# arendu-zz/MacaronicUserModeling

Measured on AMD Instinct MI355X. Metric: LBP sweep iters/sec (whole node), batch=8192 graphs |X|=64, higher is better.
Workload: dtype f64

## Files before the change

include/mlbp.h:

```cpp
#ifndef MLBP_H
#define MLBP_H

#include <stdint.h>

#ifdef __cplusplus
extern "C" {
#endif

#define MLBP_VERSION_MAJOR 0
#define MLBP_VERSION_MINOR 1

enum {
  MLBP_OK = 0,
  MLBP_EINVAL = -1,
  MLBP_EHIP = -2,
  MLBP_ENODEVICE = -3,
  MLBP_ENOMEM = -4,
  MLBP_EUNSUPPORTED = -5
};

int mlbp_version(void);
const char* mlbp_arch(void);
const char* mlbp_last_error(void);
int mlbp_device_count(void);
// ... 16 lines not shown
                       int32_t* unary_slot);

enum { MLBP_OP_UNARY = 0, MLBP_OP_PAIR_TM = 1, MLBP_OP_PAIR_MT = 2, MLBP_OP_VAR = 3 };
int mlbp_compile_sweep(const mlbp_topology* t, int32_t root_var, int32_t* ops, int32_t cap_ops,
                       int32_t* srcs, int32_t cap_srcs, int32_t* n_srcs);

typedef struct mlbp_program mlbp_program;

int mlbp_program_create(const int32_t* ops, int32_t n_ops, const int32_t* srcs, int32_t n_srcs,
                        const int32_t* sweeps, int32_t n_sweeps, int32_t n_msgs, int32_t P, int32_t U,
                        mlbp_program** out);
int mlbp_program_destroy(mlbp_program* p);

int mlbp_program_reserve(mlbp_program* p, int32_t max_graphs);

int mlbp_program_plan(const int32_t* ops, int32_t n_ops, const int32_t* srcs, int32_t n_srcs,
                      const int32_t* sweeps, int32_t n_sweeps, int32_t n_msgs, int32_t P, int32_t U,
                      int32_t* out8);

enum { MLBP_IMAGE_FUSED = 0, MLBP_IMAGE_LEAN = 1, MLBP_IMAGE_SHARED = 2, MLBP_IMAGE_LEAN_READOUT = 3,
       MLBP_IMAGE_SHARED_READOUT = 4, MLBP_IMAGE_PRUNED = 5 };
int mlbp_program_image(const int32_t* ops, int32_t n_ops, const int32_t* srcs, int32_t n_srcs,
                       const int32_t* sweeps, int32_t n_sweeps, int32_t n_msgs, int32_t P, int32_t U,
                       int32_t n_vars, const int32_t* in_off, const int32_t* in_slots,
                       int32_t which, int32_t* out, int32_t cap);

int mlbp_program_set_readout(mlbp_program* p, int32_t n_vars, const int32_t* in_off, const int32_t* in_slots);

int mlbp_program_exact_count(const mlbp_program* p, int32_t B);
int mlbp_program_skippable_updates(const mlbp_program* p);

int mlbp_program_status(const mlbp_program* p);

struct mlbp_gradient_args;

typedef struct mlbp_posterior_args {
  const int32_t* labels;
  double* out;
  double* sum_out;
} mlbp_posterior_args;

typedef struct mlbp_sweep_args {
  int32_t B;
  int32_t X;
  int32_t n_pair_tables;
  int32_t n_unary_tables;
  const double* pair_tables;
  const int32_t* pair_tab;
  const double* unary_tables;
  const int32_t* unary_tab;
  double* msgs;
  int32_t normalize_messages;
  int32_t init_messages;
  double* marginals;
  const struct mlbp_gradient_args* gradient;
  int32_t flags;
  const int32_t* pair_tab_host;
  const float* pair_tables_f32;
  const mlbp_posterior_args* posterior;
} mlbp_sweep_args;

#define MLBP_SWEEP_SHARED_PAIR_TABLES 1
#define MLBP_SWEEP_NO_MESSAGE_WRITEBACK 2
#define MLBP_SWEEP_PAIR_TABLES_F32 4
#define MLBP_SWEEP_DENSE_TABLES 8
#define MLBP_SWEEP_APPROX_INFERENCE 16
#define MLBP_APPROX_K 100
#define MLBP_SWEEP_SKIP_UNCHANGED 32

int mlbp_sweep_f64(const mlbp_program* prog, const mlbp_sweep_args* a, void* stream);

int mlbp_sweep_groups_f64(const mlbp_program* const* progs, const mlbp_sweep_args* args, int32_t n_groups, void* stream);

int mlbp_set_sweep_variant(int32_t variant);

#define MLBP_KERNEL_EXACT 2
#define MLBP_KERNEL_SHARED_MFMA 3
#define MLBP_KERNEL_WIDE 4
#define MLBP_KERNEL_GENERIC 5
#define MLBP_KERNEL_SHARED_GEMM 6
#define MLBP_KERNEL_LEAN 7
int mlbp_last_sweep_kernel(void);
int mlbp_last_sweep_fused_gradient(void);

void mlbp_launch_log_reset(void);
int mlbp_launch_log(const void** handles, int max);

int mlbp_init_messages_f64(double* msgs, int64_t n_rows, int32_t X, void* stream);

int mlbp_marginals_f64(const double* msgs, int32_t B, int32_t n_msgs, int32_t X, int32_t n_vars,
                       const int32_t* in_off, const int32_t* in_slots, int32_t normalize_messages,
                       double* out, void* stream);

int mlbp_log_posterior_f64(const double* marginals, const int32_t* labels, int32_t B, int32_t n_vars,
                           int32_t X, double* out, void* stream);
int mlbp_log_posterior_sum_f64(const double* marginals, const int32_t* labels, int32_t B, int32_t n_vars,
                               int32_t X, double* out, double* sum_out, void* stream);

typedef struct mlbp_posterior_group {
  const double* marginals;
  const int32_t* labels;
  int32_t n_vars, B;
  int64_t start;
} mlbp_posterior_group;
int mlbp_log_posterior_groups_f64(const mlbp_posterior_group* groups, int32_t n_groups, int64_t n_total, int32_t X, double* out,
                                  void* stream);

int mlbp_pair_beliefs_f64(const double* msgs, int32_t B, int32_t n_msgs, int32_t X, int32_t P,
                          const double* pair_tables, const int32_t* pair_tab, int32_t n_pair_tables,
                          const int32_t* c_slot, const int32_t* r_slot, double* out, void* stream);

typedef struct mlbp_gradient_args {
  int32_t B, X, n_msgs, P, U;
  int32_t F_ee, F_ed;
  int32_t Vde;
  int32_t n_pair_tables, n_unary_tables;
  const double* msgs;
  const double* pair_tables;
  const int32_t* pair_tab;
  const int32_t* pair_c_slot;
  const int32_t* pair_r_slot;
  const int32_t* pair_phi;
  const int32_t* pair_label;
  const double* unary_tables;
  const int32_t* unary_tab;
  const int32_t* unary_kind;
  const int32_t* unary_obs;
  const int32_t* unary_label;
  const double* phi_en_en;
  const double* phi_en_en_w1;
  const double* phi_en_de;
  const double* phi_en_en_t;
  const double* phi_en_en_w1_t;
  const double* phi_en_de_t;
  const double* phi_en_en_p;
  const double* phi_en_en_w1_p;
  double* grad_en_en;
  double* grad_en_de;
  int32_t flags;
  const int32_t* pair_tab_host;
  const double* unary_expect;
  const int32_t* pair_slots_host;
  void* workspace;
  int64_t workspace_bytes;
} mlbp_gradient_args;
int64_t mlbp_gradient_workspace_bytes(const mlbp_gradient_args* a);
#define MLBP_GRADIENT_SHARED_PAIR_TABLES 1
#define MLBP_GRADIENT_APPROX_BELIEFS 2
int mlbp_gradient_f64(const mlbp_gradient_args* a, void* stream);

int mlbp_unary_expectations_f64(const double* unary_tables, int32_t n_rows, int32_t X, const int32_t* row_kind,
                                const int32_t* row_obs, const double* phi_en_en_t, const double* phi_en_en_w1_t,
                                const double* phi_en_de_t, int32_t F_ee, int32_t F_ed, int32_t Vde, double* out,
                                void* stream);
int mlbp_gradient_status(void);

int mlbp_patch_unary_tables_f64(const double* base_tables, const int32_t* base_row, const int32_t* item_off,
                                const int32_t* item_x, const int32_t* item_k, const double* item_val,
                                const double* theta, int32_t n_rows, int32_t X, double* out, void* stream);

int mlbp_patch_gradient_f64(const double* priv_tables, const int32_t* item_off, const int32_t* item_x,
                            const int32_t* item_k, const double* item_val, const int32_t* row_graph,
                            const int32_t* row_label, int32_t n_rows, int32_t X, int32_t F, double* grad, void* stream);

int mlbp_sum_rows_f64(const double* in, int64_t rows, int32_t cols, double* out, void* stream);
int mlbp_sum_rows_cat_f64(const double* in0, int32_t cols0, const double* in1, int32_t cols1, const double* in2,
// ... 67 lines not shown
```

macaronicusermodeling_amd/_ffi.py:

```python
import ctypes as C
import os

_PKG = os.path.dirname(os.path.abspath(__file__))
LIB_PATH = os.path.join(_PKG, 'libmlbp.so')

MLBP_OK, MLBP_EINVAL, MLBP_EHIP, MLBP_ENODEVICE, MLBP_ENOMEM, MLBP_EUNSUPPORTED = 0, -1, -2, -3, -4, -5
OP_UNARY, OP_PAIR_TM, OP_PAIR_MT, OP_VAR = 0, 1, 2, 3
IMAGES = ('fused', 'lean', 'shared', 'lean_readout', 'shared_readout', 'pruned')
NORM_ZERO, NORM_UNIFORM = 0, 1


class MlbpError(RuntimeError):
    def __init__(self, code, msg):
        RuntimeError.__init__(self, 'libmlbp error %d: %s' % (code, msg))
        self.code = code


class Topology(C.Structure):
    _fields_ = [('n_vars', C.c_int32), ('n_factors', C.c_int32),
                ('fac_nvars', C.POINTER(C.c_int32)), ('fac_var', C.POINTER(C.c_int32)),
                ('fac_dim', C.POINTER(C.c_int32)), ('var_fac_off', C.POINTER(C.c_int32)),
                ('var_fac', C.POINTER(C.c_int32))]


class GradientArgs(C.Structure):
    _fields_ = [('B', C.c_int32), ('X', C.c_int32), ('n_msgs', C.c_int32), ('P', C.c_int32), ('U', C.c_int32),
                ('F_ee', C.c_int32), ('F_ed', C.c_int32), ('Vde', C.c_int32), ('n_pair_tables', C.c_int32),
                ('n_unary_tables', C.c_int32), ('msgs', C.c_void_p), ('pair_tables', C.c_void_p),
                ('pair_tab', C.c_void_p), ('pair_c_slot', C.c_void_p), ('pair_r_slot', C.c_void_p),
                ('pair_phi', C.c_void_p), ('pair_label', C.c_void_p), ('unary_tables', C.c_void_p),
                ('unary_tab', C.c_void_p), ('unary_kind', C.c_void_p), ('unary_obs', C.c_void_p),
                ('unary_label', C.c_void_p), ('phi_en_en', C.c_void_p), ('phi_en_en_w1', C.c_void_p),
                ('phi_en_de', C.c_void_p), ('phi_en_en_t', C.c_void_p), ('phi_en_en_w1_t', C.c_void_p),
                ('phi_en_de_t', C.c_void_p), ('phi_en_en_p', C.c_void_p), ('phi_en_en_w1_p', C.c_void_p),
                ('grad_en_en', C.c_void_p), ('grad_en_de', C.c_void_p), ('flags', C.c_int32), ('pair_tab_host', C.c_void_p), ('unary_expect', C.c_void_p),
                ('pair_slots_host', C.c_void_p), ('workspace', C.c_void_p), ('workspace_bytes', C.c_int64)]


class PotentialsJob(C.Structure):
    _fields_ = [('phi', C.c_void_p), ('theta', C.c_void_p), ('pot', C.c_void_p), ('pot_t', C.c_void_p),
                ('theta_stride', C.c_int64), ('pot_stride', C.c_int64), ('pot_t_stride', C.c_int64),
                ('rows', C.c_int32), ('cols', C.c_int32), ('F', C.c_int32), ('reserved', C.c_int32),
                ('expect', C.c_void_p), ('expect_stride', C.c_int64)]


class PosteriorArgs(C.Structure):
    _fields_ = [('labels', C.c_void_p), ('out', C.c_void_p), ('sum_out', C.c_void_p)]


class SweepArgs(C.Structure):
    _fields_ = [('B', C.c_int32), ('X', C.c_int32), ('n_pair_tables', C.c_int32),
                ('n_unary_tables', C.c_int32), ('pair_tables', C.c_void_p), ('pair_tab', C.c_void_p),
                ('unary_tables', C.c_void_p), ('unary_tab', C.c_void_p), ('msgs', C.c_void_p),
                ('normalize_messages', C.c_int32), ('init_messages', C.c_int32), ('marginals', C.c_void_p), ('gradient', C.c_void_p),
                ('flags', C.c_int32), ('pair_tab_host', C.c_void_p), ('pair_tables_f32', C.c_void_p), ('posterior', C.c_void_p)]


SWEEP_SHARED_PAIR_TABLES = 1
SWEEP_NO_MESSAGE_WRITEBACK = 2
SWEEP_PAIR_TABLES_F32 = 4
SWEEP_DENSE_TABLES = 8
SWEEP_APPROX_INFERENCE = 16
SWEEP_SKIP_UNCHANGED = 32
APPROX_K = 100
GRADIENT_SHARED_PAIR_TABLES = 1
GRADIENT_APPROX_BELIEFS = 2


_i32p = C.POINTER(C.c_int32)
_vp = C.c_void_p
_i32, _i64 = C.c_int32, C.c_int64

SIGNATURES = {
    'mlbp_version': (C.c_int, []),
    'mlbp_arch': (C.c_char_p, []),
    'mlbp_last_error': (C.c_char_p, []),
    'mlbp_device_count': (C.c_int, []),
    'mlbp_last_sweep_kernel': (C.c_int, []),
    'mlbp_last_sweep_fused_gradient': (C.c_int, []),
    'mlbp_launch_log_reset': (None, []),
    'mlbp_launch_log': (C.c_int, [C.POINTER(_vp), C.c_int]),
    'mlbp_has_loops': (C.c_int, [C.POINTER(Topology), _i32]),
    'mlbp_message_schedule': (C.c_int, [C.POINTER(Topology), _i32, _i32p, _i32]),
    'mlbp_message_slots': (C.c_int, [C.POINTER(Topology), _i32p, _i32p, _i32p, _i32p]),
    'mlbp_compile_sweep': (C.c_int, [C.POINTER(Topology), _i32, _i32p, _i32, _i32p, _i32, _i32p]),
    'mlbp_program_create': (C.c_int, [_i32p, _i32, _i32p, _i32, _i32p, _i32, _i32, _i32, _i32,
                                      C.POINTER(_vp)]),
    'mlbp_program_destroy': (C.c_int, [_vp]),
    'mlbp_program_plan': (C.c_int, [_i32p, _i32, _i32p, _i32, _i32p, _i32, _i32, _i32, _i32, _i32p]),
    'mlbp_program_image': (C.c_int, [_i32p, _i32, _i32p, _i32, _i32p, _i32, _i32, _i32, _i32, _i32, _i32p, _i32p, _i32, _i32p, _i32]),
    'mlbp_program_reserve': (C.c_int, [_vp, _i32]),
    'mlbp_program_set_readout': (C.c_int, [_vp, _i32, _i32p, _i32p]),
    'mlbp_program_exact_count': (C.c_int, [_vp, _i32]),
    'mlbp_program_skippable_updates': (C.c_int, [_vp]),
    'mlbp_program_status': (C.c_int, [_vp]),
    'mlbp_set_sweep_variant': (C.c_int, [_i32]),
    'mlbp_sweep_f64': (C.c_int, [_vp, C.POINTER(SweepArgs), _vp]),
    'mlbp_sweep_groups_f64': (C.c_int, [C.POINTER(_vp), C.POINTER(SweepArgs), _i32, _vp]),
    'mlbp_init_messages_f64': (C.c_int, [_vp, _i64, _i32, _vp]),
    'mlbp_marginals_f64': (C.c_int, [_vp, _i32, _i32, _i32, _i32, _vp, _vp, _i32, _vp, _vp]),
    'mlbp_log_posterior_f64': (C.c_int, [_vp, _vp, _i32, _i32, _i32, _vp, _vp]),
    'mlbp_log_posterior_sum_f64': (C.c_int, [_vp, _vp, _i32, _i32, _i32, _vp, _vp, _vp]),
    'mlbp_log_posterior_groups_f64': (C.c_int, [_vp, _i32, _i64, _i32, _vp, _vp]),
    'mlbp_pair_beliefs_f64': (C.c_int, [_vp, _i32, _i32, _i32, _i32, _vp, _vp, _i32, _vp, _vp, _vp, _vp]),
    'mlbp_gradient_f64': (C.c_int, [C.POINTER(GradientArgs), _vp]),
    'mlbp_gradient_status': (C.c_int, []),
    'mlbp_gradient_workspace_bytes': (C.c_int64, [C.POINTER(GradientArgs)]),
    'mlbp_unary_expectations_f64': (C.c_int, [_vp, _i32, _i32, _vp, _vp, _vp, _vp, _vp, _i32, _i32, _i32, _vp, _vp]),
    'mlbp_patch_unary_tables_f64': (C.c_int, [_vp, _vp, _vp, _vp, _vp, _vp, _vp, _i32, _i32, _vp, _vp]),
    'mlbp_patch_gradient_f64': (C.c_int, [_vp, _vp, _vp, _vp, _vp, _vp, _vp, _i32, _i32, _i32, _vp, _vp]),
    'mlbp_sum_rows_f64': (C.c_int, [_vp, _i64, _i32, _vp, _vp]),
    'mlbp_sum_rows_cat_f64': (C.c_int, [_vp, _i32, _vp, _i32, _vp, _i32, _i64, _i32, _vp, _vp]),
    'mlbp_select_sum_rows_cat_f64': (C.c_int, [_vp, _i32, _vp, _i32, _vp, _i32, _i64, _vp, _vp, _i32, _vp, _vp]),
    'mlbp_segment_sum_rows_f64': (C.c_int, [_vp, _i64, _i32, _vp, _i32, _vp, _vp]),
    'mlbp_step_statistics_f64': (C.c_int, [_vp, _i32, _vp, _i32, _vp, _vp, _i32, _i32, _i64, _vp, _vp, _vp]),
    'mlbp_dense_dot_f64': (C.c_int, [_i32, _i32, _i32, _i32, _vp, _i64, _i64, _i64, _vp, _i64, _i64,
                                     _i64, _vp, _i64, _i64, _vp]),
    'mlbp_pointwise_multiply_f64': (C.c_int, [_vp, _vp, _vp, _i64, _i32, _vp]),
    'mlbp_normalize_f64': (C.c_int, [_vp, _vp, _i32, _i64, _i32, _vp, _vp]),
    'mlbp_topk_f64': (C.c_int, [_vp, _i64, _i32, _i32, _vp, _vp]),
    'mlbp_topk_rows_f64': (C.c_int, [_vp, _i64, _i32, _i32, _vp, _vp]),
    'mlbp_sparse_vec_mat_dot_f64': (C.c_int, [_vp, _i64, _vp, _i64, _i64, _i32, _vp, _i32, _i32, _vp, _vp]),
    'mlbp_sparse_dot_f64': (C.c_int, [_vp, _vp, _i32, _vp, _vp, _i32, _vp, _vp]),
    'mlbp_sparse_pointwise_multiply_f64': (C.c_int, [_vp, _vp, _i32, _i32, _vp, _i32, _vp, _i32, _vp, _vp]),
    'mlbp_sparse_normalize_f64': (C.c_int, [_vp, _i32, _vp, _i32, _vp, _i32, _vp, _vp]),
    'mlbp_potentials_f64': (C.c_int, [_vp, _vp, _i32, _i32, _i32, _vp, _vp, _vp]),
    'mlbp_potentials_multi_f64': (C.c_int, [_vp, _i32, _i32, _vp]),
    'mlbp_log_f64': (C.c_int, [_vp, _vp, _i64, _vp]),
    'mlbp_observed_minus_f64': (C.c_int, [_vp, _i64, _i64, _vp, _vp]),
}


def _load():
    if not os.path.exists(LIB_PATH):
        raise ImportError(
            'libmlbp.so not found at %s.  Build it with `python -m macaronicusermodeling_amd.build` '
            '(hipcc, gfx950).  There is no CPU fallback.' % LIB_PATH)
    import torch
    lib = C.CDLL(LIB_PATH)
    for name, (res, args) in SIGNATURES.items():
        fn = getattr(lib, name)
        fn.restype = res
        fn.argtypes = args
    return lib


lib = _load()


def last_error():
    return lib.mlbp_last_error().decode('utf-8', 'replace')


def check(rc):
    if rc < 0:
        raise MlbpError(rc, last_error())
    return rc


def i32ptr(arr):
    return arr.ctypes.data_as(_i32p)
```

macaronicusermodeling_amd/build.py:

```python
import os
import subprocess
import sys

PKG = os.path.dirname(os.path.abspath(__file__))
CSRC = os.path.join(PKG, 'csrc')
LIB = os.path.join(PKG, 'libmlbp.so')
SOURCES = ['mlbp_host.cpp', 'mlbp_compile.cpp', 'mlbp_compile_shared.cpp', 'mlbp_sweep.hip', 'mlbp_lean.hip', 'mlbp_shared.hip', 'mlbp_gemm.hip', 'mlbp_prims.hip', 'mlbp_grad.hip']
CSRC_MAP = os.path.join(PKG, 'csrc_map')
LIB_MAP = os.path.join(PKG, 'libmlbp_map.so')
SOURCES_MAP = ['mlbp_map.hip']
CSRC_LOGZ = os.path.join(PKG, 'csrc_logz')
LIB_LOGZ = os.path.join(PKG, 'libmlbp_logz.so')
SOURCES_LOGZ = ['mlbp_logz.hip']
FLAGS = ['-O3', '-std=c++17', '-fPIC', '--offload-arch=gfx950', '-fno-fast-math', '-Wall',
         '-Wno-unused-function']


def _stale(obj, deps):
    if not os.path.exists(obj):
        return True
    t = os.path.getmtime(obj)
    return any(os.path.getmtime(d) > t for d in deps)


def _build_one(hipcc, csrc, sources, headers, lib, force, verbose):
    objs = []
    for src in sources:
        path = os.path.join(csrc, src)
        obj = os.path.join(csrc, os.path.splitext(src)[0] + '.o')
        if force or _stale(obj, [path] + headers):
            cmd = [hipcc] + FLAGS + ['-x', 'hip', '-c', path, '-o', obj]
            if verbose:
                cmd.insert(1, '-Rpass-analysis=kernel-resource-usage')
                print(' '.join(cmd))
            subprocess.check_call(cmd)
        objs.append(obj)
    if force or _stale(lib, objs):
        subprocess.check_call([hipcc, '-shared', '-fPIC', '--offload-arch=gfx950', '-o', lib] + objs)
    return lib


def build(force=False, verbose=False):
    hipcc = os.environ.get('HIPCC', '/opt/rocm/bin/hipcc')
    headers = [os.path.join(CSRC, 'mlbp_internal.h'), os.path.join(CSRC, 'mlbp_device.h'), os.path.join(PKG, '..', 'include', 'mlbp.h')]
    lib = _build_one(hipcc, CSRC, SOURCES, headers, LIB, force, verbose)
    headers_map = [os.path.join(CSRC, 'mlbp_device.h'), os.path.join(PKG, '..', 'include', 'mlbp_map.h')]
    _build_one(hipcc, CSRC_MAP, SOURCES_MAP, headers_map, LIB_MAP, force, verbose)
    headers_logz = [os.path.join(CSRC, 'mlbp_device.h'), os.path.join(PKG, '..', 'include', 'mlbp_logz.h')]
    _build_one(hipcc, CSRC_LOGZ, SOURCES_LOGZ, headers_logz, LIB_LOGZ, force, verbose)
    return lib


if __name__ == '__main__':
    print(build(force='--force' in sys.argv, verbose='-v' in sys.argv))
```

macaronicusermodeling_amd/csrc/mlbp_internal.h:

```cpp
#ifndef MLBP_INTERNAL_H
#define MLBP_INTERNAL_H

#include <vector>

#include "../../include/mlbp.h"

namespace mlbp_dev { struct GradFusedDev; }

struct mlbp_program;

namespace mlbp {
int fail(int code, const char* fmt, ...) __attribute__((format(printf, 2, 3)));

#define HIP_TRY(expr)                                                                      \
  do {                                                                                     \
    hipError_t _e = (expr);                                                                \
    if (_e != hipSuccess) return mlbp::fail(MLBP_EHIP, "%s failed: %s", #expr, hipGetErrorString(_e)); \
  } while (0)

int grant_lds(const void* kernel, size_t bytes, bool* fresh = nullptr);
void launch_begin();
int launch_verdict(const char* what);

void launch_log_record(const void* kernel);
#define MLBP_LAUNCH(kernel, ...)                                                           \
  do {                                                                                     \
    mlbp::launch_log_record((const void*)(kernel));                                        \
    hipLaunchKernelGGL(kernel, __VA_ARGS__);                                               \
  } while (0)

int validate_program(const int32_t* ops, int32_t n_ops, const int32_t* srcs, int32_t n_srcs, const int32_t* sweeps,
                     int32_t n_sweeps, int32_t n_msgs, int32_t P, int32_t U, int* max_srcs_out);
int drop_unchanged_updates(const int32_t* ops, const int32_t* srcs, const int32_t* sweeps, int n_sweeps, int n_msgs,
                           std::vector<int32_t>& ops_out, std::vector<int32_t>& sweeps_out);
int find_cprod(const std::vector<std::vector<int32_t>>& cprods, const std::vector<int32_t>& consts);

enum { FOP_UNARY = 0, FOP_PAIR_TM = 1, FOP_PAIR_MT = 2, FOP_VAR = 3, FOP_VAR_PAIR_TM = 4, FOP_VAR_PAIR_MT = 5,
       FOP_BUNDLED = 0x100  };
struct FusedProgram {
  std::vector<int32_t> fops, psrcs, fsweeps, hoist, cpw, pairseq, written;
  int n_cprod = 0;
  bool has_unary_fops = false;
};
void build_fused_program(const int32_t* ops, const int32_t* srcs, const int32_t* sweeps, int n_sweeps, int n_msgs, FusedProgram& out);

constexpr int UOP_VAR = 1;
constexpr int UOP_MT = 2;
constexpr int UOP_PSLOT_SHIFT = 2;
constexpr int UOP_NOP = 32;
constexpr int UOP_STORE_VF = 64;
constexpr int UOP_NSRC_SHIFT = 8;
constexpr int UOP_CARRY_IN = 0x1000;
constexpr int UOP_CARRY_OUT = 0x2000;
struct LeanProgram {
  bool ok = false;
  const char* why = "";
  int n_bundles = 0, HL = 0, n_cprod = 0, WL = 0;
  std::vector<int32_t> image;
  std::vector<char> hoisted;
  std::vector<std::vector<int32_t>> cprods;
};
void build_lean_program(const FusedProgram& fp, int n_msgs, LeanProgram& out);
bool build_lean_readout(const LeanProgram& lp, int n_msgs, int n_vars, const int32_t* in_off, const int32_t* in_slots,
                        std::vector<int32_t>& image);
int launch_lean_sweep(const mlbp_program* prog, const mlbp_sweep_args* a, const mlbp_dev::GradFusedDev* gf, void* stream, bool* launched);
int launch_lean_groups(const mlbp_program* const* progs, const mlbp_sweep_args* args, int n_groups, void* stream, std::vector<char>& member);

struct SharedProgram {
  bool ok = false;
  const char* why = "";
  int n_ops = 0, n_live = 0, n_cpw = 0, n_back = 0, n_fill = 0, n_init = 0, n_bundles = 0;
  int off_ent = 0, off_back = 0, off_fill = 0, off_init = 0, off_ptile = 0, off_written = 0;
  int max_sources = 1;
  bool pf_ok = false;
  int off_pfb = 0, off_stash = 0, off_pinit = 0, n_stash = 0, n_pinit = 0, off_vftile = 0;
  bool vf_direct = false;
  bool p3_ok = false;
  int n_lds = 0, sqrt_mask = 0, off_map3 = 0, off_kind3 = 0, off_back3 = 0;
  std::vector<int32_t> sweeps;
  std::vector<int32_t> image;
  std::vector<int32_t> live_of_slot;
  std::vector<int32_t> hoisted;
  std::vector<char> written;
  std::vector<std::vector<int32_t>> cprods;
};
void build_shared_program(const FusedProgram& fp, int n_msgs, int P, int U, SharedProgram& out);
bool build_shared_readout(const SharedProgram& sp, int n_msgs, int n_vars, const int32_t* in_off, const int32_t* in_slots,
                          std::vector<int32_t>& image);
int launch_shared_sweep(const mlbp_program* prog, const mlbp_sweep_args* a, void* stream, bool* launched);
bool shared_gradient_fused(const mlbp_program* prog, const mlbp_sweep_args* a);
bool exact_kernel_fuses_gradient(const mlbp_program* prog, const mlbp_sweep_args* a);
int gradient_flagged_only(const mlbp_gradient_args* a, const uint8_t* flags, void* stream);
int gradient_flagged_groups(const mlbp_gradient_args* args, const uint8_t* const* flags, int n_groups, mlbp_program* owner, void* stream);
int launch_shared_groups(const mlbp_program* const* progs, const mlbp_sweep_args* args, int n_groups, void* stream, std::vector<char>& member);
int launch_shared_pair_gradient(const mlbp_gradient_args* a, int32_t* status, void* stream);
int launch_gemm_sweep(const mlbp_program* prog, const mlbp_sweep_args* a, void* stream);
int gemm_path_ready();
bool gemm_path_supports(int X);
int launch_gemm_pair_gradient(const mlbp_gradient_args* a, int32_t* status, void* stream);
size_t gemm_gradient_workspace_bytes(const mlbp_gradient_args* a);
size_t shared_gradient_workspace_bytes(const mlbp_gradient_args* a);

int program_grow(mlbp_program* prog, void** p, size_t* cap, size_t bytes, bool zero = false);
int fallback_scratch(int purpose, size_t bytes, void** out);
enum { SCRATCH_GEMM_GRADIENT = 0, SCRATCH_SHARED_GRADIENT = 1, SCRATCH_PURPOSES = 2 };
}

namespace mlbp {
struct GroupTables {
  enum { MAX = 64 };
  struct Entry { std::vector<int32_t> words; int32_t* dev = nullptr; size_t cap_words = 0; };
  std::vector<Entry> entries;
  size_t next_evict = 0;
};
int group_table_device(GroupTables& gt, const std::vector<int32_t>& table, void* stream, int32_t** out);
void group_tables_free(GroupTables& gt);
}

struct mlbp_program {
  int32_t n_ops, n_srcs, n_sweeps, n_msgs, P, U;
  int32_t n_pairseq;
  int32_t max_srcs;
  int32_t* d_ops;
  int32_t* d_srcs;
  int32_t* d_sweeps;
  int32_t* d_pairseq;
  int32_t* d_status;
  int32_t n_fops, n_hoist, n_psrcs, n_cprod, n_cpw, n_written;
  bool sf_ok;
  unsigned char* d_bail;
  int32_t bail_cap;
  int32_t* d_readout;
  int32_t n_vars, n_readout;
  int32_t* d_fops;
  int32_t* d_fsweeps;
  int32_t* d_fpairseq;
  int device;
  mlbp::FusedProgram fused;
  mlbp::LeanProgram lean;
  mlbp_program* pruned = nullptr;
  int32_t n_dropped = 0;
  bool is_twin = false;
  bool last_was_pruned = false;
  int32_t* d_limage = nullptr;
  int32_t* d_lreadout = nullptr;
  mlbp::GroupTables gtables;
  mlbp::GroupTables stables;
  mlbp::SharedProgram shared;
// ... 24 lines not shown
```

macaronicusermodeling_amd/csrc/mlbp_lean.hip:

```cpp
#include <hip/hip_runtime.h>

#include <vector>

#include "mlbp_device.h"
#include "mlbp_internal.h"

using mlbp::fail;
using namespace mlbp_dev;

namespace {

constexpr int WG = 256;

typedef double nt_d2 __attribute__((ext_vector_type(2)));
#define NT_LOAD2(p) ([&] { const nt_d2 v_ = __builtin_nontemporal_load(reinterpret_cast<const nt_d2*>(p)); return make_double2(v_.x, v_.y); }())

constexpr int GROUP_WORDS = 48;
using mlbp::UOP_VAR; using mlbp::UOP_MT; using mlbp::UOP_PSLOT_SHIFT; using mlbp::UOP_NOP; using mlbp::UOP_STORE_VF;
using mlbp::UOP_NSRC_SHIFT; using mlbp::UOP_CARRY_IN; using mlbp::UOP_CARRY_OUT;

struct LeanDev {
  const int32_t* image;
  const int32_t* readout;
  uint8_t* bail;
  int32_t n_bundles, HL, n_cprod, WL, n_ext, init, dense, keep;
};

__device__ __forceinline__ double swapadd16(double a, double b) {
  auto lo = __builtin_amdgcn_permlane16_swap((unsigned)__double2loint(a), (unsigned)__double2loint(b), false, false);
  auto hi = __builtin_amdgcn_permlane16_swap((unsigned)__double2hiint(a), (unsigned)__double2hiint(b), false, false);
  return __hiloint2double((int)hi[0], (int)lo[0]) + __hiloint2double((int)hi[1], (int)lo[1]);
}
__device__ __forceinline__ double swapadd32(double a, double b) {
  auto lo = __builtin_amdgcn_permlane32_swap((unsigned)__double2loint(a), (unsigned)__double2loint(b), false, false);
  auto hi = __builtin_amdgcn_permlane32_swap((unsigned)__double2hiint(a), (unsigned)__double2hiint(b), false, false);
  return __hiloint2double((int)hi[0], (int)lo[0]) + __hiloint2double((int)hi[1], (int)lo[1]);
}

__device__ __forceinline__ bool vote_any(bool p, int32_t* votes, int wave, int lane) {
  const int mine = __ballot(p) != 0 ? 1 : 0;
  if (lane == 0) votes[wave] = mine;
  lds_barrier();
  const int4 v = *reinterpret_cast<const int4*>(votes);
  return (v.x | v.y | v.z | v.w) != 0;
}

struct LaneGeo {
  int tm0, tm1;
  int mt;
  int red_tm;
  int red_mt;
  bool up, st_tm, st_mt, wr_tm;
};

__device__ __forceinline__ double2 lds2(const char* p) { return *reinterpret_cast<const double2*>(p); }
__device__ __forceinline__ void mul2(double2& a, const double2 b) { a.x *= b.x; a.y *= b.y; }

struct RegTable {
  const double2 (&T)[4][2];
  __device__ __forceinline__ double2 operator()(int r, int k) const { return T[r][k]; }
};
struct LdsTable {
  const double2* base;
  __device__ __forceinline__ double2 operator()(int r, int k) const { return base[(r * 2 + k) * WG]; }
};

template <bool MT, bool WIDE, typename TB>
__device__ __forceinline__ void contract(const TB T, char* wb, int u0, int s1, int s2, int s3, int s4, int vf,
                                         const LaneGeo& G, char* redA) {
  const int nsrc = (u0 >> UOP_NSRC_SHIFT) & 15;
  const bool has_vf = (u0 & UOP_STORE_VF) != 0;
  if (MT) {
    double2 ma = lds2(wb + s1 + G.mt), mb = lds2(wb + s1 + G.mt + 16);
    {
      const double2 a = lds2(wb + s2 + G.mt), b = lds2(wb + s2 + G.mt + 16);
      mul2(ma, a); mul2(mb, b);
    }
    if (nsrc > 2) {
      if (WIDE) {
        const double2 a2 = lds2(wb + s3 + G.mt), b2 = lds2(wb + s3 + G.mt + 16);
        const double2 a3 = lds2(wb + s4 + G.mt), b3 = lds2(wb + s4 + G.mt + 16);
        mul2(ma, a2); mul2(mb, b2);
        mul2(ma, a3); mul2(mb, b3);
      } else {
        mul2(ma, lds2(wb + s3 + G.mt)); mul2(mb, lds2(wb + s3 + G.mt + 16));
        if (nsrc > 3) { mul2(ma, lds2(wb + s4 + G.mt)); mul2(mb, lds2(wb + s4 + G.mt + 16)); }
      }
    }
    if (has_vf && G.st_mt) {
      *reinterpret_cast<double2*>(wb + vf + G.mt) = ma;
      *reinterpret_cast<double2*>(wb + vf + G.mt + 16) = mb;
    }
    double a00, a01, a10, a11;
    { const double2 t0 = T(0, 0), t1 = T(0, 1); a00 = ma.x * t0.x; a01 = ma.x * t0.y; a10 = ma.x * t1.x; a11 = ma.x * t1.y; }
    { const double2 t0 = T(1, 0), t1 = T(1, 1); a00 += ma.y * t0.x; a01 += ma.y * t0.y; a10 += ma.y * t1.x; a11 += ma.y * t1.y; }
    { const double2 t0 = T(2, 0), t1 = T(2, 1); a00 += mb.x * t0.x; a01 += mb.x * t0.y; a10 += mb.x * t1.x; a11 += mb.x * t1.y; }
    { const double2 t0 = T(3, 0), t1 = T(3, 1); a00 += mb.y * t0.x; a01 += mb.y * t0.y; a10 += mb.y * t1.x; a11 += mb.y * t1.y; }
    a00 += dpp_mov<0x128>(a10);
    a01 += dpp_mov<0x128>(a11);
    *reinterpret_cast<double*>(redA + G.red_mt) = swapadd32(a00, a01);
  } else {
    double2 m0 = lds2(wb + s1 + G.tm0), m1 = lds2(wb + s1 + G.tm1);
    {
      const double2 a = lds2(wb + s2 + G.tm0), b = lds2(wb + s2 + G.tm1);
      mul2(m0, a); mul2(m1, b);
    }
    if (nsrc > 2) {
      if (WIDE) {
        const double2 a2 = lds2(wb + s3 + G.tm0), b2 = lds2(wb + s3 + G.tm1);
// ... 162 lines not shown
        const int kind = __builtin_amdgcn_readfirstlane(gst[2 * U + u]), obs = __builtin_amdgcn_readfirstlane(gst[3 * U + u]);
        const int lab = __builtin_amdgcn_readfirstlane(gst[4 * U + u]);
        const int cols = kind == 2 ? gf.Vde : 64;
        if ((unsigned)obs >= (unsigned)cols || (unsigned)lab >= 64u || (unsigned)kind > 2u) { bad = true; continue; }
        kd[j] = kind;
        const int slot = __builtin_amdgcn_readfirstlane(gst[u]);
        b[j] = __builtin_amdgcn_readfirstlane(gst[U + u]) ? *reinterpret_cast<const double*>(wb + slot * 512 + lane * 8) : 0.0;
        if (kind == 2) {
          const double2* ph = reinterpret_cast<const double2*>(gf.phi_en_de_t + ((size_t)obs * 64 + lane) * FED);
          at[j] = (obs * 64 + lab) * FED;
          const double2 a0 = ph[0], a1 = ph[1], a2 = ph[2];
          pv[j][0] = a0.x; pv[j][1] = a0.y; pv[j][2] = a1.x; pv[j][3] = a1.y; pv[j][4] = a2.x; pv[j][5] = a2.y;
        } else {
          typedef const double __attribute__((address_space(1))) * gptr1;
          const gptr1 ph = (gptr1)(uintptr_t)((kind ? gf.phi_en_en_w1_t : gf.phi_en_en_t) + ((size_t)obs * 64 + lane) * FEE);
          at[j] = (obs * 64 + lab) * FEE;
#pragma unroll
          for (int q = 0; q < FEE; ++q) pv[j][q] = ph[q];
        }
      }
    }
#pragma unroll
    for (int j = 0; j < UB; ++j) {
      if (kd[j] == 2) {
#pragma unroll
        for (int q = 0; q < FED; ++q) { lab_ed[q] += as_const_f64(gf.phi_en_de_t)[at[j] + q]; exp_ed[q] += b[j] * pv[j][q]; }
      } else if (kd[j] >= 0) {
        const double* base = kd[j] ? gf.phi_en_en_w1_t : gf.phi_en_en_t;
#pragma unroll
        for (int q = 0; q < FEE; ++q) { lab_ee[q] += as_const_f64(base)[at[j] + q]; exp_ee[q] += b[j] * pv[j][q]; }
      }
    }
  }
  if (bad && lane == 0) atomicExch(d.status, 1);
  constexpr int PER = FEE + FEE + FED;
  {
    double ue[FEE], ud[FED];
#pragma unroll
    for (int q = 0; q < FEE; ++q) ue[q] = lab_ee[q] - wave_sum(exp_ee[q]);
#pragma unroll
    for (int q = 0; q < FED; ++q) ud[q] = lab_ed[q] - wave_sum(exp_ed[q]);
    if (lane == 0) {
      double* o = scratch + wave * PER;
#pragma unroll
      for (int q = 0; q < FEE; ++q) o[q] = gsum[q];
#pragma unroll
      for (int q = 0; q < FEE; ++q) o[FEE + q] = ue[q];
#pragma unroll
      for (int q = 0; q < FED; ++q) o[FEE + FEE + q] = ud[q];
    }
  }
  lds_barrier();
  if (t == 0) {
    double tot[PER];
#pragma unroll
    for (int q = 0; q < PER; ++q) tot[q] = (scratch[q] + scratch[PER + q]) + (scratch[2 * PER + q] + scratch[3 * PER + q]);
    double gee[FEE];
#pragma unroll
    for (int q = 0; q < FEE; ++q) gee[q] = tot[FEE + q] - tot[q];
#pragma unroll
    for (int p = 0; p < NT; ++p) {
      if (p < d.P) {
#pragma unroll
        for (int q = 0; q < FEE; ++q) gee[q] += lfs[p * FEE + q];
      }
    }
#pragma unroll
    for (int q = 0; q < FEE; ++q) gf.grad_en_en[(size_t)g * FEE + q] = gee[q];
#pragma unroll
    for (int q = 0; q < FED; ++q) gf.grad_en_de[(size_t)g * FED + q] = tot[FEE + FEE + q];
  }
}

__device__ __forceinline__ double rescale(double r, int& bad) {
  const unsigned key = mag_key(r);
  const unsigned long long normal = __ballot(key - KEY_MIN < KEY_BAD - KEY_MIN);
  const unsigned long long wrong = __ballot(key >= KEY_BAD);
  bad |= (wrong != 0) | (normal == 0);
  const int ref = __builtin_amdgcn_readlane((int)key, normal ? __builtin_ctzll(normal) : 0);
  return __builtin_ldexp(r, 1023 - ((ref >> 20) & 0x7FF));
}

template <int NT, bool PADX, bool MULTI, int NL, bool GRAD>
__global__ __launch_bounds__(WG, (NT >= 7 ? 1 : (NT >= 4 ? 2 : 3))) void sweep_x64_lean_kernel(SweepDev d, LeanDev f, const int32_t* groups,
                                                                                             int n_groups, GradFusedDev gf) {
  int g = blockIdx.x;
  if (MULTI) {
    int lo = 0, hi = n_groups - 1;
    while (lo < hi) {
      const int mid = (lo + hi + 1) >> 1;
      if (as_const(groups)[(size_t)mid * GROUP_WORDS] <= g) lo = mid; else hi = mid - 1;
    }
    const int32_t* G = groups + (size_t)lo * GROUP_WORDS;
    const Words16 w0 = sload16(G), w1 = sload16(G + 16), w2 = sload16(G + 32);
    auto ptr = [](int32_t a, int32_t b) { return (uintptr_t)(uint32_t)a | ((uintptr_t)(uint32_t)b << 32); };
    g -= w0.w[0];
    f.image = (const int32_t*)ptr(w0.w[2], w0.w[3]); f.readout = (const int32_t*)ptr(w0.w[4], w0.w[5]);
    f.bail = (uint8_t*)ptr(w0.w[6], w0.w[7]); d.msgs = (double*)ptr(w0.w[8], w0.w[9]);
    d.marginals = (double*)ptr(w0.w[10], w0.w[11]); d.pair_tables = (const double*)ptr(w0.w[12], w0.w[13]);
    d.pair_tab = (const int32_t*)ptr(w0.w[14], w0.w[15]); d.unary_tables = (const double*)ptr(w1.w[0], w1.w[1]);
    d.unary_tab = (const int32_t*)ptr(w1.w[2], w1.w[3]); d.status = (int32_t*)ptr(w1.w[4], w1.w[5]);
    f.n_bundles = w1.w[6]; f.HL = w1.w[7]; f.n_cprod = w1.w[8]; f.WL = w1.w[9]; f.n_ext = w1.w[10];
    d.n_msgs = w1.w[11]; d.P = w1.w[12]; d.U = w1.w[13]; d.n_vars = w1.w[14]; d.n_pair_tables = w1.w[15];
    d.n_unary_tables = w2.w[0]; f.dense = w2.w[1];
  }
  extern __shared__ double lds[];
  double* work = lds;
  double* red = lds + (size_t)(d.n_msgs + f.n_ext) * 64;
  int32_t* limg = reinterpret_cast<int32_t*>(red + 4 * 256);
  double2* tl = reinterpret_cast<double2*>(limg + 16 * (f.n_bundles + 1));
  int32_t* gst = reinterpret_cast<int32_t*>(tl + (size_t)NL * 8 * WG);

  const int t = threadIdx.x, lane = t & 63, wave = __builtin_amdgcn_readfirstlane(t >> 6);
  const int X = PADX ? d.X : 64;
  const double uniform = 1.0 / (double)X;
  const double uni_l = (!PADX || lane < X) ? uniform : 0.0;
  double* gm = d.msgs + (size_t)g * d.n_msgs * X;
  const int32_t* img_hoist = f.image + 16 * (size_t)f.n_bundles;
  const int32_t* img_cprod = img_hoist + 8 * (size_t)f.HL;
  const int32_t* img_written = img_cprod + 16 * (size_t)f.n_cprod;
  int32_t* votes = reinterpret_cast<int32_t*>(red);
  constexpr bool LEAN_SYNC = !GRAD;
  constexpr bool EARLY = !GRAD;
  static_assert(!(GRAD && PADX), "the GRAD form of phase A loads whole rows: X = 64 only");

  LaneGeo G;
  const int c_ = (lane & 7) | ((lane >> 1) & 8), b3_ = (lane >> 3) & 1, R_ = 4 * wave + (b3_ | ((lane >> 5) << 1));
  {
    const int b5 = lane >> 5, b4 = (lane >> 4) & 1, b2 = (lane >> 2) & 1;
    G.tm0 = (32 * b3_ + 2 * c_) * 8;
    G.tm1 = (32 * (1 - b3_) + 2 * c_) * 8;
    G.mt = 4 * R_ * 8;
    G.red_tm = (4 * R_ + 2 * b4 + b2) * 8;
    G.red_mt = (wave * 64 + 32 * b3_ + 2 * c_ + b5) * 8;
    G.up = b2 != 0;
    G.st_tm = wave == 0 && (lane & 0x28) == 0;
    G.st_mt = (lane & 0x17) == 0;
    G.wr_tm = (lane & 3) == 0;
  }

  if (t == 0) f.bail[g] = 0;
  int g_kind = 0, g_obs = 0, g_lab = 0;
  if (GRAD && t < d.U) {
    g_kind = gf.unary_kind[t]; g_obs = gf.unary_obs[(size_t)g * d.U + t]; g_lab = gf.unary_label[(size_t)g * d.U + t];
  }
  bool ok = true;
  const double* nowhere = reinterpret_cast<const double*>(f.image);
  constexpr int HB = 8;
  double ur[HB];
  int uslot[HB], ufac[HB];
  {
    const Words16 hl = sload16(img_hoist + wave * 2 * f.HL);
#pragma unroll
    for (int j = 0; j < HB; ++j) {
      const int u = hl.w[2 * j];
      uslot[j] = hl.w[2 * j + 1];
      ufac[j] = u;
      if (EARLY) {
        int row = -1;
        if (u >= 0) row = f.dense ? g * d.U + u : as_const(d.unary_tab)[(size_t)g * d.U + u];
        const bool in = (unsigned)row < (unsigned)d.n_unary_tables;
        if (u >= 0 && !in) ok = false;
        const double* at = in ? d.unary_tables + (size_t)row * X + (PADX ? min(lane, X - 1) : lane) : nowhere;
        ur[j] = *at;
      } else {
        ur[j] = 0.0;
        if (u >= 0) {
          const int row = f.dense ? g * d.U + u : as_const(d.unary_tab)[(size_t)g * d.U + u];
          if ((unsigned)row >= (unsigned)d.n_unary_tables) ok = false;
          else ur[j] = d.unary_tables[(size_t)row * X + lane];
        }
      }
    }
  }
  double2 tab[NT][4][2];
#pragma unroll
  for (int p = 0; p < NT; ++p) {
    if (!PADX && EARLY) {
      const int pc = p < d.P ? p : 0;
      const int ti = f.dense ? g * d.P + pc : as_const(d.pair_tab)[(size_t)g * d.P + pc];
      const bool in = (unsigned)ti < (unsigned)d.n_pair_tables;
      if (p < d.P && !in) ok = false;
      const double* T = (p < d.P && in) ? d.pair_tables + (size_t)ti * 4096 + (size_t)(4 * R_) * 64 + 2 * c_ : nowhere;
#pragma unroll
      for (int r = 0; r < 4; ++r) {
        tab[p][r][0] = NT_LOAD2(T + r * 64 + 32 * b3_);
        tab[p][r][1] = NT_LOAD2(T + r * 64 + 32 * (1 - b3_));
      }
    } else if (p < d.P) {
      const int ti = f.dense ? g * d.P + p : as_const(d.pair_tab)[(size_t)g * d.P + p];
      if ((unsigned)ti >= (unsigned)d.n_pair_tables) { ok = false; continue; }
      if (!PADX) {
        const double* T = d.pair_tables + (size_t)ti * 4096 + (size_t)(4 * R_) * 64 + 2 * c_;
#pragma unroll
        for (int r = 0; r < 4; ++r) {
          tab[p][r][0] = NT_LOAD2(T + r * 64 + 32 * b3_);
          tab[p][r][1] = NT_LOAD2(T + r * 64 + 32 * (1 - b3_));
        }
      } else {
        const double* T = d.pair_tables + (size_t)ti * X * X;
#pragma unroll
        for (int r = 0; r < 4; ++r)
#pragma unroll
          for (int k = 0; k < 2; ++k) {
            const int row = 4 * R_ + r, col = 32 * (k ? 1 - b3_ : b3_) + 2 * c_;
            tab[p][r][k].x = (row < X && col < X) ? T[(size_t)row * X + col] : 0.0;
            tab[p][r][k].y = (row < X && col + 1 < X) ? T[(size_t)row * X + col + 1] : 0.0;
          }
      }
    }
  }
#pragma unroll
  for (int p = NT; p < NT + NL; ++p) {
    if (p < d.P && !PADX) {
      const int ti = f.dense ? g * d.P + p : as_const(d.pair_tab)[(size_t)g * d.P + p];
      if ((unsigned)ti >= (unsigned)d.n_pair_tables) { ok = false; continue; }
      const double* T = d.pair_tables + (size_t)ti * 4096 + (size_t)(4 * R_) * 64 + 2 * c_;
#pragma unroll
      for (int r = 0; r < 4; ++r)
#pragma unroll
        for (int k = 0; k < 2; ++k) {
          typedef __attribute__((address_space(3))) void* lds_ptr;
          typedef const __attribute__((address_space(1))) void* glb_ptr;
          double2* dst = tl + ((p - NT) * 8 + r * 2 + k) * WG + wave * 64;
          __builtin_amdgcn_global_load_lds((glb_ptr)(T + r * 64 + 32 * (k ? 1 - b3_ : b3_)), (lds_ptr)dst, 16, 0, 0);
        }
    }
  }
  int dense_word = 0;
  bool dense_ok = true;
  if (EARLY) {
    const int i = min(t, d.P + d.U - 1);
    const int32_t* at = i < d.P ? d.pair_tab + (size_t)g * d.P + i : d.unary_tab + (size_t)g * d.U + (i - d.P);
    dense_word = *(f.dense ? at : f.image);
  } else if (f.dense) {
    for (int i = t; i < d.P + d.U; i += WG)
      dense_ok &= i < d.P ? d.pair_tab[(size_t)g * d.P + i] == g * d.P + i : d.unary_tab[(size_t)g * d.U + (i - d.P)] == g * d.U + (i - d.P);
  }
  constexpr int PW = 2;
  int32_t pre[PW];
#pragma unroll
  for (int q = 0; q < PW; ++q)
    pre[q] = EARLY ? f.image[min(t + q * WG, 16 * (f.n_bundles + 1) - 1)] : ((t + q * WG < 16 * (f.n_bundles + 1)) ? f.image[t + q * WG] : 0);
  unsigned bad_key = 0;
  {
    double2* dst = reinterpret_cast<double2*>(work);
    const int x0 = (2 * t) & 63;
    const double2 uni2 = PADX ? make_double2(x0 < X ? uniform : 0.0, x0 + 1 < X ? uniform : 0.0) : make_double2(uniform, uniform);
    if (f.init) {
      for (int i = t; i < d.n_msgs * 32; i += WG) dst[i] = uni2;
    } else if (!PADX) {
      const double2* src = reinterpret_cast<const double2*>(gm);
      for (int i = t; i < d.n_msgs * 32; i += WG) {
        const double2 v = src[i];
        bad_key = max(bad_key, max(mag_key(v.x), mag_key(v.y)));
        dst[i] = v;
      }
    } else {
      for (int i = t; i < d.n_msgs * 64; i += WG) {
        const int slot = i >> 6, x = i & 63;
        const double v = x < X ? gm[(size_t)slot * X + x] : 0.0;
        bad_key = max(bad_key, mag_key(v));
        work[i] = v;
      }
    }
    if (t < 32) dst[d.n_msgs * 32 + t] = uni2;
    if (t >= 32 && t < 64) dst[(d.n_msgs + f.n_ext - 1) * 32 + (t - 32)] = make_double2(1.0, 1.0);
  }
  lds_barrier();
#pragma unroll
  for (int j = 0; j < HB; ++j) {
    if (uslot[j] >= 0) {
      const double r = (!PADX || lane < X) ? ur[j] : 0.0;
      const double s = wave_sum(r);
      const double m = renorm(r, s, uni_l, true);
      bad_key = max(bad_key, s > 0.0 ? mag_key(m) : KEY_BAD);
      work[uslot[j] * 64 + lane] = m;
      if (GRAD && lane == 0) { gst[ufac[j]] = uslot[j]; gst[d.U + ufac[j]] = s > 0.0 ? 1 : 0; }
    }
  }
  if (GRAD && t < d.U) { gst[2 * d.U + t] = g_kind; gst[3 * d.U + t] = g_obs; gst[4 * d.U + t] = g_lab; }
  for (int j = HB; j < f.HL; ++j) {
    const const_i32p hp = as_const(img_hoist + (wave * f.HL + j) * 2);
    const int u = hp[0], slot = hp[1];
    if (u < 0) break;
    const int row = f.dense ? g * d.U + u : as_const(d.unary_tab)[(size_t)g * d.U + u];
    double r = 0.0;
    if ((unsigned)row >= (unsigned)d.n_unary_tables) ok = false;
    else if (!PADX || lane < X) r = d.unary_tables[(size_t)row * X + lane];
    const double s = wave_sum(r);
    const double m = renorm(r, s, uni_l, true);
    bad_key = max(bad_key, s > 0.0 ? mag_key(m) : KEY_BAD);
    work[slot * 64 + lane] = m;
    if (GRAD && lane == 0) { gst[u] = slot; gst[d.U + u] = s > 0.0 ? 1 : 0; }
  }
  if (LEAN_SYNC ? vote_any(!ok, votes, wave, lane) : !__syncthreads_and(ok ? 1 : 0)) {
    if (t == 0) atomicExch(d.status, 1);
    if (f.init)
      for (int i = t; i < d.n_msgs * X; i += WG) gm[i] = uniform;
    return;
  }
  for (int k = wave; k < f.n_cprod; k += 4) {
    const Words16 cl = sload16(img_cprod + 16 * k);
    double acc = uni_l;
#pragma unroll
    for (int q0 = 1; q0 < 16; q0 += 5) {
      if (cl.w[0] >= q0) {
        double m[5];
#pragma unroll
        for (int q = 0; q < 5; ++q) m[q] = work[cl.w[q0 + q] * 64 + lane];
#pragma unroll
        for (int q = 0; q < 5; ++q) acc *= m[q];
      }
    }
    bad_key = max(bad_key, mag_key(acc));
    work[(d.n_msgs + 1 + k) * 64 + lane] = acc;
  }
  auto fill_limg = [&]() {
    if (NL > 0) asm volatile("s_waitcnt vmcnt(0)" ::: "memory");
#pragma unroll
    for (int q = 0; q < PW; ++q)
      if (t + q * WG < 16 * (f.n_bundles + 1)) limg[t + q * WG] = pre[q];
    for (int i = t + PW * WG; i < 16 * (f.n_bundles + 1); i += WG) limg[i] = f.image[i];
  };
  if (LEAN_SYNC) fill_limg();
  if (LEAN_SYNC ? vote_any(bad_key >= KEY_BAD, votes + 1024, wave, lane) : __syncthreads_or(bad_key >= KEY_BAD ? 1 : 0) != 0) {
    if (t == 0) f.bail[g] = 1;
    return;
  }
  if (!LEAN_SYNC) { fill_limg(); lds_barrier(); }

  char* wb = reinterpret_cast<char*>(work);
  int parity = 0, bad = 0;
  double carry = 1.0;
  const int4* li = reinterpret_cast<const int4*>(limg);
  int4 A0 = li[0], A1 = li[1], B0 = li[2], B1 = li[3];
  for (int k = 0; k < f.n_bundles; ++k) {
    const int4 nA0 = li[4 * k + 4], nA1 = li[4 * k + 5], nB0 = li[4 * k + 6], nB1 = li[4 * k + 7];
    const int fA = __builtin_amdgcn_readfirstlane(A0.x), fB = __builtin_amdgcn_readfirstlane(B0.x);
    if (fA & UOP_VAR) {
      const int nsrc = (fA >> UOP_NSRC_SHIFT) & 15;
      double m = work[(A0.y >> 3) + lane];
      const double m2 = work[(A0.z >> 3) + lane];
      if (fA & UOP_CARRY_IN) m *= carry;
      m *= m2;
      if (nsrc > 2) {
        const double m3 = work[(A0.w >> 3) + lane], m4 = work[(A1.x >> 3) + lane];
        m *= m3;
        m *= m4;
      }
      if (fA & UOP_CARRY_OUT) carry = m;
      else work[(A1.y >> 3) + lane] = m;
    } else {
      char* redP = reinterpret_cast<char*>(red) + parity * 4096;
      front<NT, NL>(tab, tl + t, wb, fA, A0, A1, G, redP);
      const bool two = !(fB & UOP_NOP);
      if (two) front<NT, NL>(tab, tl + t, wb, fB, B0, B1, G, redP + 2048);
      lds_barrier();
      const double* rd = reinterpret_cast<const double*>(redP);
      double rA = rd[lane];
      if (fA & UOP_MT) rA = (rA + rd[64 + lane]) + (rd[128 + lane] + rd[192 + lane]);
      work[(A1.z >> 3) + lane] = rescale(rA, bad);
      if (two) {
        double rB = rd[256 + lane];
        if (fB & UOP_MT) rB = (rB + rd[320 + lane]) + (rd[384 + lane] + rd[448 + lane]);
        work[(B1.z >> 3) + lane] = rescale(rB, bad);
      }
      parity ^= 1;
    }
    A0 = nA0; A1 = nA1; B0 = nB0; B1 = nB1;
  }
  if (bad) {
    if (t == 0) f.bail[g] = 2;
    return;
  }
  lds_barrier();
  double marg[2] = {0.0, 0.0};
  if (EARLY) dense_ok = !f.dense || t >= d.P + d.U || dense_word == (t < d.P ? g * d.P + t : g * d.U + (t - d.P));
  bool bad_out = !dense_ok;
  if (f.readout) {
#pragma unroll
    for (int j = 0; j < 2; ++j) {
      const int v = wave + 4 * j;
      if (v < d.n_vars) {
        const Words16 rl = sload16(f.readout + 16 * v);
        double acc = work[rl.w[1] * 64 + lane];
#pragma unroll
        for (int q0 = 2; q0 < 16; q0 += 7) {
          if (rl.w[0] >= q0) {
            double m[7];
#pragma unroll
            for (int q = 0; q < 7; ++q) m[q] = work[rl.w[q0 + q] * 64 + lane];
#pragma unroll
            for (int q = 0; q < 7; ++q) acc *= m[q];
          }
        }
        const unsigned key = wave_max_u32(mag_key(acc));
        bad_out |= key >= KEY_BAD || key < KEY_MIN;
        marg[j] = acc / wave_sum(acc);
      }
    }
    for (int v = wave + 8; v < d.n_vars; v += 4) {
      const Words16 rl = sload16(f.readout + 16 * v);
      double acc = work[rl.w[1] * 64 + lane];
      for (int q = 2; q <= rl.w[0]; ++q) acc *= work[as_const(f.readout + 16 * v)[q] * 64 + lane];
      const unsigned key = wave_max_u32(mag_key(acc));
      bad_out |= key >= KEY_BAD || key < KEY_MIN;
      if (!bad_out) d.marginals[((size_t)g * d.n_vars + v) * 64 + lane] = acc / wave_sum(acc);
    }
  }
  lds_barrier();
  if (f.keep || GRAD) {
    for (int j0 = 0; j0 < f.WL; j0 += 4) {
      const const_i32p wl = as_const(img_written + wave * f.WL + j0);
      int slot[4];
      double v[4], s[4];
#pragma unroll
      for (int j = 0; j < 4; ++j) { slot[j] = wl[j]; v[j] = slot[j] >= 0 ? work[slot[j] * 64 + lane] : 1.0; }
#pragma unroll
      for (int j = 0; j < 4; ++j) {
        const unsigned key = wave_max_u32(mag_key(v[j]));
        bad_out |= key >= KEY_BAD || key < KEY_MIN;
        s[j] = wave_sum(v[j]);
      }
#pragma unroll
      for (int j = 0; j < 4; ++j)
        if (slot[j] >= 0) work[slot[j] * 64 + lane] = v[j] / s[j];
    }
  }
  if (LEAN_SYNC ? vote_any(bad_out, votes, wave, lane) : __syncthreads_or(bad_out ? 1 : 0) != 0) {
    if (t == 0) f.bail[g] = 3;
    return;
  }
  if (f.keep && !PADX) {
    const double2* src = reinterpret_cast<const double2*>(work);
    double2* dst = reinterpret_cast<double2*>(gm);
    for (int i = t; i < d.n_msgs * 32; i += WG) dst[i] = src[i];
  } else if (f.keep) {
    for (int i = t; i < d.n_msgs * 64; i += WG)
      if ((i & 63) < X) gm[(size_t)(i >> 6) * X + (i & 63)] = work[i];
  }
  if (f.readout) {
#pragma unroll
    for (int j = 0; j < 2; ++j) {
      const int v = wave + 4 * j;
      if (v < d.n_vars) d.marginals[((size_t)g * d.n_vars + v) * 64 + lane] = marg[j];
    }
  }
  if (GRAD) {
    gradient_epilogue<NT>(d, gf, tab, reinterpret_cast<const char*>(work), gst, reinterpret_cast<double*>(red), G, g, R_, c_, b3_);
  }
}

}

namespace mlbp {

static int lean_plan(const mlbp_program* prog, const mlbp_sweep_args* a, bool grad, bool* ok, SweepDev* d, LeanDev* f, size_t* lds) {
  *ok = false;
  const LeanProgram& lp = prog->lean;
  if (!lp.ok || !prog->d_limage || a->X > 64 || a->X < 2 || !a->normalize_messages || prog->P < 1 || prog->P > 8) return MLBP_OK;
  const bool padx = a->X < 64;
  if (padx && prog->P > 4) return MLBP_OK;
  if (a->gradient && padx) return MLBP_OK;
  if (grad && (prog->P > 3 || prog->U > WG)) return fail(MLBP_EINVAL, "lean kernel: fused gradient needs P <= 3 and U <= %d", WG);
  if (a->flags & MLBP_SWEEP_APPROX_INFERENCE) return MLBP_OK;
  if (a->marginals && !prog->d_lreadout && !padx) return MLBP_OK;
  const int n_ext = 2 + lp.n_cprod;
  *lds = ((size_t)(prog->n_msgs + n_ext) * 64 + 4 * 256) * sizeof(double) + 16 * (size_t)(lp.n_bundles + 1) * sizeof(int32_t);
  if (prog->P == 7 && !padx) *lds += 32 * 1024;
  if (grad) *lds += 5 * (size_t)prog->U * sizeof(int32_t);
  if (*lds > 80 * 1024) return MLBP_OK;
  if (prog->P + prog->U > WG) return MLBP_OK;
  const bool dense = (a->flags & MLBP_SWEEP_DENSE_TABLES) != 0;
  if (dense && ((int64_t)a->B * prog->P > a->n_pair_tables || (int64_t)a->B * prog->U > a->n_unary_tables))
    return fail(MLBP_EINVAL, "mlbp_sweep_f64: MLBP_SWEEP_DENSE_TABLES needs B*P pair tables and B*U unary columns");
  mlbp_program* mp = const_cast<mlbp_program*>(prog);
  if (mp->bail_cap < a->B)
    if (int e = mlbp_program_reserve(mp, a->B)) return e;
  d->pair_tables = a->pair_tables; d->pair_tab = a->pair_tab;
  d->unary_tables = a->unary_tables; d->unary_tab = a->unary_tab;
  d->msgs = a->msgs;
  d->ops = nullptr; d->srcs = nullptr; d->sweeps = nullptr; d->pairseq = nullptr;
  d->status = prog->d_status;
  d->n_sweeps = prog->n_sweeps; d->n_msgs = prog->n_msgs; d->P = prog->P; d->U = prog->U; d->X = a->X;
  d->n_pair_tables = a->n_pair_tables; d->n_unary_tables = a->n_unary_tables;
  d->marginals = padx ? nullptr : a->marginals; d->readout = nullptr; d->n_vars = prog->n_vars;
  d->only = nullptr; d->fill_uniform = 0; d->approx_k = 0;
  f->image = prog->d_limage; f->readout = (a->marginals && !padx) ? prog->d_lreadout : nullptr; f->bail = mp->d_bail;
  f->n_bundles = lp.n_bundles; f->HL = lp.HL; f->n_cprod = lp.n_cprod; f->WL = lp.WL;
  f->n_ext = n_ext; f->init = a->init_messages; f->dense = dense ? 1 : 0;
  const bool waived = (a->flags & MLBP_SWEEP_NO_MESSAGE_WRITEBACK) && !padx && (a->marginals || grad) && (!a->gradient || grad);
  f->keep = waived ? 0 : 1;
  *ok = true;
  return MLBP_OK;
}

typedef void (*lean_fn)(SweepDev, LeanDev, const int32_t*, int, GradFusedDev);

template <bool MULTI>
static lean_fn pick_lean(int P, bool padx) {
  if constexpr (!MULTI) {
    if (padx) {
      switch (P) {
        case 1: return sweep_x64_lean_kernel<1, true, false, 0, false>;
        case 2: return sweep_x64_lean_kernel<2, true, false, 0, false>;
        case 3: return sweep_x64_lean_kernel<3, true, false, 0, false>;
        default: return sweep_x64_lean_kernel<4, true, false, 0, false>;
      }
    }
  }
  switch (P) {
    case 1: return sweep_x64_lean_kernel<1, false, MULTI, 0, false>;
    case 2: return sweep_x64_lean_kernel<2, false, MULTI, 0, false>;
    case 3: return sweep_x64_lean_kernel<3, false, MULTI, 0, false>;
    case 4: return sweep_x64_lean_kernel<4, false, MULTI, 0, false>;
    case 5: case 6: return sweep_x64_lean_kernel<6, false, MULTI, 0, false>;
    case 7: return sweep_x64_lean_kernel<6, false, MULTI, 1, false>;
    default: return sweep_x64_lean_kernel<8, false, MULTI, 0, false>;
  }
}
static lean_fn pick_lean_grad(int P) {
  switch (P) {
    case 1: return sweep_x64_lean_kernel<1, false, false, 0, true>;
    case 2: return sweep_x64_lean_kernel<2, false, false, 0, true>;
    default: return sweep_x64_lean_kernel<3, false, false, 0, true>;
  }
}

int launch_lean_sweep(const mlbp_program* prog, const mlbp_sweep_args* a, const GradFusedDev* gf, void* stream, bool* launched) {
  *launched = false;
  SweepDev d;
  LeanDev f;
  size_t lds = 0;
  bool ok = false;
  if (int e = lean_plan(prog, a, gf != nullptr, &ok, &d, &f, &lds)) return e;
  if (!ok) return MLBP_OK;
  lean_fn k = gf ? pick_lean_grad(prog->P) : pick_lean<false>(prog->P, a->X < 64);
  if (int e = grant_lds((const void*)k, lds)) return e;
  launch_begin();
  MLBP_LAUNCH(k, dim3(a->B), dim3(WG), lds, (hipStream_t)stream, d, f, nullptr, 0, gf ? *gf : GradFusedDev{});
  if (int e = launch_verdict("lean sweep")) return e;
  *launched = true;
  return MLBP_OK;
}

int launch_lean_groups(const mlbp_program* const* progs, const mlbp_sweep_args* args, int n_groups, void* stream, std::vector<char>& member) {
  std::vector<int32_t> table;
  size_t lds_max = 0;
  int p_max = 0, total = 0, n_in = 0;
  SweepDev d0;
  LeanDev f0;
  for (int k = 0; k < n_groups; ++k) {
    if (!member[k]) continue;
    member[k] = 0;
    if (args[k].X != 64) continue;
    SweepDev d;
    LeanDev f;
    size_t lds = 0;
    bool ok = false;
    if (int e = lean_plan(progs[k], &args[k], false, &ok, &d, &f, &lds)) return e;
    if (!ok) continue;
    if (n_in == 0) { d0 = d; f0 = f; }
    else if (f.init != f0.init || f.keep != f0.keep || (f.readout != nullptr) != (f0.readout != nullptr)) continue;
    member[k] = 1;
    ++n_in;
    lds_max = std::max(lds_max, lds + (progs[k]->P < 7 ? 32 * 1024 : 0));
    p_max = std::max(p_max, (int)progs[k]->P);
    table.resize(table.size() + GROUP_WORDS, 0);
    int32_t* w = &table[table.size() - GROUP_WORDS];
    auto put = [&](int at, const void* p) { const uintptr_t v = (uintptr_t)p; w[at] = (int32_t)(uint32_t)v; w[at + 1] = (int32_t)(uint32_t)(v >> 32); };
    w[0] = total; w[1] = args[k].B;
    put(2, f.image); put(4, f.readout); put(6, f.bail); put(8, d.msgs); put(10, d.marginals); put(12, d.pair_tables);
    put(14, d.pair_tab); put(16, d.unary_tables); put(18, d.unary_tab); put(20, d.status);
    w[22] = f.n_bundles; w[23] = f.HL; w[24] = f.n_cprod; w[25] = f.WL; w[26] = f.n_ext; w[27] = d.n_msgs; w[28] = d.P; w[29] = d.U;
    w[30] = d.n_vars; w[31] = d.n_pair_tables; w[32] = d.n_unary_tables; w[33] = f.dense;
    total += args[k].B;
  }
  if (n_in == 0) return MLBP_OK;
  mlbp_program* owner = const_cast<mlbp_program*>(progs[0]);
  int32_t* d_gtable = nullptr;
  if (int e = group_table_device(owner->gtables, table, stream, &d_gtable)) return e;
  lean_fn k = pick_lean<true>(p_max, false);
  if (int e = grant_lds((const void*)k, lds_max)) return e;
  launch_begin();
  MLBP_LAUNCH(k, dim3(total), dim3(WG), lds_max, (hipStream_t)stream, d0, f0, d_gtable, n_in, GradFusedDev{});
  return launch_verdict("grouped lean sweep");
}

}
```

macaronicusermodeling_amd/csrc/mlbp_sweep.hip:

```cpp
#include <hip/hip_runtime.h>

#include <atomic>

#include <algorithm>
#include <cfloat>
#include <cstdlib>
#include <cstring>
#include <mutex>
#include <utility>
#include <map>
#include <vector>

#include "mlbp_internal.h"
#include "mlbp_device.h"

using mlbp::fail;
using namespace mlbp_dev;

namespace {

constexpr int WG = 256;

__device__ __forceinline__ bool tables_in_range(const SweepDev& d, int g) {
  bool ok = true;
  for (int i = threadIdx.x; i < d.P; i += WG)
    ok &= (unsigned)d.pair_tab[(size_t)g * d.P + i] < (unsigned)d.n_pair_tables;
  for (int i = threadIdx.x; i < d.U; i += WG)
    ok &= (unsigned)d.unary_tab[(size_t)g * d.U + i] < (unsigned)d.n_unary_tables;
  int all_ok = __syncthreads_and(ok ? 1 : 0);
  if (!all_ok && threadIdx.x == 0) atomicExch(d.status, 1);
  return all_ok != 0;
}

__device__ __forceinline__ void marginals_from_lds_x64(const SweepDev& d, const double* msg, int g, int wave, int lane) {
  if (!d.marginals) return;
  const const_i32p off = as_const(d.readout), slots = as_const(d.readout + d.n_vars + 1);
  for (int v = wave; v < d.n_vars; v += 4) {
    double acc = 1.0 / 64.0;
    for (int q = off[v]; q < off[v + 1]; ++q) acc = mul_nan_to_num(msg[slots[q] * 64 + lane], acc);
    d.marginals[((size_t)g * d.n_vars + v) * 64 + lane] = renorm(acc, wave_sum(acc), 1.0 / 64.0, true);
  }
}

using mlbp::FOP_UNARY; using mlbp::FOP_PAIR_TM; using mlbp::FOP_PAIR_MT; using mlbp::FOP_VAR;
using mlbp::FOP_VAR_PAIR_TM; using mlbp::FOP_VAR_PAIR_MT; using mlbp::FOP_BUNDLED;

constexpr int LP_MAX_BLOCKS = 4096;
constexpr int LP_WG = 256;
__device__ double g_lp_partials[LP_MAX_BLOCKS];
__device__ unsigned g_lp_done[2] = {0, 0};

struct PosteriorDev {
  const int32_t* labels;
  double* out;
  double* sum_out;
  unsigned generation;
  int32_t pad_;
};

struct FusedDev {
  PosteriorDev post;
  const uint8_t* only;
  const int32_t* image;
  const int32_t* fsweeps;
  int32_t n_fops, n_psrcs, n_hoist, n_cprod, n_cpw, n_ext, init;
  int32_t n_graphs;
};
constexpr int FIXUP_GRAPHS_PER_WG = 64;

template <bool MT>
__device__ __forceinline__ void pair_partials(const double2 (&T)[8], const double* m, double* red, int rg, int cp,
                                              int lane) {
  if (MT) {
    double a0 = 0.0, a1 = 0.0;
#pragma unroll
    for (int k = 0; k < 8; ++k) {
      const double mi = m[8 * k + rg];
      a0 += mi * T[k].x;
      a1 += mi * T[k].y;
    }
    reinterpret_cast<double2*>(red + rg * 64)[cp] = make_double2(a0, a1);
  } else {
    const double2 mj = reinterpret_cast<const double2*>(m)[cp];
    double v[8];
#pragma unroll
    for (int k = 0; k < 8; ++k) v[k] = T[k].x * mj.x + T[k].y * mj.y;
    {
      const bool up = lane & 8;
#pragma unroll
      for (int i = 0; i < 4; ++i) {
        const double send = up ? v[i] : v[i + 4], keep = up ? v[i + 4] : v[i];
        v[i] = keep + dpp_mov<0x140>(send);
      }
    }
    {
      const bool up = lane & 4;
#pragma unroll
      for (int i = 0; i < 2; ++i) {
        const double send = up ? v[i] : v[i + 2], keep = up ? v[i + 2] : v[i];
        v[i] = keep + dpp_mov<0x141>(send);
      }
    }
    {
      const bool up = lane & 2;
      const double send = up ? v[0] : v[1], keep = up ? v[1] : v[0];
      v[0] = keep + dpp_mov<0x1B>(send);
    }
    v[0] += dpp_mov<0xB1>(v[0]);
    if ((lane & 1) == 0) {
      const int k = ((lane >> 3) & 1) * 4 + ((lane >> 2) & 1) * 2 + ((lane >> 1) & 1);
      red[((lane >> 4) & 1) * 64 + 8 * k + rg] = v[0];
    }
  }
}

template <int NT>
__device__ __forceinline__ void gradient_epilogue_x64(const SweepDev& d, const GradFusedDev& gf, const double2 (&tab)[NT][8],
                                                      const double* msg, const int32_t* umsg, const int32_t* upos,
                                                      double* scratch, int g) {
  const int32_t* ukind = upos + d.U;
  const int32_t* uobs = ukind + d.U;
  const int32_t* ulab = uobs + d.U;
  constexpr int FEE = 3, FED = 6;
  const int t = threadIdx.x, lane = t & 63, wave = t >> 6, rg = t >> 5, cp = t & 31;
  double pacc[NT][FEE + 1];
#pragma unroll
  for (int p = 0; p < NT; ++p) {
#pragma unroll
    for (int f = 0; f <= FEE; ++f) pacc[p][f] = 0.0;
    if (p < d.P) {
      const double* c = msg + gf.pair_c_slot[p] * 64;
      const double* r = msg + gf.pair_r_slot[p] * 64;
      const double* phi = gf.pair_phi[p] ? gf.phi_en_en_w1 : gf.phi_en_en;
      const double2 rj = reinterpret_cast<const double2*>(r)[cp];
#pragma unroll
      for (int k = 0; k < 8; ++k) {
        const double ci = c[8 * k + rg];
        const double w0 = (ci * rj.x) * tab[p][k].x, w1 = (ci * rj.y) * tab[p][k].y;
        pacc[p][0] += w0 + w1;
        const double* ph = phi + ((size_t)(8 * k + rg) * 64 + 2 * cp) * FEE;
#pragma unroll
        for (int f = 0; f < FEE; ++f) pacc[p][1 + f] += w0 * ph[f] + w1 * ph[FEE + f];
      }
#pragma unroll
      for (int f = 0; f <= FEE; ++f) pacc[p][f] = wave_sum(pacc[p][f]);
    }
  }
  double uee[FEE] = {0.0, 0.0, 0.0}, ued[FED] = {0.0, 0.0, 0.0, 0.0, 0.0, 0.0};
  bool bad = false;
  constexpr int UB = 3;
  for (int u0 = wave; u0 < d.U; u0 += 4 * UB) {
    double b[UB], pv[UB][FED];
    int kd[UB], at[UB];
#pragma unroll
    for (int j = 0; j < UB; ++j) {
      const int u = u0 + 4 * j;
      kd[j] = -1;
      if (u < d.U) {
        const int kind = __builtin_amdgcn_readfirstlane(ukind[u]), obs = __builtin_amdgcn_readfirstlane(uobs[u]);
        const int lab = __builtin_amdgcn_readfirstlane(ulab[u]);
        const int cols = kind == 2 ? gf.Vde : 64;
        if ((unsigned)obs >= (unsigned)cols || (unsigned)lab >= 64u) { bad = true; continue; }
        kd[j] = kind;
        b[j] = upos[u] ? msg[umsg[u] * 64 + lane] : 0.0;
        if (kind == 2) {
          const double* ph = gf.phi_en_de_t + ((size_t)obs * 64 + lane) * FED;
          at[j] = (obs * 64 + lab) * FED;
#pragma unroll
          for (int f = 0; f < FED; ++f) pv[j][f] = ph[f];
        } else {
          const double* ph = (kind ? gf.phi_en_en_w1_t : gf.phi_en_en_t) + ((size_t)obs * 64 + lane) * FEE;
          at[j] = (obs * 64 + lab) * FEE;
#pragma unroll
          for (int f = 0; f < FEE; ++f) pv[j][f] = ph[f];
        }
      }
    }
#pragma unroll
    for (int j = 0; j < UB; ++j) {
      if (kd[j] == 2) {
#pragma unroll
        for (int f = 0; f < FED; ++f) ued[f] += gf.phi_en_de_t[at[j] + f] - wave_sum(b[j] * pv[j][f]);
      } else if (kd[j] >= 0) {
        const double* base = kd[j] ? gf.phi_en_en_w1_t : gf.phi_en_en_t;
#pragma unroll
        for (int f = 0; f < FEE; ++f) uee[f] += base[at[j] + f] - wave_sum(b[j] * pv[j][f]);
      }
    }
  }
  if (bad && lane == 0) atomicExch(d.status, 1);
  constexpr int PER = NT * (FEE + 1) + FEE + FED;
  if (lane == 0) {
    double* o = scratch + wave * PER;
#pragma unroll
    for (int p = 0; p < NT; ++p)
#pragma unroll
      for (int f = 0; f <= FEE; ++f) o[p * (FEE + 1) + f] = pacc[p][f];
#pragma unroll
    for (int f = 0; f < FEE; ++f) o[NT * (FEE + 1) + f] = uee[f];
#pragma unroll
    for (int f = 0; f < FED; ++f) o[NT * (FEE + 1) + FEE + f] = ued[f];
  }
  lds_barrier();
  if (t == 0) {
    double tot[PER];
#pragma unroll
    for (int q = 0; q < PER; ++q) tot[q] = (scratch[q] + scratch[PER + q]) + (scratch[2 * PER + q] + scratch[3 * PER + q]);
    double gee[FEE];
#pragma unroll
    for (int f = 0; f < FEE; ++f) gee[f] = tot[NT * (FEE + 1) + f];
    bool lbad = false;
#pragma unroll
    for (int p = 0; p < NT; ++p) {
      if (p < d.P) {
        const int l0 = gf.pair_label[((size_t)g * d.P + p) * 2], l1 = gf.pair_label[((size_t)g * d.P + p) * 2 + 1];
        if ((unsigned)l0 >= 64u || (unsigned)l1 >= 64u) { lbad = true; continue; }
        const double* phi = gf.pair_phi[p] ? gf.phi_en_en_w1 : gf.phi_en_en;
        const double Z = tot[p * (FEE + 1)];
#pragma unroll
        for (int f = 0; f < FEE; ++f)
          gee[f] += phi[((size_t)l0 * 64 + l1) * FEE + f] - (Z > 0.0 ? tot[p * (FEE + 1) + 1 + f] / Z : 0.0);
      }
    }
    if (lbad) atomicExch(d.status, 1);
#pragma unroll
    for (int f = 0; f < FEE; ++f) gf.grad_en_en[(size_t)g * FEE + f] = gee[f];
#pragma unroll
    for (int f = 0; f < FED; ++f) gf.grad_en_de[(size_t)g * FED + f] = tot[NT * (FEE + 1) + FEE + f];
  }
}

template <bool NORM, int NT, bool GRAD>
__device__ __forceinline__ void sweep_x64_fused_body(const SweepDev& d, const FusedDev& f, const GradFusedDev& gf, const int g) {
  extern __shared__ double lds[];
  double* msg = lds;
  double* gin = lds + (size_t)(d.n_msgs + f.n_ext) * 64;
  double* red = gin + 64;
  int32_t* prog = reinterpret_cast<int32_t*>(red + 512);
  const int32_t* psrcs = prog + f.n_fops * 8;
  const int32_t* phoist = psrcs + f.n_psrcs;
  const int32_t* pcp = phoist + 2 * f.n_hoist;
  int32_t* tabidx = const_cast<int32_t*>(pcp) + f.n_cpw;
  int32_t* flags = tabidx + d.P + d.U;
  int32_t* umsg = flags + 4;
  int32_t* upos = umsg + d.U;

  const int t = threadIdx.x;
  const int lane = t & 63, wave = t >> 6;
  const int rg = t >> 5, cp = t & 31;
  double* gm = d.msgs + (size_t)g * d.n_msgs * 64;
  const double uniform = 1.0 / 64.0;
  const const_i32p c_fsweeps = as_const(f.fsweeps), c_pairseq = as_const(d.pairseq);

  bool ok = true;
  for (int i = t; i < d.P + d.U; i += WG) {
    const int v = i < d.P ? d.pair_tab[(size_t)g * d.P + i] : d.unary_tab[(size_t)g * d.U + (i - d.P)];
    ok &= (unsigned)v < (unsigned)(i < d.P ? d.n_pair_tables : d.n_unary_tables);
    tabidx[i] = v;
  }
  {
    const int n_img = f.n_fops * 8 + f.n_psrcs + 2 * f.n_hoist + f.n_cpw;
    for (int i = t; i < n_img; i += WG) prog[i] = f.image[i];
    double2* dst = reinterpret_cast<double2*>(msg);
    if (f.init) {
      for (int i = t; i < d.n_msgs * 32; i += WG) dst[i] = make_double2(uniform, uniform);
    } else {
      const double2* src = reinterpret_cast<const double2*>(gm);
      for (int i = t; i < d.n_msgs * 32; i += WG) dst[i] = src[i];
    }
    if (t < 32) dst[d.n_msgs * 32 + t] = make_double2(uniform, uniform);
    if (t == 0) flags[0] = 0;
    if (GRAD)
      for (int i = t; i < d.U; i += WG) {
        umsg[i] = -1; upos[i] = 0;
        upos[d.U + i] = gf.unary_kind[i];
        upos[2 * d.U + i] = gf.unary_obs[(size_t)g * d.U + i];
        upos[3 * d.U + i] = gf.unary_label[(size_t)g * d.U + i];
      }
  }
  if (!__syncthreads_and(ok ? 1 : 0)) {
    if (t == 0) atomicExch(d.status, 1);
    return;
  }

  constexpr int NR = NT > 0 ? NT : 1;
  double2 tab[NR][8];
  int pair_k = 0;
  if (NT > 0) {
#pragma unroll
    for (int p = 0; p < NT; ++p) {
      if (p < d.P) {
        const int ti = __builtin_amdgcn_readfirstlane(tabidx[p]);
        const double2* T = reinterpret_cast<const double2*>(d.pair_tables + (size_t)ti * 4096);
#pragma unroll
        for (int k = 0; k < 8; ++k) tab[p][k] = T[k * WG + t];
      }
    }
  } else {
    const int s0 = c_pairseq[0];
    if (s0 >= 0) {
      const int ti = __builtin_amdgcn_readfirstlane(tabidx[s0]);
      const double2* T = reinterpret_cast<const double2*>(d.pair_tables + (size_t)ti * 4096);
#pragma unroll
      for (int k = 0; k < 8; ++k) tab[0][k] = T[k * WG + t];
    }
  }
  constexpr int HB = 8;
  for (int h0 = wave; h0 < f.n_hoist; h0 += 4 * HB) {
    double r[HB];
#pragma unroll
    for (int j = 0; j < HB; ++j) {
      const int h = h0 + 4 * j;
      r[j] = (h < f.n_hoist) ? d.unary_tables[(size_t)tabidx[d.P + phoist[2 * h]] * 64 + lane] : 0.0;
    }
#pragma unroll
    for (int j = 0; j < HB; ++j) {
      const int h = h0 + 4 * j;
      if (h < f.n_hoist) {
        const double tot = wave_sum(r[j]);
        msg[phoist[2 * h + 1] * 64 + lane] = renorm(r[j], tot, uniform, NORM);
        if (GRAD && lane == 0) { umsg[phoist[2 * h]] = phoist[2 * h + 1]; upos[phoist[2 * h]] = tot > 0.0 ? 1 : 0; }
      }
    }
  }
  lds_barrier();
  {
    int at = 0;
    for (int k = 0; k < f.n_cprod; ++k) {
      const int cnt = pcp[at];
      if ((k & 3) == wave) {
        double acc = uniform;
        bool clean = true;
        for (int q = 0; q < cnt; ++q) {
          acc *= msg[pcp[at + 1 + q] * 64 + lane];
          clean = clean && __all(__builtin_isfinite(acc));
        }
        msg[(d.n_msgs + 1 + k) * 64 + lane] = clean ? acc : __builtin_nan("");
      }
      at += 1 + cnt;
    }
  }
  lds_barrier();

  for (int s = 0; s < d.n_sweeps; ++s) {
    const int op0 = c_fsweeps[2 * s], nop = c_fsweeps[2 * s + 1];
    for (int o = op0; o < op0 + nop; ++o) {
      const int4 h0 = reinterpret_cast<const int4*>(prog)[2 * o];
      const int4 h1 = reinterpret_cast<const int4*>(prog)[2 * o + 1];
      const int kind = __builtin_amdgcn_readfirstlane(h0.x) & 0xFF;
      if (kind == FOP_UNARY) {
        if (wave == 0) {
          const int us = __builtin_amdgcn_readfirstlane(h0.y), c = __builtin_amdgcn_readfirstlane(h0.w);
          const double r = d.unary_tables[(size_t)tabidx[d.P + us] * 64 + lane];
          msg[c * 64 + lane] = renorm(r, wave_sum(r), uniform, NORM);
        }
        continue;
      }
      int pslot, dst;
      const double* m;
      const bool from_var = (kind == FOP_VAR || kind == FOP_VAR_PAIR_TM || kind == FOP_VAR_PAIR_MT);
      const int c = __builtin_amdgcn_readfirstlane(h0.w);
      if (from_var) {
        if (wave == 0) {
          const int a = __builtin_amdgcn_readfirstlane(h0.y), n = __builtin_amdgcn_readfirstlane(h0.z);
          const int4 s4 = *reinterpret_cast<const int4*>(psrcs + a);
          double acc = msg[s4.x * 64 + lane];
          if (n > 1) acc *= msg[s4.y * 64 + lane];
          if (n > 2) acc *= msg[s4.z * 64 + lane];
          if (n > 3) acc *= msg[s4.w * 64 + lane];
          for (int q = 4; q < n; ++q) acc *= msg[psrcs[a + q] * 64 + lane];
          const bool fast = __all(acc >= 0.0 && acc < __builtin_huge_val()) && __any(acc > 0.0);
          if (fast && kind != FOP_VAR) {
            gin[lane] = acc;
            if (lane == 0) flags[0] = 0;
          } else {
            const int ae = __builtin_amdgcn_readfirstlane(h1.z), ne = __builtin_amdgcn_readfirstlane(h1.w);
            double ex = uniform;
            for (int q = 0; q < ne; ++q) ex = mul_nan_to_num(msg[psrcs[ae + q] * 64 + lane], ex);
            const double mn = renorm(ex, wave_sum(ex), uniform, NORM);
            msg[c * 64 + lane] = mn;
            gin[lane] = mn;
            if (lane == 0) flags[0] = 1;
          }
        }
        if (kind == FOP_VAR) continue;
        m = gin;
        pslot = __builtin_amdgcn_readfirstlane(h1.x);
        dst = __builtin_amdgcn_readfirstlane(h1.y);
      } else {
        pslot = __builtin_amdgcn_readfirstlane(h0.y);
        m = msg + __builtin_amdgcn_readfirstlane(h0.z) * 64;
        dst = c;
      }
      const bool mt = (kind == FOP_PAIR_MT || kind == FOP_VAR_PAIR_MT);
      lds_barrier();
      if (NT > 0) {
#pragma unroll
        for (int p = 0; p < NT; ++p) {
          if (p == pslot) {
            if (mt) pair_partials<true>(tab[p], m, red, rg, cp, lane);
            else pair_partials<false>(tab[p], m, red, rg, cp, lane);
          }
        }
      } else {
        double2 cur[8];
#pragma unroll
        for (int k = 0; k < 8; ++k) cur[k] = tab[0][k];
        ++pair_k;
        const int sn = c_pairseq[pair_k];
        if (sn >= 0) {
          const int ti = __builtin_amdgcn_readfirstlane(tabidx[sn]);
          const double2* T = reinterpret_cast<const double2*>(d.pair_tables + (size_t)ti * 4096);
#pragma unroll
          for (int k = 0; k < 8; ++k) tab[0][k] = T[k * WG + t];
        }
        if (mt) pair_partials<true>(cur, m, red, rg, cp, lane);
        else pair_partials<false>(cur, m, red, rg, cp, lane);
      }
      if (from_var && wave == 1 && flags[0] == 0) {
        const double v = gin[lane];
        msg[c * 64 + lane] = renorm(v, wave_sum(v), uniform, NORM);
      }
      lds_barrier();
      if (wave == 0) {
        double r;
        if (mt) {
          r = 0.0;
#pragma unroll
          for (int q = 0; q < 8; ++q) r += red[q * 64 + lane];
        } else {
          r = red[lane] + red[64 + lane];
        }
        msg[dst * 64 + lane] = renorm(r, wave_sum(r), uniform, NORM);
      }
    }
  }
  lds_barrier();
  {
    const double2* src = reinterpret_cast<const double2*>(msg);
    double2* dst = reinterpret_cast<double2*>(gm);
    for (int i = t; i < d.n_msgs * 32; i += WG) dst[i] = src[i];
  }
  if (NORM) marginals_from_lds_x64(d, msg, g, wave, lane);
  if (GRAD) gradient_epilogue_x64<(NT > 0 ? NT : 1)>(d, gf, tab, msg, umsg, upos, red, g);
}

__device__ __forceinline__ int posterior_prefetch_label(const SweepDev& d, const PosteriorDev& p, int base, int n_graphs) {
  const int t = threadIdx.x, v = t >> 6, g = base + (t & 63);
  if (!p.labels || d.n_vars > WG / 64 || v >= d.n_vars || g >= n_graphs) return -1;
  return p.labels[(size_t)g * d.n_vars + v];
}
__device__ __forceinline__ void posterior_of_block(const SweepDev& d, const PosteriorDev& p, int base, int n_graphs, int my_label) {
  __shared__ double part[WG / 64];
  __shared__ double lpv[WG];
  __shared__ bool last;
  __syncthreads();
  const int t = threadIdx.x, lane = t & 63, wave = t >> 6;
  double total = 0.0;
  const int g = base + t;
  if (d.n_vars <= WG / 64) {
    double lp = 0.0;
    if (wave < d.n_vars && base + lane < n_graphs) {
      if ((unsigned)my_label >= 64u) atomicExch(d.status, 1);
      else {
        lp = log(d.marginals[((size_t)(base + lane) * d.n_vars + wave) * 64 + my_label]);
        if (lp == -__builtin_huge_val()) lp = -99.99;
      }
    }
    lpv[t] = lp;
    __syncthreads();
    if (t < FIXUP_GRAPHS_PER_WG && g < n_graphs) {
      for (int v = 0; v < d.n_vars; ++v) total += lpv[v * 64 + t];
      p.out[g] = total;
    }
  } else if (t < FIXUP_GRAPHS_PER_WG && g < n_graphs) {
    for (int v = 0; v < d.n_vars; ++v) {
      const int lab = p.labels[(size_t)g * d.n_vars + v];
      if ((unsigned)lab >= 64u) { atomicExch(d.status, 1); continue; }
      const double lp = log(d.marginals[((size_t)g * d.n_vars + v) * 64 + lab]);
      total += (lp == -__builtin_huge_val()) ? -99.99 : lp;
    }
    p.out[g] = total;
  }
  if (!p.sum_out) return;
  if (wave == 0) {
    const double ws = wave_sum(total);
    if (lane == 0) {
      g_lp_partials[blockIdx.x] = ws;
      __threadfence();
      if (blockIdx.x == 0) g_lp_done[(p.generation + 1) & 1] = 0;
      last = atomicAdd(&g_lp_done[p.generation & 1], 1u) == gridDim.x - 1;
    }
  }
  __syncthreads();
  if (!last) return;
  __threadfence();
  double acc = 0.0;
  for (unsigned q = t; q < gridDim.x; q += WG) acc += __builtin_nontemporal_load(&g_lp_partials[q]);
  const double fs = wave_sum(acc);
  if (lane == 0) part[wave] = fs;
  __syncthreads();
  if (t == 0) {
    double v = part[0];
    for (int w = 1; w < WG / 64; ++w) v += part[w];
    *p.sum_out = v;
    g_lp_done[p.generation & 1] = 0;
  }
}

template <bool NORM, int NT, bool GRAD>
__global__ __launch_bounds__(WG, (NT >= 4 ? 2 : (NT == 3 ? 3 : 4))) void sweep_x64_fused_kernel(SweepDev d, FusedDev f, GradFusedDev gf) {
  int base = blockIdx.x;
  unsigned long long todo = 1;
  int my_label = -1;
  if (f.only) {
    base = blockIdx.x * FIXUP_GRAPHS_PER_WG;
    const int mine = base + (threadIdx.x & 63);
    my_label = posterior_prefetch_label(d, f.post, base, f.n_graphs);
    todo = __ballot(mine < f.n_graphs && f.only[mine] != 0);
  }
  while (todo) {
    const int i = __builtin_ctzll(todo);
    todo &= todo - 1;
    sweep_x64_fused_body<NORM, NT, GRAD>(d, f, gf, base + i);
    if (todo) __syncthreads();
  }
  if (f.only && f.post.labels) posterior_of_block(d, f.post, base, f.n_graphs, my_label);
}

struct FixupGroup { SweepDev d; FusedDev f; int32_t first_block, per_wg; };
__global__ __launch_bounds__(WG, 4) void sweep_x64_fixup_groups_kernel(const FixupGroup* groups, int n_groups) {
  int lo = 0, hi = n_groups - 1;
  while (lo < hi) {
    const int mid = (lo + hi + 1) >> 1;
    if (groups[mid].first_block <= (int)blockIdx.x) lo = mid; else hi = mid - 1;
  }
  const FixupGroup& G = groups[lo];
  const int base = ((int)blockIdx.x - G.first_block) * G.per_wg;
  const int mine = base + (threadIdx.x & 63);
  unsigned long long todo = __ballot((int)(threadIdx.x & 63) < G.per_wg && mine < G.f.n_graphs && G.f.only[mine] != 0);
  if (!todo) return;
  const SweepDev d = G.d;
  const FusedDev f = G.f;
  const GradFusedDev gf = {};
  while (todo) {
    const int i = __builtin_ctzll(todo);
    todo &= todo - 1;
    sweep_x64_fused_body<true, 0, false>(d, f, gf, base + i);
    if (todo) __syncthreads();
  }
}

__device__ __forceinline__ double block_sum(double v, double* scratch ) {
  v = wave_sum(v);
  __syncthreads();
  if ((threadIdx.x & 63) == 0) scratch[threadIdx.x >> 6] = v;
  __syncthreads();
  return scratch[0] + scratch[1] + scratch[2] + scratch[3];
}

template <bool NORM, bool LDSMSG>
__global__ __launch_bounds__(WG) void sweep_generic_kernel(SweepDev d) {
  extern __shared__ double lds[];
  const int X = d.X;
// ... 249 lines not shown
    double* o = out + ((size_t)g * n_vars + v) * X;
    for (int j = t; j < X; j += WG) {
      double acc = uniform;
      for (int q = s0; q < s1; ++q) acc = nan_to_num(gm[(size_t)in_slots[q] * X + j] * acc);
      o[j] = acc;
      part += acc;
    }
    if (normalize) {
      const double total = block_sum(part, scratch);
      for (int j = t; j < X; j += WG) o[j] = renorm(o[j], total, uniform, true);
    }
    __syncthreads();
  }
}


__global__ __launch_bounds__(LP_WG) void log_posterior_kernel(const double* marg, const int32_t* labels, int B, int n_vars, int X,
                                                              double* out, double* sum_out, int32_t* status, unsigned generation) {
  __shared__ double part[LP_WG / 64];
  __shared__ bool last;
  const int g = blockIdx.x * LP_WG + threadIdx.x, lane = threadIdx.x & 63, wave = threadIdx.x >> 6;
  double total = 0.0;
  if (g < B) {
    for (int v = 0; v < n_vars; ++v) {
      int lab = labels[(size_t)g * n_vars + v];
      if ((unsigned)lab >= (unsigned)X) { atomicExch(status, 1); continue; }
      double lp = log(marg[((size_t)g * n_vars + v) * X + lab]);
      total += (lp == -__builtin_huge_val()) ? -99.99 : lp;
    }
    out[g] = total;
  }
  if (!sum_out) return;
  const double ws = wave_sum(total);
  if (lane == 0) part[wave] = ws;
  __syncthreads();
  if (threadIdx.x == 0) {
    double v = part[0];
    for (int w = 1; w < LP_WG / 64; ++w) v += part[w];
    g_lp_partials[blockIdx.x] = v;
    __threadfence();
    if (blockIdx.x == 0) g_lp_done[(generation + 1) & 1] = 0;
    last = atomicAdd(&g_lp_done[generation & 1], 1u) == gridDim.x - 1;
  }
  __syncthreads();
  if (!last) return;
  __threadfence();
  double acc = 0.0;
  for (unsigned q = threadIdx.x; q < gridDim.x; q += LP_WG) acc += __builtin_nontemporal_load(&g_lp_partials[q]);
  const double fs = wave_sum(acc);
  if (lane == 0) part[wave] = fs;
  __syncthreads();
  if (threadIdx.x == 0) {
    double v = part[0];
    for (int w = 1; w < LP_WG / 64; ++w) v += part[w];
    *sum_out = v;
    g_lp_done[generation & 1] = 0;
  }
}

__global__ __launch_bounds__(LP_WG) void log_posterior_groups_kernel(const mlbp_posterior_group* groups, int n_groups, long long n_total, int X,
                                                                     double* out, int32_t* status) {
  const long long i = (long long)blockIdx.x * LP_WG + threadIdx.x;
  if (i >= n_total) return;
  int lo = 0, hi = n_groups - 1;
  while (lo < hi) {
    const int mid = (lo + hi + 1) >> 1;
    if (groups[mid].start <= i) lo = mid; else hi = mid - 1;
  }
  const mlbp_posterior_group g = groups[lo];
  const long long b = i - g.start;
  if (b >= g.B) return;
  double total = 0.0;
  for (int v = 0; v < g.n_vars; ++v) {
    const int lab = g.labels[(size_t)b * g.n_vars + v];
    if ((unsigned)lab >= (unsigned)X) { atomicExch(status, 1); continue; }
    const double lp = log(g.marginals[((size_t)b * g.n_vars + v) * X + lab]);
    total += (lp == -__builtin_huge_val()) ? -99.99 : lp;
  }
  out[i] = total;
}

int g_sweep_variant = 1;
thread_local int g_last_kernel = -1;
thread_local int g_last_fused_gradient = 0;
}

namespace mlbp {
bool exact_kernel_fuses_gradient(const mlbp_program* prog, const mlbp_sweep_args* a) {
  const mlbp_gradient_args* ga = a->gradient;
  if (!ga || a->X != 64 || !a->normalize_messages) return false;
  if (ga->B != a->B || ga->X != a->X || ga->P != prog->P || ga->U != prog->U || ga->n_msgs != prog->n_msgs || ga->msgs != a->msgs) return false;
  if (prog->P == 0 && a->B > 1024) return false;
  return ga->F_ee == 3 && ga->F_ed == 6 && prog->P >= 0 && prog->P <= 3 && prog->n_hoist == prog->U && prog->U <= WG &&
         ga->phi_en_en_t && ga->phi_en_en_w1_t && ga->phi_en_de_t && !(ga->flags & MLBP_GRADIENT_APPROX_BELIEFS);
}
}

namespace {
int check_device() {
  int n = 0;
  if (hipGetDeviceCount(&n) != hipSuccess || n <= 0) {
    (void)hipGetLastError();
    return fail(MLBP_ENODEVICE, "no HIP device visible: libmlbp.so has no CPU fallback");
  }
  return MLBP_OK;
}

int32_t* g_status = nullptr;
int global_status(int32_t** out) {
  if (!g_status) {
    HIP_TRY(hipMalloc(&g_status, sizeof(int32_t)));
    HIP_TRY(hipMemset(g_status, 0, sizeof(int32_t)));
  }
  *out = g_status;
  return MLBP_OK;
}

}

extern "C" {

int mlbp_device_count(void) {
  int n = 0;
  if (hipGetDeviceCount(&n) != hipSuccess) {
    (void)hipGetLastError();
    return 0;
  }
  return n;
}

static int create_program(const int32_t* ops, int32_t n_ops, const int32_t* srcs, int32_t n_srcs,
                          const int32_t* sweeps, int32_t n_sweeps, int32_t n_msgs, int32_t P, int32_t U,
                          mlbp_program** out, bool with_pruned);

int mlbp_program_create(const int32_t* ops, int32_t n_ops, const int32_t* srcs, int32_t n_srcs,
                        const int32_t* sweeps, int32_t n_sweeps, int32_t n_msgs, int32_t P, int32_t U,
                        mlbp_program** out) {
  return create_program(ops, n_ops, srcs, n_srcs, sweeps, n_sweeps, n_msgs, P, U, out, true);
}

static int create_program(const int32_t* ops, int32_t n_ops, const int32_t* srcs, int32_t n_srcs,
                          const int32_t* sweeps, int32_t n_sweeps, int32_t n_msgs, int32_t P, int32_t U,
                          mlbp_program** out, bool with_pruned) {
  if (!out) return fail(MLBP_EINVAL, "out is NULL");
  *out = nullptr;
  int max_srcs = 0;
  if (int e = mlbp::validate_program(ops, n_ops, srcs, n_srcs, sweeps, n_sweeps, n_msgs, P, U, &max_srcs)) return e;
  std::vector<int32_t> pairseq;
  for (int s = 0; s < n_sweeps; ++s) {
    const int first = sweeps[2 * s], cnt = sweeps[2 * s + 1];
    for (int o = first; o < first + cnt; ++o)
      if (ops[4 * o] == MLBP_OP_PAIR_TM || ops[4 * o] == MLBP_OP_PAIR_MT) pairseq.push_back(ops[4 * o + 1]);
  }
  if (int e = check_device()) return e;
  mlbp_program* p = new mlbp_program();
  p->n_ops = n_ops; p->n_srcs = n_srcs; p->n_sweeps = n_sweeps; p->n_msgs = n_msgs; p->P = P; p->U = U;
  p->n_pairseq = (int)pairseq.size();
  p->max_srcs = max_srcs;
  pairseq.push_back(-1);
  p->d_ops = p->d_srcs = p->d_sweeps = p->d_pairseq = p->d_status = nullptr;
  p->d_fops = p->d_fsweeps = p->d_fpairseq = nullptr;
  (void)hipGetDevice(&p->device);
  auto up = [&](int32_t** dst, const int32_t* src, size_t n) -> hipError_t {
    hipError_t e = hipMalloc(dst, (n ? n : 1) * sizeof(int32_t));
    if (e != hipSuccess) return e;
    return n ? hipMemcpy(*dst, src, n * sizeof(int32_t), hipMemcpyHostToDevice) : hipSuccess;
  };
  hipError_t e = up(&p->d_ops, ops, (size_t)n_ops * 4);
  std::vector<int32_t> srcs_padded(srcs ? srcs : nullptr, srcs ? srcs + n_srcs : nullptr);
  srcs_padded.resize(((size_t)n_srcs + 16 + 3) / 4 * 4, 0);
  if (e == hipSuccess) e = up(&p->d_srcs, srcs_padded.data(), srcs_padded.size());
  if (e == hipSuccess) e = up(&p->d_sweeps, sweeps, (size_t)n_sweeps * 2);
  if (e == hipSuccess) e = up(&p->d_pairseq, pairseq.data(), pairseq.size());
  int32_t zero = 0;
  if (e == hipSuccess) e = up(&p->d_status, &zero, 1);
  mlbp::FusedProgram fp;
  mlbp::build_fused_program(ops, srcs, sweeps, n_sweeps, n_msgs, fp);
  p->n_fops = (int)fp.fops.size() / 8;
  p->n_hoist = (int)fp.hoist.size() / 2;
  p->n_psrcs = (int)fp.psrcs.size();
  p->n_cprod = fp.n_cprod;
  p->n_cpw = (int)fp.cpw.size();
  std::vector<int32_t> image(fp.fops);
  image.insert(image.end(), fp.psrcs.begin(), fp.psrcs.end());
  image.insert(image.end(), fp.hoist.begin(), fp.hoist.end());
  image.insert(image.end(), fp.cpw.begin(), fp.cpw.end());
  image.insert(image.end(), fp.written.begin(), fp.written.end());
  p->n_written = (int)fp.written.size();
  p->sf_ok = !fp.has_unary_fops;
  p->d_bail = nullptr;
  p->bail_cap = 0;
  p->d_readout = nullptr;
  p->n_vars = 0;
  p->n_readout = 0;
  p->d_simage = p->d_sreadout = nullptr;
  p->d_tfrag = nullptr;
  p->h_ops.assign(ops, ops + 4 * (size_t)n_ops);
  p->h_sweeps.assign(sweeps, sweeps + 2 * (size_t)n_sweeps);
  p->n_sreadout = 0;
  mlbp::build_shared_program(fp, n_msgs, P, U, p->shared);
  if (p->shared.ok && e == hipSuccess) e = up(&p->d_simage, p->shared.image.data(), p->shared.image.size());
  p->fused = fp;
  mlbp::build_lean_program(fp, n_msgs, p->lean);
  if (p->lean.ok && e == hipSuccess) e = up(&p->d_limage, p->lean.image.data(), p->lean.image.size());
  if (e == hipSuccess) e = up(&p->d_fops, image.data(), image.size());
  if (e == hipSuccess) e = up(&p->d_fsweeps, fp.fsweeps.data(), fp.fsweeps.size());
  if (e == hipSuccess) e = up(&p->d_fpairseq, fp.pairseq.data(), fp.pairseq.size());
  if (e != hipSuccess) {
    mlbp_program_destroy(p);
    return fail(MLBP_EHIP, "mlbp_program_create: device upload failed: %s", hipGetErrorString(e));
  }
  if (with_pruned) {
    std::vector<int32_t> ops2, sweeps2;
    p->n_dropped = mlbp::drop_unchanged_updates(ops, srcs, sweeps, n_sweeps, n_msgs, ops2, sweeps2);
    if (p->n_dropped > 0) {
      if (int rc = create_program(ops2.data(), (int)ops2.size() / 4, srcs, n_srcs, sweeps2.data(), n_sweeps, n_msgs, P, U, &p->pruned, false)) {
        mlbp_program_destroy(p);
        return rc;
      }
      p->pruned->is_twin = true;
    }
  }
  *out = p;
  return MLBP_OK;
}

static const mlbp_program* effective_program(const mlbp_program* p, const mlbp_sweep_args* a) {
  const bool pruned = p && a && (a->flags & MLBP_SWEEP_SKIP_UNCHANGED) && p->pruned;
  if (p && a && !p->is_twin) const_cast<mlbp_program*>(p)->last_was_pruned = pruned;
  return pruned ? p->pruned : p;
}

int mlbp_program_destroy(mlbp_program* p) {
  if (!p) return MLBP_OK;
  if (p->pruned) (void)mlbp_program_destroy(p->pruned);
  (void)hipFree(p->d_ops); (void)hipFree(p->d_srcs); (void)hipFree(p->d_sweeps);
  (void)hipFree(p->d_pairseq); (void)hipFree(p->d_status);
  (void)hipFree(p->d_fops); (void)hipFree(p->d_fsweeps); (void)hipFree(p->d_fpairseq); (void)hipFree(p->d_bail); (void)hipFree(p->d_readout);
  (void)hipFree(p->d_limage); (void)hipFree(p->d_lreadout); (void)hipFree(p->d_simage); (void)hipFree(p->d_sreadout); (void)hipFree(p->d_tfrag); (void)hipFree(p->d_spill); (void)hipFree(p->d_ptiles); (void)hipFree(p->d_wfrag); (void)hipFree(p->d_header);
  if (p->side_stream) (void)hipStreamDestroy((hipStream_t)p->side_stream);
  if (p->ev_fork) (void)hipEventDestroy((hipEvent_t)p->ev_fork);
  if (p->ev_join) (void)hipEventDestroy((hipEvent_t)p->ev_join);
  (void)hipFree(p->d_gfrag); (void)hipFree(p->d_gxbuf); (void)hipFree(p->d_gwork);
  for (void* q : p->retired) (void)hipFree(q);
  mlbp::group_tables_free(p->gtables); mlbp::group_tables_free(p->stables);
  delete p;
  return MLBP_OK;
}

static int gradient_behind_sweeps(const mlbp_program* prog, const mlbp_gradient_args* ga, void* stream) {
  mlbp_gradient_args g = *ga;
  if (!g.workspace) {
    const int64_t need = mlbp_gradient_workspace_bytes(&g);
    if (need > 0) {
      mlbp_program* mp = const_cast<mlbp_program*>(prog);
      if (int e = mlbp::program_grow(mp, &mp->d_gwork, &mp->gwork_cap, (size_t)need)) return e;
      g.workspace = mp->d_gwork;
      g.workspace_bytes = (int64_t)mp->gwork_cap;
// ... 10 lines not shown
static int posterior_behind_sweeps(const mlbp_program* prog, const mlbp_sweep_args* a, void* stream) {
  const mlbp_posterior_args* pa = a->posterior;
  if (!pa) return MLBP_OK;
  return mlbp_log_posterior_sum_f64(a->marginals, pa->labels, a->B, prog->n_vars, a->X, pa->out, pa->sum_out, stream);
}

static int check_sweep_args(const mlbp_program* prog, const mlbp_sweep_args* a) {
  if (a->B <= 0 || a->X <= 0) return fail(MLBP_EINVAL, "mlbp_sweep_f64: B=%d X=%d", a->B, a->X);
  if (!a->msgs) return fail(MLBP_EINVAL, "mlbp_sweep_f64: msgs is NULL");
  const bool f32_tables = (a->flags & MLBP_SWEEP_PAIR_TABLES_F32) != 0;
  if (prog->P > 0 && (!(f32_tables ? (const void*)a->pair_tables_f32 : (const void*)a->pair_tables) || !a->pair_tab || a->n_pair_tables <= 0))
    return fail(MLBP_EINVAL, "mlbp_sweep_f64: program has %d pairwise factors but no pair tables", prog->P);
  if (prog->U > 0 && (!a->unary_tables || !a->unary_tab || a->n_unary_tables <= 0))
    return fail(MLBP_EINVAL, "mlbp_sweep_f64: program has %d unary factors but no unary tables", prog->U);
  if (a->X > 4096) return fail(MLBP_EUNSUPPORTED, "mlbp_sweep_f64: X=%d > 4096", a->X);
  const bool approx = (a->flags & MLBP_SWEEP_APPROX_INFERENCE) != 0;
  if (approx && a->X < MLBP_APPROX_K)
    return fail(MLBP_EINVAL, "mlbp_sweep_f64: approximate inference keeps the %d largest entries; kth(=%d) out of bounds (%d)",
                MLBP_APPROX_K, MLBP_APPROX_K - 1, a->X);
  if (approx && !(a->X > 64 && a->X <= 1024 && a->normalize_messages && !f32_tables))
    return fail(MLBP_EUNSUPPORTED, "mlbp_sweep_f64: batched approximate inference needs 100 <= X <= 1024, normalised messages, float64 tables");
  if (f32_tables && !(a->X == 256 || a->X == 512))
    return fail(MLBP_EUNSUPPORTED, "mlbp_sweep_f64: float32 pairwise tables need X = 256 or 512 (got %d)", a->X);
  if (f32_tables && a->gradient) return fail(MLBP_EUNSUPPORTED, "mlbp_sweep_f64: no gradient with float32 pairwise tables");
  if (int e = check_device()) return e;
  int dev = -1;
  if (hipGetDevice(&dev) != hipSuccess || dev != prog->device)
    return fail(MLBP_EINVAL, "mlbp_sweep_f64: the program was created on device %d, the calling thread's current device is %d",
                prog->device, dev);
  if (a->marginals && !prog->d_readout)
    return fail(MLBP_EINVAL, "mlbp_sweep_f64: marginals requested but mlbp_program_set_readout was not called");
  if (a->posterior && (!a->marginals || !a->posterior->labels || !a->posterior->out))
    return fail(MLBP_EINVAL, "mlbp_sweep_f64: posterior needs marginals, labels and an output array");
  const mlbp_gradient_args* ga = a->gradient;
  if (ga && (ga->B != a->B || ga->X != a->X || ga->P != prog->P || ga->U != prog->U || ga->n_msgs != prog->n_msgs || ga->msgs != a->msgs))
    return fail(MLBP_EINVAL, "mlbp_sweep_f64: gradient arguments do not describe the same batch");
  return MLBP_OK;
}

static void fill_sweep_dev(const mlbp_program* prog, const mlbp_sweep_args* a, SweepDev* d) {
  memset(d, 0, sizeof(*d));
  d->pair_tables = a->pair_tables; d->pair_tab = a->pair_tab; d->unary_tables = a->unary_tables; d->unary_tab = a->unary_tab;
  d->msgs = a->msgs; d->ops = prog->d_ops; d->srcs = prog->d_srcs; d->sweeps = prog->d_sweeps; d->pairseq = prog->d_pairseq;
  d->status = prog->d_status;
  d->n_sweeps = prog->n_sweeps; d->n_msgs = prog->n_msgs; d->P = prog->P; d->U = prog->U; d->X = a->X;
  d->n_pair_tables = a->n_pair_tables; d->n_unary_tables = a->n_unary_tables;
  d->readout = prog->d_readout; d->n_vars = prog->n_vars;
}

constexpr size_t X64_LDS_MAX = 160 * 1024;
static size_t fill_fixup_group(const mlbp_program* prog, const mlbp_sweep_args* a, FixupGroup* G) {
  memset(G, 0, sizeof(*G));
  fill_sweep_dev(prog, a, &G->d);
  G->d.pairseq = prog->d_fpairseq;
  G->d.marginals = a->normalize_messages ? a->marginals : nullptr;
  FusedDev& f = G->f;
  f.image = prog->d_fops; f.fsweeps = prog->d_fsweeps;
  f.n_fops = prog->n_fops; f.n_psrcs = prog->n_psrcs; f.n_hoist = prog->n_hoist; f.n_cprod = prog->n_cprod; f.n_cpw = prog->n_cpw;
  f.n_ext = 1 + prog->n_cprod; f.init = a->init_messages; f.n_graphs = a->B;
  const size_t img_words = (size_t)prog->n_fops * 8 + prog->n_psrcs + 2 * prog->n_hoist + prog->n_cpw + prog->n_written;
  return ((size_t)(prog->n_msgs + f.n_ext) * 64 + 64 + 512) * sizeof(double) + (img_words + prog->P + 6 * prog->U + 8) * sizeof(int32_t);
}

struct SweepTail {
  bool marginals = true;
  bool grad_done = false;
  bool grad_flagged = false;
  bool post_done = false;
};
static int sweep_tail(const mlbp_program* prog, const mlbp_sweep_args* a, const SweepTail& t, void* stream) {
  if (a->marginals && t.marginals)
    if (int e = mlbp_marginals_f64(a->msgs, a->B, prog->n_msgs, a->X, prog->n_vars, prog->d_readout, prog->d_readout + prog->n_vars + 1,
                                   a->normalize_messages ? 1 : 0, a->marginals, stream)) return e;
  if (a->gradient && !t.grad_done)
    if (int e = t.grad_flagged ? mlbp::gradient_flagged_only(a->gradient, prog->d_bail, stream) : gradient_behind_sweeps(prog, a->gradient, stream))
      return e;
  return t.post_done ? MLBP_OK : posterior_behind_sweeps(prog, a, stream);
}

enum FastPass { FAST_NONE, FAST_LEAN, FAST_SHARED };

static int run_sweep(const mlbp_program* prog, const mlbp_sweep_args* a, FastPass pass, int variant, void* stream) {
  g_last_fused_gradient = 0;
  hipStream_t st = (hipStream_t)stream;
  const bool norm = a->normalize_messages != 0;
  FixupGroup G;
  const size_t lds = fill_fixup_group(prog, a, &G);
  if (a->X == 64 && lds <= X64_LDS_MAX) {
    mlbp_program* mp = const_cast<mlbp_program*>(prog);
    const bool fast = variant == 1;
    if (pass == FAST_NONE && fast) {
      bool launched = false;
      if (int e = mlbp::launch_shared_sweep(prog, a, stream, &launched)) return e;
      if (launched) pass = FAST_SHARED;
    }
    const bool exact_grad = mlbp::exact_kernel_fuses_gradient(prog, a) && pass != FAST_LEAN;
    const bool shared_grad = pass == FAST_SHARED && mlbp::shared_gradient_fused(prog, a);
    SweepTail tail;
    tail.marginals = !norm;
    tail.grad_done = exact_grad && (pass != FAST_SHARED || shared_grad);
    tail.grad_flagged = shared_grad && !exact_grad;
    GradFusedDev gf = {};
    if (tail.grad_done) {
      const mlbp_gradient_args* ga = a->gradient;
      gf.pair_c_slot = ga->pair_c_slot; gf.pair_r_slot = ga->pair_r_slot; gf.pair_phi = ga->pair_phi; gf.pair_label = ga->pair_label;
      gf.unary_kind = ga->unary_kind; gf.unary_obs = ga->unary_obs; gf.unary_label = ga->unary_label;
      gf.phi_en_en = ga->phi_en_en; gf.phi_en_en_w1 = ga->phi_en_en_w1;
      gf.phi_en_en_t = ga->phi_en_en_t; gf.phi_en_en_w1_t = ga->phi_en_en_w1_t; gf.phi_en_de_t = ga->phi_en_de_t;
      gf.grad_en_en = ga->grad_en_en; gf.grad_en_de = ga->grad_en_de; gf.Vde = ga->Vde; gf.enabled = 1;
    }
    if (pass == FAST_NONE && fast && norm && prog->sf_ok && prog->P >= 1 && prog->P <= 8) {
      bool launched = false;
      if (int e = mlbp::launch_lean_sweep(prog, a, tail.grad_done ? &gf : nullptr, stream, &launched)) return e;
      if (launched) pass = FAST_LEAN;
    }
    g_last_kernel = pass == FAST_SHARED ? MLBP_KERNEL_SHARED_MFMA : (pass == FAST_LEAN ? MLBP_KERNEL_LEAN : MLBP_KERNEL_EXACT);
    g_last_fused_gradient = (tail.grad_done || tail.grad_flagged) ? 1 : 0;
    FusedDev& f = G.f;
    f.only = pass != FAST_NONE ? mp->d_bail : nullptr;
    const mlbp_posterior_args* pa = a->posterior;
    tail.post_done = pa && f.only && norm && (a->B + FIXUP_GRAPHS_PER_WG - 1) / FIXUP_GRAPHS_PER_WG <= LP_MAX_BLOCKS;
    if (tail.post_done) {
      f.post.labels = pa->labels; f.post.out = pa->out; f.post.sum_out = pa->sum_out;
      f.post.generation = pa->sum_out ? next_lp_generation() : 0u;
    }
    const int nt = (prog->P >= 1 && prog->P <= 3) ? prog->P : 0;
    void (*k)(SweepDev, FusedDev, GradFusedDev) = nullptr;
#define MLBP_PICK(N) k = tail.grad_done ? sweep_x64_fused_kernel<true, N, true> : (norm ? sweep_x64_fused_kernel<true, N, false> : sweep_x64_fused_kernel<false, N, false>)
    switch (nt) {
      case 1: MLBP_PICK(1); break;
      case 2: MLBP_PICK(2); break;
      case 3: MLBP_PICK(3); break;
      default: MLBP_PICK(0); break;
    }
#undef MLBP_PICK
    if (int e = mlbp::grant_lds((const void*)k, lds)) return e;
    mlbp::launch_begin();
    MLBP_LAUNCH(k, dim3(f.only ? (a->B + FIXUP_GRAPHS_PER_WG - 1) / FIXUP_GRAPHS_PER_WG : a->B), dim3(WG), lds, st, G.d, f, gf);
    if (int e = mlbp::launch_verdict("exact X = 64 sweep")) return e;
    return sweep_tail(prog, a, tail, stream);
  }
  const bool approx = (a->flags & MLBP_SWEEP_APPROX_INFERENCE) != 0;
  const bool small_lean_candidate = a->X < 64 && a->X >= 2 && norm && prog->sf_ok && prog->P >= 1 && prog->P <= 4 && variant == 1 &&
                                    !a->gradient && prog->lean.ok && prog->d_limage;
  if (a->init_messages && !small_lean_candidate) {
    int e = mlbp_init_messages_f64(a->msgs, (int64_t)a->B * prog->n_msgs, a->X, stream);
    if (e) return e;
  }
  if ((a->flags & MLBP_SWEEP_SHARED_PAIR_TABLES) && a->pair_tab_host && mlbp::gemm_path_supports(a->X) && !approx &&
      prog->P >= 1 && prog->P <= 16 && variant == 1) {
    const int eg = mlbp::launch_gemm_sweep(prog, a, stream);
    if (eg != MLBP_EUNSUPPORTED) {
      if (eg) return eg;
      g_last_kernel = MLBP_KERNEL_SHARED_GEMM;
      return sweep_tail(prog, a, SweepTail(), stream);
    }
  }
  SweepDev d;
  fill_sweep_dev(prog, a, &d);
  const bool f32_tables = (a->flags & MLBP_SWEEP_PAIR_TABLES_F32) != 0;
  d.approx_k = approx ? MLBP_APPROX_K : 0;
  const bool wide_exact = a->X == 128 || a->X == 256 || a->X == 512;
  const bool wide_padded = !wide_exact && !f32_tables && norm && a->X > 64 && a->X <= 1024;
  if (wide_exact || wide_padded) {
    g_last_kernel = MLBP_KERNEL_WIDE;
    void (*kw)(SweepDev) = nullptr;
    int xp = a->X;
    if (f32_tables) {
      d.pair_tables = reinterpret_cast<const double*>(a->pair_tables_f32);
      if (a->X == 256) kw = norm ? sweep_wide_kernel<true, 1, float, 4, 0> : sweep_wide_kernel<false, 1, float, 4, 0>;
      else kw = norm ? sweep_wide_kernel<true, 2, float, 4, 0> : sweep_wide_kernel<false, 2, float, 4, 0>;
    } else if (a->X == 128) kw = norm ? sweep_wide_kernel<true, 1, double, 2, 0> : sweep_wide_kernel<false, 1, double, 2, 0>;
    else if (a->X == 256) kw = norm ? sweep_wide_kernel<true, 2, double, 2, 0> : sweep_wide_kernel<false, 2, double, 2, 0>;
    else if (a->X == 512) kw = norm ? sweep_wide_kernel<true, 4, double, 2, 0> : sweep_wide_kernel<false, 4, double, 2, 0>;
    else {
      const int q = (a->X + 127) / 128;
      const bool odd = (a->X & 1) != 0;
#define MLBP_WIDE_PAD(QQ) (kw = odd ? sweep_wide_kernel<true, QQ, double, 2, 2> : sweep_wide_kernel<true, QQ, double, 2, 1>, xp = 128 * QQ)
      if (q <= 1) MLBP_WIDE_PAD(1);
      else if (q <= 2) MLBP_WIDE_PAD(2);
      else if (q <= 3) MLBP_WIDE_PAD(3);
      else if (q <= 4) MLBP_WIDE_PAD(4);
      else if (q <= 6) MLBP_WIDE_PAD(6);
      else MLBP_WIDE_PAD(8);
#undef MLBP_WIDE_PAD
    }
    const size_t ldsw = ((size_t)6 * xp + 4) * sizeof(double);
    mlbp::launch_begin();
    MLBP_LAUNCH(kw, dim3(a->B), dim3(WG), ldsw, st, d);
    if (int e = mlbp::launch_verdict("wide sweep")) return e;
    return sweep_tail(prog, a, SweepTail(), stream);
  }
  bool lean_small = false;
  if (a->X < 64 && a->X >= 2 && norm && prog->sf_ok && prog->P >= 1 && prog->P <= 4 && variant == 1 && !a->gradient) {
    if (int e = mlbp::launch_lean_sweep(prog, a, nullptr, stream, &lean_small)) return e;
    if (lean_small) {
      d.only = const_cast<mlbp_program*>(prog)->d_bail;
      d.fill_uniform = a->init_messages;
    } else if (small_lean_candidate && a->init_messages) {
      if (int e = mlbp_init_messages_f64(a->msgs, (int64_t)a->B * prog->n_msgs, a->X, stream)) return e;
    }
  }
  g_last_kernel = lean_small ? MLBP_KERNEL_LEAN : MLBP_KERNEL_GENERIC;
  size_t base = ((size_t)a->X + 4) * sizeof(double);
  size_t with_msgs = base + (size_t)prog->n_msgs * a->X * sizeof(double);
  mlbp::launch_begin();
  if (with_msgs <= 64 * 1024) {
    auto k = norm ? sweep_generic_kernel<true, true> : sweep_generic_kernel<false, true>;
    MLBP_LAUNCH(k, dim3(a->B), dim3(WG), with_msgs, st, d);
  } else {
    auto k = norm ? sweep_generic_kernel<true, false> : sweep_generic_kernel<false, false>;
    MLBP_LAUNCH(k, dim3(a->B), dim3(WG), base, st, d);
  }
  if (int e = mlbp::launch_verdict("generic sweep")) return e;
  return sweep_tail(prog, a, SweepTail(), stream);
}

int mlbp_sweep_f64(const mlbp_program* prog, const mlbp_sweep_args* a, void* stream) {
  g_last_fused_gradient = 0;
  if (!prog || !a) return fail(MLBP_EINVAL, "mlbp_sweep_f64: NULL program or args");
  prog = effective_program(prog, a);
  if (int e = check_sweep_args(prog, a)) return e;
  return run_sweep(prog, a, FAST_NONE, g_sweep_variant, stream);
}

static int finish_shared_groups(const mlbp_program* const* progs, const mlbp_sweep_args* args, int n_groups, const std::vector<char>& member,
                                void* stream, bool* done) {
  *done = false;
  std::vector<FixupGroup> table;
  std::vector<mlbp_gradient_args> grads;
  std::vector<const uint8_t*> grad_flags;
  size_t lds_max = 0;
  int blocks = 0;
  for (int k = 0; k < n_groups; ++k) {
    if (!member[k]) continue;
    const mlbp_program* prog = progs[k];
    const mlbp_sweep_args* a = &args[k];
    if (a->X != 64 || !a->normalize_messages || !a->init_messages) return MLBP_OK;
    table.emplace_back();
    FixupGroup& G = table.back();
    const size_t lds = fill_fixup_group(prog, a, &G);
    if (lds > X64_LDS_MAX) return MLBP_OK;
    lds_max = std::max(lds_max, lds);
    if (a->gradient && prog->P > 0 && !mlbp::shared_gradient_fused(prog, a)) return MLBP_OK;
    G.f.only = prog->d_bail;
    G.first_block = blocks;
    G.per_wg = prog->P == 0 ? 1 : FIXUP_GRAPHS_PER_WG;
    blocks += (a->B + G.per_wg - 1) / G.per_wg;
    if (a->gradient) { grads.push_back(*a->gradient); grad_flags.push_back(prog->d_bail); }
  }
  const int n_in = (int)table.size();
  if (!grads.empty() && (int)grads.size() != n_in) return MLBP_OK;
  static_assert(sizeof(FixupGroup) % 4 == 0, "");
  std::vector<int32_t> words(sizeof(FixupGroup) / 4 * (size_t)n_in + 1);
  memcpy(words.data(), table.data(), sizeof(FixupGroup) * (size_t)n_in);
  words.back() = 0x46495855;
  mlbp_program* owner = const_cast<mlbp_program*>(progs[0]);
  int32_t* d_table = nullptr;
  if (int e = mlbp::group_table_device(owner->stables, words, stream, &d_table)) return e;
  if (int e = mlbp::grant_lds((const void*)sweep_x64_fixup_groups_kernel, lds_max)) return e;
  mlbp::launch_begin();
  MLBP_LAUNCH(sweep_x64_fixup_groups_kernel, dim3(blocks), dim3(WG), lds_max, (hipStream_t)stream,
                     reinterpret_cast<const FixupGroup*>(d_table), n_in);
  if (int e = mlbp::launch_verdict("grouped exact X = 64 fix-up")) return e;
  if (!grads.empty())
    if (int e = mlbp::gradient_flagged_groups(grads.data(), grad_flags.data(), n_in, owner, stream)) return e;
  SweepTail tail;
  tail.marginals = false;
  tail.grad_done = true;
  for (int k = 0; k < n_groups; ++k)
    if (member[k])
      if (int e = sweep_tail(progs[k], &args[k], tail, stream)) return e;
  g_last_kernel = MLBP_KERNEL_SHARED_MFMA;
  g_last_fused_gradient = grads.empty() ? 0 : 1;
  *done = true;
  return MLBP_OK;
}

int mlbp_sweep_groups_f64(const mlbp_program* const* progs, const mlbp_sweep_args* args, int32_t n_groups, void* stream) {
  if (!progs || !args || n_groups < 1) return fail(MLBP_EINVAL, "mlbp_sweep_groups_f64: bad arguments");
  std::vector<const mlbp_program*> eff(n_groups);
  for (int k = 0; k < n_groups; ++k) {
    if (!progs[k]) return fail(MLBP_EINVAL, "mlbp_sweep_groups_f64: NULL program");
    eff[k] = effective_program(progs[k], &args[k]);
    if (int e = check_sweep_args(eff[k], &args[k])) return e;
  }
  progs = eff.data();
  const int variant = g_sweep_variant;
  std::vector<char> shared(n_groups, 0), lean(n_groups, 0);
  if (variant == 1) {
    std::vector<char> first(n_groups);
    for (int k = 0; k < n_groups; ++k) first[k] = std::find(progs, progs + k, progs[k]) == progs + k;
    shared = first;
    if (int e = mlbp::launch_shared_groups(progs, args, n_groups, stream, shared)) return e;
    if (std::find(shared.begin(), shared.end(), 1) != shared.end()) {
      bool done = false;
      if (int e = finish_shared_groups(progs, args, n_groups, shared, stream, &done)) return e;
      for (int k = 0; k < n_groups && !done; ++k)
        if (shared[k])
          if (int e = run_sweep(progs[k], &args[k], FAST_SHARED, variant, stream)) return e;
    }
    for (int k = 0; k < n_groups; ++k) lean[k] = first[k] && !shared[k];
    if (int e = mlbp::launch_lean_groups(progs, args, n_groups, stream, lean)) return e;
    for (int k = 0; k < n_groups; ++k)
      if (lean[k])
        if (int e = run_sweep(progs[k], &args[k], FAST_LEAN, variant, stream)) return e;
  }
  for (int k = 0; k < n_groups; ++k)
    if (!shared[k] && !lean[k])
      if (int e = run_sweep(progs[k], &args[k], FAST_NONE, variant, stream)) return e;
  return MLBP_OK;
}

}

namespace mlbp {
int grant_lds(const void* kernel, size_t bytes, bool* fresh) {
  static std::vector<std::pair<const void*, size_t>> granted;
  static std::mutex mu;
  std::lock_guard<std::mutex> lock(mu);
  if (fresh) *fresh = false;
  auto g = std::find_if(granted.begin(), granted.end(), [&](const std::pair<const void*, size_t>& e) { return e.first == kernel; });
  if (g != granted.end() && g->second >= bytes) return MLBP_OK;
  HIP_TRY(hipFuncSetAttribute(kernel, hipFuncAttributeMaxDynamicSharedMemorySize, (int)bytes));
  if (g != granted.end()) g->second = bytes;
  else granted.push_back({kernel, bytes});
  if (fresh) *fresh = true;
  return MLBP_OK;
}

void launch_begin() { (void)hipGetLastError(); }

int launch_verdict(const char* what) {
  const hipError_t e = hipGetLastError();
  return e == hipSuccess ? MLBP_OK : fail(MLBP_EHIP, "%s launch failed: %s", what, hipGetErrorString(e));
}

int program_grow(mlbp_program* prog, void** p, size_t* cap, size_t bytes, bool zero) {
  if (bytes <= *cap && *p) return MLBP_OK;
  void* fresh = nullptr;
  if (hipMalloc(&fresh, bytes ? bytes : 1) != hipSuccess) return fail(MLBP_EHIP, "program scratch: allocation of %zu bytes failed", bytes);
  if (zero && hipMemset(fresh, 0, bytes) != hipSuccess) { (void)hipFree(fresh); return fail(MLBP_EHIP, "program scratch: memset failed"); }
  if (*p) prog->retired.push_back(*p);
  *p = fresh;
  *cap = bytes;
  return MLBP_OK;
}

int fallback_scratch(int purpose, size_t bytes, void** out) {
  struct Block { void* p = nullptr; size_t cap = 0; };
  static std::mutex mu;
  static std::vector<std::vector<Block>> per_device;
  int dev = 0;
  if (hipGetDevice(&dev) != hipSuccess) return fail(MLBP_EHIP, "hipGetDevice failed");
  std::lock_guard<std::mutex> lock(mu);
  if ((int)per_device.size() <= dev) per_device.resize(dev + 1, std::vector<Block>(SCRATCH_PURPOSES));
  Block& b = per_device[dev][purpose];
  if (bytes > b.cap) {
    void* fresh = nullptr;
    const size_t want = bytes > 2 * b.cap ? bytes : 2 * b.cap;
    if (hipMalloc(&fresh, want) != hipSuccess) return fail(MLBP_EHIP, "scratch allocation of %zu bytes failed", want);
    b.p = fresh; b.cap = want;
  }
  *out = b.p;
  return MLBP_OK;
}

int group_table_device(GroupTables& gt, const std::vector<int32_t>& table, void* stream, int32_t** out) {
  for (auto& e : gt.entries)
    if (e.words == table) { *out = e.dev; return MLBP_OK; }
  if (getenv("MLBP_DEBUG_GROUP_TABLE")) {
// ... 4 lines not shown
          if (e.words[i] != table[i]) { fprintf(stderr, "  first difference to a cached table at word %zu: %d vs %d\n", i, e.words[i], table[i]); break; }
  }
  GroupTables::Entry* slot = nullptr;
  if (gt.entries.size() < (size_t)GroupTables::MAX) { gt.entries.emplace_back(); slot = &gt.entries.back(); }
  else { slot = &gt.entries[gt.next_evict]; gt.next_evict = (gt.next_evict + 1) % GroupTables::MAX; }
  if (table.size() > slot->cap_words) {
    int32_t* fresh = nullptr;
    if (hipMalloc(&fresh, table.size() * sizeof(int32_t)) != hipSuccess) return fail(MLBP_EHIP, "group table allocation failed");
    (void)hipFree(slot->dev);
    slot->dev = fresh; slot->cap_words = table.size();
  }
  slot->words = table;
  if (hipMemcpyAsync(slot->dev, slot->words.data(), table.size() * sizeof(int32_t), hipMemcpyHostToDevice, (hipStream_t)stream) != hipSuccess)
    return fail(MLBP_EHIP, "group table upload failed");
  *out = slot->dev;
  return MLBP_OK;
}

void group_tables_free(GroupTables& gt) {
  for (auto& e : gt.entries) (void)hipFree(e.dev);
  gt.entries.clear();
}
}

extern "C" {

int mlbp_program_reserve(mlbp_program* p, int32_t max_graphs) {
  if (!p || max_graphs <= 0) return fail(MLBP_EINVAL, "mlbp_program_reserve: bad arguments");
  if (p->pruned)
    if (int e = mlbp_program_reserve(p->pruned, max_graphs)) return e;
  if (p->bail_cap >= max_graphs) return MLBP_OK;
  size_t cap = (size_t)p->bail_cap;
  if (int e = mlbp::program_grow(p, reinterpret_cast<void**>(&p->d_bail), &cap, (size_t)max_graphs, true)) return e;
  p->bail_cap = max_graphs;
  return MLBP_OK;
}

int mlbp_program_set_readout(mlbp_program* p, int32_t n_vars, const int32_t* in_off, const int32_t* in_slots) {
  if (!p || n_vars <= 0 || !in_off || !in_slots) return fail(MLBP_EINVAL, "mlbp_program_set_readout: bad arguments");
  if (in_off[0] != 0) return fail(MLBP_EINVAL, "in_off[0] must be 0");
  for (int v = 0; v < n_vars; ++v)
    if (in_off[v + 1] < in_off[v]) return fail(MLBP_EINVAL, "in_off must be non-decreasing");
  const int n_in = in_off[n_vars];
  for (int q = 0; q < n_in; ++q)
    if (in_slots[q] < 0 || in_slots[q] >= p->n_msgs) return fail(MLBP_EINVAL, "in_slots[%d] = %d out of [0,%d)", q, in_slots[q], p->n_msgs);
  if (p->pruned)
    if (int e = mlbp_program_set_readout(p->pruned, n_vars, in_off, in_slots)) return e;
  std::vector<int32_t> img(in_off, in_off + n_vars + 1);
  img.insert(img.end(), in_slots, in_slots + n_in);
  img.push_back(0);
  (void)hipFree(p->d_readout);
  p->d_readout = nullptr;
  HIP_TRY(hipMalloc(&p->d_readout, img.size() * sizeof(int32_t)));
  HIP_TRY(hipMemcpy(p->d_readout, img.data(), img.size() * sizeof(int32_t), hipMemcpyHostToDevice));
  p->n_vars = n_vars;
  p->n_readout = (int)img.size();
  (void)hipFree(p->d_lreadout);
  p->d_lreadout = nullptr;
  std::vector<int32_t> limg;
  if (p->lean.ok && mlbp::build_lean_readout(p->lean, p->n_msgs, n_vars, in_off, in_slots, limg)) {
    HIP_TRY(hipMalloc(&p->d_lreadout, limg.size() * sizeof(int32_t)));
    HIP_TRY(hipMemcpy(p->d_lreadout, limg.data(), limg.size() * sizeof(int32_t), hipMemcpyHostToDevice));
  }
  (void)hipFree(p->d_sreadout);
  p->d_sreadout = nullptr;
  p->n_sreadout = 0;
  std::vector<int32_t> simg;
  p->sreadout_all_based = false; p->sreadout_all_tiled = false;
  if (p->shared.ok && mlbp::build_shared_readout(p->shared, p->n_msgs, n_vars, in_off, in_slots, simg)) {
    p->sreadout_all_based = true; p->sreadout_all_tiled = true;
    for (int v = 0; v < n_vars; ++v) {
      p->sreadout_all_based &= simg[simg[v]] >= 0;
      p->sreadout_all_tiled &= simg[simg[v] + 1] >= 1;
      for (int u = 0; u < v; ++u) p->sreadout_all_based &= simg[simg[u]] != simg[simg[v]];
    }
    HIP_TRY(hipMalloc(&p->d_sreadout, simg.size() * sizeof(int32_t)));
    HIP_TRY(hipMemcpy(p->d_sreadout, simg.data(), simg.size() * sizeof(int32_t), hipMemcpyHostToDevice));
    p->n_sreadout = (int)simg.size();
  }
  return MLBP_OK;
}

int mlbp_set_sweep_variant(int32_t variant) {
  const bool known = variant == 1 || variant == 3;
  if (!known) return fail(MLBP_EINVAL, "unknown sweep variant %d", variant);
  g_sweep_variant = variant;
  return MLBP_OK;
}

int mlbp_last_sweep_kernel(void) { return g_last_kernel; }
int mlbp_last_sweep_fused_gradient(void) { return g_last_fused_gradient; }

int mlbp_program_exact_count(const mlbp_program* prog, int32_t B) {
  if (!prog || B < 0) return fail(MLBP_EINVAL, "mlbp_program_exact_count: bad arguments");
  if (prog->last_was_pruned && prog->pruned) prog = prog->pruned;
  if (!prog->d_bail || B == 0) return 0;
  if (B > prog->bail_cap) B = prog->bail_cap;
  std::vector<unsigned char> h((size_t)B);
  HIP_TRY(hipMemcpy(h.data(), prog->d_bail, (size_t)B, hipMemcpyDeviceToHost));
  int n = 0, hist[4] = {0, 0, 0, 0};
  for (unsigned char c : h) { n += c ? 1 : 0; hist[c & 3]++; }
  fail(0, "exact-kernel graphs by reason: prologue %d, main loop %d, final pass %d (shared-table kernel: 2 = degenerate total, 4 -> counted under 0 = tables not shared)", hist[1], hist[2], hist[3]);
  return n;
}

int mlbp_program_status(const mlbp_program* prog) {
  if (!prog) return fail(MLBP_EINVAL, "NULL program");
  int32_t v = 0, zero = 0;
  HIP_TRY(hipMemcpy(&v, prog->d_status, sizeof(v), hipMemcpyDeviceToHost));
  if (v) HIP_TRY(hipMemcpy(prog->d_status, &zero, sizeof(zero), hipMemcpyHostToDevice));
  if (prog->pruned) {
    const int w = mlbp_program_status(prog->pruned);
    if (w < 0) return w;
    v |= w;
  }
  return v;
}

int mlbp_program_skippable_updates(const mlbp_program* prog) {
  if (!prog) return fail(MLBP_EINVAL, "NULL program");
  return prog->n_dropped;
}

int mlbp_init_messages_f64(double* msgs, int64_t n_rows, int32_t X, void* stream) {
  if (!msgs || n_rows <= 0 || X <= 0) return fail(MLBP_EINVAL, "mlbp_init_messages_f64: bad arguments");
  if (int e = check_device()) return e;
  int64_t n = n_rows * X;
  int blocks = (int)((n + 255) / 256 < 4096 ? (n + 255) / 256 : 4096);
  mlbp::launch_begin();
  MLBP_LAUNCH(fill_kernel, dim3(blocks), dim3(256), 0, (hipStream_t)stream, msgs, n, 1.0 / (double)X);
  return mlbp::launch_verdict("message initialisation");
}

int mlbp_marginals_f64(const double* msgs, int32_t B, int32_t n_msgs, int32_t X, int32_t n_vars,
                       const int32_t* in_off, const int32_t* in_slots, int32_t normalize_messages,
                       double* out, void* stream) {
  if (!msgs || !in_off || !in_slots || !out || B <= 0 || n_msgs <= 0 || X <= 0 || n_vars <= 0)
    return fail(MLBP_EINVAL, "mlbp_marginals_f64: bad arguments");
  if (int e = check_device()) return e;
  mlbp::launch_begin();
  MLBP_LAUNCH(marginals_kernel, dim3(B), dim3(WG), 0, (hipStream_t)stream, msgs, n_msgs, X, n_vars,
                     in_off, in_slots, normalize_messages, out);
  return mlbp::launch_verdict("marginals");
}

int mlbp_log_posterior_sum_f64(const double* marginals, const int32_t* labels, int32_t B, int32_t n_vars,
                               int32_t X, double* out, double* sum_out, void* stream) {
  if (!marginals || !labels || !out || B <= 0 || n_vars <= 0 || X <= 0)
    return fail(MLBP_EINVAL, "mlbp_log_posterior_f64: bad arguments");
  if (int e = check_device()) return e;
  int32_t* status = nullptr;
  if (int e = global_status(&status)) return e;
  const int blocks = (B + LP_WG - 1) / LP_WG;
  if (sum_out && blocks > LP_MAX_BLOCKS)
    return fail(MLBP_EUNSUPPORTED, "mlbp_log_posterior_sum_f64: at most %d graphs with sum_out", LP_MAX_BLOCKS * LP_WG);
  const unsigned gen = sum_out ? next_lp_generation() : 0u;
  mlbp::launch_begin();
  MLBP_LAUNCH(log_posterior_kernel, dim3(blocks), dim3(LP_WG), 0, (hipStream_t)stream, marginals, labels, B, n_vars, X, out,
                     sum_out, status, gen);
  return mlbp::launch_verdict("log-posterior");
}

int mlbp_log_posterior_groups_f64(const mlbp_posterior_group* groups, int32_t n_groups, int64_t n_total, int32_t X, double* out,
                                  void* stream) {
  if (!groups || !out || n_groups <= 0 || n_total <= 0 || X <= 0) return fail(MLBP_EINVAL, "mlbp_log_posterior_groups_f64: bad arguments");
  if (int e = check_device()) return e;
  int32_t* status = nullptr;
  if (int e = global_status(&status)) return e;
  mlbp::launch_begin();
  MLBP_LAUNCH(log_posterior_groups_kernel, dim3((unsigned)((n_total + LP_WG - 1) / LP_WG)), dim3(LP_WG), 0, (hipStream_t)stream, groups,
                     n_groups, (long long)n_total, X, out, status);
  return mlbp::launch_verdict("grouped log-posterior");
}

// ... 7 lines not shown
```

Before: 13940.

## Let lean sweep kernel absorb exact fixup and posterior in one launch

Moves the exact fused sweep body into a shared header so the lean sweep kernel can also run the exact fallback and posterior readout for bailed graphs in the same launch. Variant 5 offers this single-launch path, and variants 4 and 5 otherwise map to variant 1. The aim is to drop the second fixup kernel launch and its extra pass over the messages. The default variant stays 1, so the new path only runs when selected, and merging the paths may raise register or LDS pressure in the lean kernel.

New measurement: 5571. 60.0% lower.

```diff
diff --git a/include/mlbp.h b/include/mlbp.h
--- a/include/mlbp.h
+++ b/include/mlbp.h
@@ -122,6 +122,7 @@
 #define MLBP_KERNEL_LEAN 7
 int mlbp_last_sweep_kernel(void);
 int mlbp_last_sweep_fused_gradient(void);
+int mlbp_last_sweep_fixup_launched(void);
 
 void mlbp_launch_log_reset(void);
 int mlbp_launch_log(const void** handles, int max);
diff --git a/macaronicusermodeling_amd/_ffi.py b/macaronicusermodeling_amd/_ffi.py
--- a/macaronicusermodeling_amd/_ffi.py
+++ b/macaronicusermodeling_amd/_ffi.py
@@ -78,6 +78,7 @@
     'mlbp_device_count': (C.c_int, []),
     'mlbp_last_sweep_kernel': (C.c_int, []),
     'mlbp_last_sweep_fused_gradient': (C.c_int, []),
+    'mlbp_last_sweep_fixup_launched': (C.c_int, []),
     'mlbp_launch_log_reset': (None, []),
     'mlbp_launch_log': (C.c_int, [C.POINTER(_vp), C.c_int]),
     'mlbp_has_loops': (C.c_int, [C.POINTER(Topology), _i32]),
diff --git a/macaronicusermodeling_amd/build.py b/macaronicusermodeling_amd/build.py
--- a/macaronicusermodeling_amd/build.py
+++ b/macaronicusermodeling_amd/build.py
@@ -42,7 +42,8 @@
 
 def build(force=False, verbose=False):
     hipcc = os.environ.get('HIPCC', '/opt/rocm/bin/hipcc')
-    headers = [os.path.join(CSRC, 'mlbp_internal.h'), os.path.join(CSRC, 'mlbp_device.h'), os.path.join(PKG, '..', 'include', 'mlbp.h')]
+    headers = [os.path.join(CSRC, 'mlbp_internal.h'), os.path.join(CSRC, 'mlbp_device.h'), os.path.join(CSRC, 'mlbp_exact.h'),
+               os.path.join(PKG, '..', 'include', 'mlbp.h')]
     lib = _build_one(hipcc, CSRC, SOURCES, headers, LIB, force, verbose)
     headers_map = [os.path.join(CSRC, 'mlbp_device.h'), os.path.join(PKG, '..', 'include', 'mlbp_map.h')]
     _build_one(hipcc, CSRC_MAP, SOURCES_MAP, headers_map, LIB_MAP, force, verbose)
diff --git a/macaronicusermodeling_amd/csrc/mlbp_exact.h b/macaronicusermodeling_amd/csrc/mlbp_exact.h
--- /dev/null
+++ b/macaronicusermodeling_amd/csrc/mlbp_exact.h
@@ -0,0 +1,439 @@
+#ifndef MLBP_EXACT_H
+#define MLBP_EXACT_H
+
+#include <hip/hip_runtime.h>
+
+#include "mlbp_device.h"
+#include "mlbp_internal.h"
+
+namespace mlbp_dev {
+
+constexpr int WG = 256;
+
+__device__ __forceinline__ void marginals_from_lds_x64(const SweepDev& d, const double* msg, int g, int wave, int lane) {
+  if (!d.marginals) return;
+  const const_i32p off = as_const(d.readout), slots = as_const(d.readout + d.n_vars + 1);
+  for (int v = wave; v < d.n_vars; v += 4) {
+    double acc = 1.0 / 64.0;
+    for (int q = off[v]; q < off[v + 1]; ++q) acc = mul_nan_to_num(msg[slots[q] * 64 + lane], acc);
+    d.marginals[((size_t)g * d.n_vars + v) * 64 + lane] = renorm(acc, wave_sum(acc), 1.0 / 64.0, true);
+  }
+}
+
+using mlbp::FOP_UNARY; using mlbp::FOP_PAIR_TM; using mlbp::FOP_PAIR_MT; using mlbp::FOP_VAR;
+using mlbp::FOP_VAR_PAIR_TM; using mlbp::FOP_VAR_PAIR_MT; using mlbp::FOP_BUNDLED;
+
+constexpr int LP_MAX_BLOCKS = 4096;
+
+struct PosteriorDev {
+  const int32_t* labels;
+  double* out;
+  double* sum_out;
+  unsigned generation;
+  int32_t pad_;
+};
+
+struct FusedDev {
+  PosteriorDev post;
+  const uint8_t* only;
+  const int32_t* image;
+  const int32_t* fsweeps;
+  int32_t n_fops, n_psrcs, n_hoist, n_cprod, n_cpw, n_ext, init;
+  int32_t n_graphs;
+};
+constexpr int FIXUP_GRAPHS_PER_WG = 64;
+
+template <bool MT>
+__device__ __forceinline__ void pair_partials(const double2 (&T)[8], const double* m, double* red, int rg, int cp,
+                                              int lane) {
+  if (MT) {
+    double a0 = 0.0, a1 = 0.0;
+#pragma unroll
+    for (int k = 0; k < 8; ++k) {
+      const double mi = m[8 * k + rg];
+      a0 += mi * T[k].x;
+      a1 += mi * T[k].y;
+    }
+    reinterpret_cast<double2*>(red + rg * 64)[cp] = make_double2(a0, a1);
+  } else {
+    const double2 mj = reinterpret_cast<const double2*>(m)[cp];
+    double v[8];
+#pragma unroll
+    for (int k = 0; k < 8; ++k) v[k] = T[k].x * mj.x + T[k].y * mj.y;
+    {
+      const bool up = lane & 8;
+#pragma unroll
+      for (int i = 0; i < 4; ++i) {
+        const double send = up ? v[i] : v[i + 4], keep = up ? v[i + 4] : v[i];
+        v[i] = keep + dpp_mov<0x140>(send);
+      }
+    }
+    {
+      const bool up = lane & 4;
+#pragma unroll
+      for (int i = 0; i < 2; ++i) {
+        const double send = up ? v[i] : v[i + 2], keep = up ? v[i + 2] : v[i];
+        v[i] = keep + dpp_mov<0x141>(send);
+      }
+    }
+    {
+      const bool up = lane & 2;
+      const double send = up ? v[0] : v[1], keep = up ? v[1] : v[0];
+      v[0] = keep + dpp_mov<0x1B>(send);
+    }
+    v[0] += dpp_mov<0xB1>(v[0]);
+    if ((lane & 1) == 0) {
+      const int k = ((lane >> 3) & 1) * 4 + ((lane >> 2) & 1) * 2 + ((lane >> 1) & 1);
+      red[((lane >> 4) & 1) * 64 + 8 * k + rg] = v[0];
+    }
+  }
+}
+
+template <int NT>
+__device__ __forceinline__ void gradient_epilogue_x64(const SweepDev& d, const GradFusedDev& gf, const double2 (&tab)[NT][8],
+                                                      const double* msg, const int32_t* umsg, const int32_t* upos,
+                                                      double* scratch, int g) {
+  const int32_t* ukind = upos + d.U;
+  const int32_t* uobs = ukind + d.U;
+  const int32_t* ulab = uobs + d.U;
+  constexpr int FEE = 3, FED = 6;
+  const int t = threadIdx.x, lane = t & 63, wave = t >> 6, rg = t >> 5, cp = t & 31;
+  double pacc[NT][FEE + 1];
+#pragma unroll
+  for (int p = 0; p < NT; ++p) {
+#pragma unroll
+    for (int f = 0; f <= FEE; ++f) pacc[p][f] = 0.0;
+    if (p < d.P) {
+      const double* c = msg + gf.pair_c_slot[p] * 64;
+      const double* r = msg + gf.pair_r_slot[p] * 64;
+      const double* phi = gf.pair_phi[p] ? gf.phi_en_en_w1 : gf.phi_en_en;
+      const double2 rj = reinterpret_cast<const double2*>(r)[cp];
+#pragma unroll
+      for (int k = 0; k < 8; ++k) {
+        const double ci = c[8 * k + rg];
+        const double w0 = (ci * rj.x) * tab[p][k].x, w1 = (ci * rj.y) * tab[p][k].y;
+        pacc[p][0] += w0 + w1;
+        const double* ph = phi + ((size_t)(8 * k + rg) * 64 + 2 * cp) * FEE;
+#pragma unroll
+        for (int f = 0; f < FEE; ++f) pacc[p][1 + f] += w0 * ph[f] + w1 * ph[FEE + f];
+      }
+#pragma unroll
+      for (int f = 0; f <= FEE; ++f) pacc[p][f] = wave_sum(pacc[p][f]);
+    }
+  }
+  double uee[FEE] = {0.0, 0.0, 0.0}, ued[FED] = {0.0, 0.0, 0.0, 0.0, 0.0, 0.0};
+  bool bad = false;
+  constexpr int UB = 3;
+  for (int u0 = wave; u0 < d.U; u0 += 4 * UB) {
+    double b[UB], pv[UB][FED];
+    int kd[UB], at[UB];
+#pragma unroll
+    for (int j = 0; j < UB; ++j) {
+      const int u = u0 + 4 * j;
+      kd[j] = -1;
+      if (u < d.U) {
+        const int kind = __builtin_amdgcn_readfirstlane(ukind[u]), obs = __builtin_amdgcn_readfirstlane(uobs[u]);
+        const int lab = __builtin_amdgcn_readfirstlane(ulab[u]);
+        const int cols = kind == 2 ? gf.Vde : 64;
+        if ((unsigned)obs >= (unsigned)cols || (unsigned)lab >= 64u) { bad = true; continue; }
+        kd[j] = kind;
+        b[j] = upos[u] ? msg[umsg[u] * 64 + lane] : 0.0;
+        if (kind == 2) {
+          const double* ph = gf.phi_en_de_t + ((size_t)obs * 64 + lane) * FED;
+          at[j] = (obs * 64 + lab) * FED;
+#pragma unroll
+          for (int f = 0; f < FED; ++f) pv[j][f] = ph[f];
+        } else {
+          const double* ph = (kind ? gf.phi_en_en_w1_t : gf.phi_en_en_t) + ((size_t)obs * 64 + lane) * FEE;
+          at[j] = (obs * 64 + lab) * FEE;
+#pragma unroll
+          for (int f = 0; f < FEE; ++f) pv[j][f] = ph[f];
+        }
+      }
+    }
+#pragma unroll
+    for (int j = 0; j < UB; ++j) {
+      if (kd[j] == 2) {
+#pragma unroll
+        for (int f = 0; f < FED; ++f) ued[f] += gf.phi_en_de_t[at[j] + f] - wave_sum(b[j] * pv[j][f]);
+      } else if (kd[j] >= 0) {
+        const double* base = kd[j] ? gf.phi_en_en_w1_t : gf.phi_en_en_t;
+#pragma unroll
+        for (int f = 0; f < FEE; ++f) uee[f] += base[at[j] + f] - wave_sum(b[j] * pv[j][f]);
+      }
+    }
+  }
+  if (bad && lane == 0) atomicExch(d.status, 1);
+  constexpr int PER = NT * (FEE + 1) + FEE + FED;
+  if (lane == 0) {
+    double* o = scratch + wave * PER;
+#pragma unroll
+    for (int p = 0; p < NT; ++p)
+#pragma unroll
+      for (int f = 0; f <= FEE; ++f) o[p * (FEE + 1) + f] = pacc[p][f];
+#pragma unroll
+    for (int f = 0; f < FEE; ++f) o[NT * (FEE + 1) + f] = uee[f];
+#pragma unroll
+    for (int f = 0; f < FED; ++f) o[NT * (FEE + 1) + FEE + f] = ued[f];
+  }
+  lds_barrier();
+  if (t == 0) {
+    double tot[PER];
+#pragma unroll
+    for (int q = 0; q < PER; ++q) tot[q] = (scratch[q] + scratch[PER + q]) + (scratch[2 * PER + q] + scratch[3 * PER + q]);
+    double gee[FEE];
+#pragma unroll
+    for (int f = 0; f < FEE; ++f) gee[f] = tot[NT * (FEE + 1) + f];
+    bool lbad = false;
+#pragma unroll
+    for (int p = 0; p < NT; ++p) {
+      if (p < d.P) {
+        const int l0 = gf.pair_label[((size_t)g * d.P + p) * 2], l1 = gf.pair_label[((size_t)g * d.P + p) * 2 + 1];
+        if ((unsigned)l0 >= 64u || (unsigned)l1 >= 64u) { lbad = true; continue; }
+        const double* phi = gf.pair_phi[p] ? gf.phi_en_en_w1 : gf.phi_en_en;
+        const double Z = tot[p * (FEE + 1)];
+#pragma unroll
+        for (int f = 0; f < FEE; ++f)
+          gee[f] += phi[((size_t)l0 * 64 + l1) * FEE + f] - (Z > 0.0 ? tot[p * (FEE + 1) + 1 + f] / Z : 0.0);
+      }
+    }
+    if (lbad) atomicExch(d.status, 1);
+#pragma unroll
+    for (int f = 0; f < FEE; ++f) gf.grad_en_en[(size_t)g * FEE + f] = gee[f];
+#pragma unroll
+    for (int f = 0; f < FED; ++f) gf.grad_en_de[(size_t)g * FED + f] = tot[NT * (FEE + 1) + FEE + f];
+  }
+}
+
+template <bool NORM, int NT, bool GRAD>
+__device__ __forceinline__ void sweep_x64_fused_body(const SweepDev& d, const FusedDev& f, const GradFusedDev& gf, const int g) {
+  extern __shared__ double lds[];
+  double* msg = lds;
+  double* gin = lds + (size_t)(d.n_msgs + f.n_ext) * 64;
+  double* red = gin + 64;
+  int32_t* prog = reinterpret_cast<int32_t*>(red + 512);
+  const int32_t* psrcs = prog + f.n_fops * 8;
+  const int32_t* phoist = psrcs + f.n_psrcs;
+  const int32_t* pcp = phoist + 2 * f.n_hoist;
+  int32_t* tabidx = const_cast<int32_t*>(pcp) + f.n_cpw;
+  int32_t* flags = tabidx + d.P + d.U;
+  int32_t* umsg = flags + 4;
+  int32_t* upos = umsg + d.U;
+
+  const int t = threadIdx.x;
+  const int lane = t & 63, wave = t >> 6;
+  const int rg = t >> 5, cp = t & 31;
+  double* gm = d.msgs + (size_t)g * d.n_msgs * 64;
+  const double uniform = 1.0 / 64.0;
+  const const_i32p c_fsweeps = as_const(f.fsweeps), c_pairseq = as_const(d.pairseq);
+
+  bool ok = true;
+  for (int i = t; i < d.P + d.U; i += WG) {
+    const int v = i < d.P ? d.pair_tab[(size_t)g * d.P + i] : d.unary_tab[(size_t)g * d.U + (i - d.P)];
+    ok &= (unsigned)v < (unsigned)(i < d.P ? d.n_pair_tables : d.n_unary_tables);
+    tabidx[i] = v;
+  }
+  {
+    const int n_img = f.n_fops * 8 + f.n_psrcs + 2 * f.n_hoist + f.n_cpw;
+    for (int i = t; i < n_img; i += WG) prog[i] = f.image[i];
+    double2* dst = reinterpret_cast<double2*>(msg);
+    if (f.init) {
+      for (int i = t; i < d.n_msgs * 32; i += WG) dst[i] = make_double2(uniform, uniform);
+    } else {
+      const double2* src = reinterpret_cast<const double2*>(gm);
+      for (int i = t; i < d.n_msgs * 32; i += WG) dst[i] = src[i];
+    }
+    if (t < 32) dst[d.n_msgs * 32 + t] = make_double2(uniform, uniform);
+    if (t == 0) flags[0] = 0;
+    if (GRAD)
+      for (int i = t; i < d.U; i += WG) {
+        umsg[i] = -1; upos[i] = 0;
+        upos[d.U + i] = gf.unary_kind[i];
+        upos[2 * d.U + i] = gf.unary_obs[(size_t)g * d.U + i];
+        upos[3 * d.U + i] = gf.unary_label[(size_t)g * d.U + i];
+      }
+  }
+  if (!__syncthreads_and(ok ? 1 : 0)) {
+    if (t == 0) atomicExch(d.status, 1);
+    return;
+  }
+
+  constexpr int NR = NT > 0 ? NT : 1;
+  double2 tab[NR][8];
+  int pair_k = 0;
+  if (NT > 0) {
+#pragma unroll
+    for (int p = 0; p < NT; ++p) {
+      if (p < d.P) {
+        const int ti = __builtin_amdgcn_readfirstlane(tabidx[p]);
+        const double2* T = reinterpret_cast<const double2*>(d.pair_tables + (size_t)ti * 4096);
+#pragma unroll
+        for (int k = 0; k < 8; ++k) tab[p][k] = T[k * WG + t];
+      }
+    }
+  } else {
+    const int s0 = c_pairseq[0];
+    if (s0 >= 0) {
+      const int ti = __builtin_amdgcn_readfirstlane(tabidx[s0]);
+      const double2* T = reinterpret_cast<const double2*>(d.pair_tables + (size_t)ti * 4096);
+#pragma unroll
+      for (int k = 0; k < 8; ++k) tab[0][k] = T[k * WG + t];
+    }
+  }
+  constexpr int HB = 8;
+  for (int h0 = wave; h0 < f.n_hoist; h0 += 4 * HB) {
+    double r[HB];
+#pragma unroll
+    for (int j = 0; j < HB; ++j) {
+      const int h = h0 + 4 * j;
+      r[j] = (h < f.n_hoist) ? d.unary_tables[(size_t)tabidx[d.P + phoist[2 * h]] * 64 + lane] : 0.0;
+    }
+#pragma unroll
+    for (int j = 0; j < HB; ++j) {
+      const int h = h0 + 4 * j;
+      if (h < f.n_hoist) {
+        const double tot = wave_sum(r[j]);
+        msg[phoist[2 * h + 1] * 64 + lane] = renorm(r[j], tot, uniform, NORM);
+        if (GRAD && lane == 0) { umsg[phoist[2 * h]] = phoist[2 * h + 1]; upos[phoist[2 * h]] = tot > 0.0 ? 1 : 0; }
+      }
+    }
+  }
+  lds_barrier();
+  {
+    int at = 0;
+    for (int k = 0; k < f.n_cprod; ++k) {
+      const int cnt = pcp[at];
+      if ((k & 3) == wave) {
+        double acc = uniform;
+        bool clean = true;
+        for (int q = 0; q < cnt; ++q) {
+          acc *= msg[pcp[at + 1 + q] * 64 + lane];
+          clean = clean && __all(__builtin_isfinite(acc));
+        }
+        msg[(d.n_msgs + 1 + k) * 64 + lane] = clean ? acc : __builtin_nan("");
+      }
+      at += 1 + cnt;
+    }
+  }
+  lds_barrier();
+
+  for (int s = 0; s < d.n_sweeps; ++s) {
+    const int op0 = c_fsweeps[2 * s], nop = c_fsweeps[2 * s + 1];
+    for (int o = op0; o < op0 + nop; ++o) {
+      const int4 h0 = reinterpret_cast<const int4*>(prog)[2 * o];
+      const int4 h1 = reinterpret_cast<const int4*>(prog)[2 * o + 1];
+      const int kind = __builtin_amdgcn_readfirstlane(h0.x) & 0xFF;
+      if (kind == FOP_UNARY) {
+        if (wave == 0) {
+          const int us = __builtin_amdgcn_readfirstlane(h0.y), c = __builtin_amdgcn_readfirstlane(h0.w);
+          const double r = d.unary_tables[(size_t)tabidx[d.P + us] * 64 + lane];
+          msg[c * 64 + lane] = renorm(r, wave_sum(r), uniform, NORM);
+        }
+        continue;
+      }
+      int pslot, dst;
+      const double* m;
+      const bool from_var = (kind == FOP_VAR || kind == FOP_VAR_PAIR_TM || kind == FOP_VAR_PAIR_MT);
+      const int c = __builtin_amdgcn_readfirstlane(h0.w);
+      if (from_var) {
+        if (wave == 0) {
+          const int a = __builtin_amdgcn_readfirstlane(h0.y), n = __builtin_amdgcn_readfirstlane(h0.z);
+          const int4 s4 = *reinterpret_cast<const int4*>(psrcs + a);
+          double acc = msg[s4.x * 64 + lane];
+          if (n > 1) acc *= msg[s4.y * 64 + lane];
+          if (n > 2) acc *= msg[s4.z * 64 + lane];
+          if (n > 3) acc *= msg[s4.w * 64 + lane];
+          for (int q = 4; q < n; ++q) acc *= msg[psrcs[a + q] * 64 + lane];
+          const bool fast = __all(acc >= 0.0 && acc < __builtin_huge_val()) && __any(acc > 0.0);
+          if (fast && kind != FOP_VAR) {
+            gin[lane] = acc;
+            if (lane == 0) flags[0] = 0;
+          } else {
+            const int ae = __builtin_amdgcn_readfirstlane(h1.z), ne = __builtin_amdgcn_readfirstlane(h1.w);
+            double ex = uniform;
+            for (int q = 0; q < ne; ++q) ex = mul_nan_to_num(msg[psrcs[ae + q] * 64 + lane], ex);
+            const double mn = renorm(ex, wave_sum(ex), uniform, NORM);
+            msg[c * 64 + lane] = mn;
+            gin[lane] = mn;
+            if (lane == 0) flags[0] = 1;
+          }
+        }
+        if (kind == FOP_VAR) continue;
+        m = gin;
+        pslot = __builtin_amdgcn_readfirstlane(h1.x);
+        dst = __builtin_amdgcn_readfirstlane(h1.y);
+      } else {
+        pslot = __builtin_amdgcn_readfirstlane(h0.y);
+        m = msg + __builtin_amdgcn_readfirstlane(h0.z) * 64;
+        dst = c;
+      }
+      const bool mt = (kind == FOP_PAIR_MT || kind == FOP_VAR_PAIR_MT);
+      lds_barrier();
+      if (NT > 0) {
+#pragma unroll
+        for (int p = 0; p < NT; ++p) {
+          if (p == pslot) {
+            if (mt) pair_partials<true>(tab[p], m, red, rg, cp, lane);
+            else pair_partials<false>(tab[p], m, red, rg, cp, lane);
+          }
+        }
+      } else {
+        double2 cur[8];
+#pragma unroll
+        for (int k = 0; k < 8; ++k) cur[k] = tab[0][k];
+        ++pair_k;
+        const int sn = c_pairseq[pair_k];
+        if (sn >= 0) {
+          const int ti = __builtin_amdgcn_readfirstlane(tabidx[sn]);
+          const double2* T = reinterpret_cast<const double2*>(d.pair_tables + (size_t)ti * 4096);
+#pragma unroll
+          for (int k = 0; k < 8; ++k) tab[0][k] = T[k * WG + t];
+        }
+        if (mt) pair_partials<true>(cur, m, red, rg, cp, lane);
+        else pair_partials<false>(cur, m, red, rg, cp, lane);
+      }
+      if (from_var && wave == 1 && flags[0] == 0) {
+        const double v = gin[lane];
+        msg[c * 64 + lane] = renorm(v, wave_sum(v), uniform, NORM);
+      }
+      lds_barrier();
+      if (wave == 0) {
+        double r;
+        if (mt) {
+          r = 0.0;
+#pragma unroll
+          for (int q = 0; q < 8; ++q) r += red[q * 64 + lane];
+        } else {
+          r = red[lane] + red[64 + lane];
+        }
+        msg[dst * 64 + lane] = renorm(r, wave_sum(r), uniform, NORM);
+      }
+    }
+  }
+  lds_barrier();
+  {
+    const double2* src = reinterpret_cast<const double2*>(msg);
+    double2* dst = reinterpret_cast<double2*>(gm);
+    for (int i = t; i < d.n_msgs * 32; i += WG) dst[i] = src[i];
+  }
+  if (NORM) marginals_from_lds_x64(d, msg, g, wave, lane);
+  if (GRAD) gradient_epilogue_x64<(NT > 0 ? NT : 1)>(d, gf, tab, msg, umsg, upos, red, g);
+}
+
+__device__ __forceinline__ double posterior_term(double entry) {
+  const double lp = log(entry);
+  return lp == -__builtin_huge_val() ? -99.99 : lp;
+}
+__device__ __forceinline__ double posterior_of_graph(const SweepDev& d, const int32_t* labels, int g) {
+  double total = 0.0;
+  for (int v = 0; v < d.n_vars; ++v) {
+    const int lab = labels[(size_t)g * d.n_vars + v];
+    if ((unsigned)lab >= 64u) { atomicExch(d.status, 1); continue; }
+    total += posterior_term(d.marginals[((size_t)g * d.n_vars + v) * 64 + lab]);
+  }
+  return total;
+}
+
+}
+
+#endif
diff --git a/macaronicusermodeling_amd/csrc/mlbp_internal.h b/macaronicusermodeling_amd/csrc/mlbp_internal.h
--- a/macaronicusermodeling_amd/csrc/mlbp_internal.h
+++ b/macaronicusermodeling_amd/csrc/mlbp_internal.h
@@ -5,7 +5,7 @@
 
 #include "../../include/mlbp.h"
 
-namespace mlbp_dev { struct GradFusedDev; }
+namespace mlbp_dev { struct GradFusedDev; struct SweepDev; struct FusedDev; }
 
 struct mlbp_program;
 
@@ -63,7 +63,8 @@
 void build_lean_program(const FusedProgram& fp, int n_msgs, LeanProgram& out);
 bool build_lean_readout(const LeanProgram& lp, int n_msgs, int n_vars, const int32_t* in_off, const int32_t* in_slots,
                         std::vector<int32_t>& image);
-int launch_lean_sweep(const mlbp_program* prog, const mlbp_sweep_args* a, const mlbp_dev::GradFusedDev* gf, void* stream, bool* launched);
+int launch_lean_sweep(const mlbp_program* prog, const mlbp_sweep_args* a, const mlbp_dev::GradFusedDev* gf, void* stream, bool* launched,
+                      const mlbp_dev::SweepDev* xd = nullptr, const mlbp_dev::FusedDev* xf = nullptr, size_t xlds = 0, bool* took_all = nullptr);
 int launch_lean_groups(const mlbp_program* const* progs, const mlbp_sweep_args* args, int n_groups, void* stream, std::vector<char>& member);
 
 struct SharedProgram {
diff --git a/macaronicusermodeling_amd/csrc/mlbp_lean.hip b/macaronicusermodeling_amd/csrc/mlbp_lean.hip
--- a/macaronicusermodeling_amd/csrc/mlbp_lean.hip
+++ b/macaronicusermodeling_amd/csrc/mlbp_lean.hip
@@ -1,16 +1,16 @@
 #include <hip/hip_runtime.h>
 
+#include <algorithm>
 #include <vector>
 
 #include "mlbp_device.h"
+#include "mlbp_exact.h"
 #include "mlbp_internal.h"
 
 using mlbp::fail;
 using namespace mlbp_dev;
 
 namespace {
-
-constexpr int WG = 256;
 
 typedef double nt_d2 __attribute__((ext_vector_type(2)));
 #define NT_LOAD2(p) ([&] { const nt_d2 v_ = __builtin_nontemporal_load(reinterpret_cast<const nt_d2*>(p)); return make_double2(v_.x, v_.y); }())
@@ -23,8 +23,58 @@
   const int32_t* image;
   const int32_t* readout;
   uint8_t* bail;
+  unsigned* ticket;
   int32_t n_bundles, HL, n_cprod, WL, n_ext, init, dense, keep;
 };
+
+constexpr bool single_launch_instance(int NT, bool PADX, bool MULTI, int NL, bool GRAD) {
+  return !PADX && !MULTI && NL == 0 && !GRAD && (NT == 1 || NT == 3 || NT == 4 || NT == 6 || NT == 8);
+}
+
+__device__ __forceinline__ void agent_store(double* p, double v) {
+  __hip_atomic_store(reinterpret_cast<unsigned long long*>(p), (unsigned long long)__double_as_longlong(v), __ATOMIC_RELAXED, __HIP_MEMORY_SCOPE_AGENT);
+}
+__device__ __forceinline__ double agent_load(const double* p) {
+  return __longlong_as_double((long long)__hip_atomic_load(reinterpret_cast<unsigned long long*>(const_cast<double*>(p)), __ATOMIC_RELAXED, __HIP_MEMORY_SCOPE_AGENT));
+}
+
+__device__ __forceinline__ bool publish_out(const PosteriorDev& post, unsigned* ticket, int g, int n_graphs, double total) {
+  if (!post.sum_out) { post.out[g] = total; return false; }
+  agent_store(post.out + g, total);
+  asm volatile("s_waitcnt vmcnt(0)" ::: "memory");
+  return __hip_atomic_fetch_add(ticket, 1u, __ATOMIC_RELAXED, __HIP_MEMORY_SCOPE_AGENT) == (unsigned)(n_graphs - 1);
+}
+
+__device__ __forceinline__ void batch_total(const PosteriorDev& post, unsigned* ticket, int n_graphs, double* parts, double* part4) {
+  const int t = threadIdx.x, lane = t & 63, wave = __builtin_amdgcn_readfirstlane(t >> 6);
+  const int nb = (n_graphs + 63) >> 6;
+  constexpr int UB = 32;
+  for (int q0 = wave; q0 < nb; q0 += 4 * UB) {
+    double v[UB];
+#pragma unroll
+    for (int j = 0; j < UB; ++j) {
+      const int gi = (q0 + 4 * j) * 64 + lane;
+      v[j] = (q0 + 4 * j < nb && gi < n_graphs) ? agent_load(post.out + gi) : 0.0;
+    }
+#pragma unroll
+    for (int j = 0; j < UB; ++j) {
+      const double ws = wave_sum(v[j]);
+      if (q0 + 4 * j < nb && lane == 0) parts[q0 + 4 * j] = ws;
+    }
+  }
+  lds_barrier();
+  double acc = 0.0;
+  for (int q = t; q < nb; q += WG) acc += parts[q];
+  const double fs = wave_sum(acc);
+  if (lane == 0) part4[wave] = fs;
+  lds_barrier();
+  if (t == 0) {
+    double v = part4[0];
+    for (int w = 1; w < WG / 64; ++w) v += part4[w];
+    *post.sum_out = v;
+    __hip_atomic_store(ticket, 0u, __ATOMIC_RELAXED, __HIP_MEMORY_SCOPE_AGENT);
+  }
+}
 
 __device__ __forceinline__ double swapadd16(double a, double b) {
   auto lo = __builtin_amdgcn_permlane16_swap((unsigned)__double2loint(a), (unsigned)__double2loint(b), false, false);
@@ -353,8 +403,9 @@
 }
 
 template <int NT, bool PADX, bool MULTI, int NL, bool GRAD>
-__global__ __launch_bounds__(WG, (NT >= 7 ? 1 : (NT >= 4 ? 2 : 3))) void sweep_x64_lean_kernel(SweepDev d, LeanDev f, const int32_t* groups,
-                                                                                             int n_groups, GradFusedDev gf) {
+__device__ __forceinline__ int lean_sweep(SweepDev d, LeanDev f, const int32_t* groups, int n_groups, const GradFusedDev& gf,
+                                          const PosteriorDev& post, int n_graphs, double* lpw, int32_t* s_last) {
+  constexpr bool SINGLE = single_launch_instance(NT, PADX, MULTI, NL, GRAD);
   int g = blockIdx.x;
   if (MULTI) {
     int lo = 0, hi = n_groups - 1;
@@ -513,6 +564,13 @@
 #pragma unroll
   for (int q = 0; q < PW; ++q)
     pre[q] = EARLY ? f.image[min(t + q * WG, 16 * (f.n_bundles + 1) - 1)] : ((t + q * WG < 16 * (f.n_bundles + 1)) ? f.image[t + q * WG] : 0);
+  const bool take_post = SINGLE && f.ticket && post.labels;
+  constexpr bool PARK = SINGLE && NT >= 3;
+  int32_t lab_word[2] = {0, 0};
+  if (PARK) {
+#pragma unroll
+    for (int j = 0; j < 2; ++j) lab_word[j] = *(take_post ? post.labels + (size_t)g * d.n_vars + min(wave + 4 * j, d.n_vars - 1) : f.image);
+  }
   unsigned bad_key = 0;
   {
     double2* dst = reinterpret_cast<double2*>(work);
@@ -569,7 +627,7 @@
     if (t == 0) atomicExch(d.status, 1);
     if (f.init)
       for (int i = t; i < d.n_msgs * X; i += WG) gm[i] = uniform;
-    return;
+    return -1;
   }
   for (int k = wave; k < f.n_cprod; k += 4) {
     const Words16 cl = sload16(img_cprod + 16 * k);
@@ -597,7 +655,7 @@
   if (LEAN_SYNC) fill_limg();
   if (LEAN_SYNC ? vote_any(bad_key >= KEY_BAD, votes + 1024, wave, lane) : __syncthreads_or(bad_key >= KEY_BAD ? 1 : 0) != 0) {
     if (t == 0) f.bail[g] = 1;
-    return;
+    return 1;
   }
   if (!LEAN_SYNC) { fill_limg(); lds_barrier(); }
 
@@ -643,7 +701,7 @@
   }
   if (bad) {
     if (t == 0) f.bail[g] = 2;
-    return;
+    return 2;
   }
   lds_barrier();
   double marg[2] = {0.0, 0.0};
@@ -680,6 +738,20 @@
       if (!bad_out) d.marginals[((size_t)g * d.n_vars + v) * 64 + lane] = acc / wave_sum(acc);
     }
   }
+  bool lab_bad = false;
+  if (take_post) {
+#pragma unroll
+    for (int j = 0; j < 2; ++j) {
+      const int v = wave + 4 * j;
+      if (v < d.n_vars) {
+        const int lab = PARK ? __builtin_amdgcn_readfirstlane(lab_word[j]) : as_const(post.labels)[(size_t)g * d.n_vars + v];
+        double term = 0.0;
+        if ((unsigned)lab >= 64u) lab_bad = true;
+        else term = posterior_term(read_lane(marg[j], lab));
+        if (lane == 0) lpw[v] = term;
+      }
+    }
+  }
   lds_barrier();
   if (f.keep || GRAD) {
     for (int j0 = 0; j0 < f.WL; j0 += 4) {
@@ -701,7 +773,16 @@
   }
   if (LEAN_SYNC ? vote_any(bad_out, votes, wave, lane) : __syncthreads_or(bad_out ? 1 : 0) != 0) {
     if (t == 0) f.bail[g] = 3;
-    return;
+    return 3;
+  }
+  bool last = false;
+  if (take_post) {
+    if (lab_bad && lane == 0) atomicExch(d.status, 1);
+    if (t == 0) {
+      double total = 0.0;
+      for (int v = 0; v < d.n_vars; ++v) total += lpw[v];
+      last = publish_out(post, f.ticket, g, n_graphs, total);
+    }
   }
   if (f.keep && !PADX) {
     const double2* src = reinterpret_cast<const double2*>(work);
@@ -720,6 +801,38 @@
   }
   if (GRAD) {
     gradient_epilogue<NT>(d, gf, tab, reinterpret_cast<const char*>(work), gst, reinterpret_cast<double*>(red), G, g, R_, c_, b3_);
+  }
+  if (take_post && t == 0) *s_last = last ? 1 : 0;
+  return 0;
+}
+
+template <int NT, bool PADX, bool MULTI, int NL, bool GRAD>
+__global__ __launch_bounds__(WG, (NT >= 7 ? 1 : (NT >= 4 ? 2 : 3))) void sweep_x64_lean_kernel(SweepDev d, LeanDev f, const int32_t* groups,
+                                                                                             int n_groups, GradFusedDev gf, SweepDev xd, FusedDev xf) {
+  constexpr bool SINGLE = single_launch_instance(NT, PADX, MULTI, NL, GRAD);
+  __shared__ double lpw[8];
+  __shared__ double part4[WG / 64];
+  __shared__ int32_t s_last;
+  const int code = lean_sweep<NT, PADX, MULTI, NL, GRAD>(d, f, groups, n_groups, gf, xf.post, xf.n_graphs, lpw, &s_last);
+  if constexpr (SINGLE) {
+    if (!f.ticket) return;
+    const int g = blockIdx.x;
+    if (code != 0) {
+      if (code > 0) {
+        __syncthreads();
+        constexpr int XNT = NT <= 3 ? NT : 0;
+        const GradFusedDev none = {};
+        sweep_x64_fused_body<true, XNT, false>(xd, xf, none, g);
+      }
+      if (xf.post.labels) {
+        __syncthreads();
+        if (threadIdx.x == 0) s_last = publish_out(xf.post, f.ticket, g, xf.n_graphs, posterior_of_graph(xd, xf.post.labels, g)) ? 1 : 0;
+      }
+    }
+    if (!xf.post.labels || !xf.post.sum_out) return;
+    extern __shared__ double lds[];
+    lds_barrier();
+    if (s_last) batch_total(xf.post, f.ticket, xf.n_graphs, lds, part4);
   }
 }
 
@@ -761,13 +874,14 @@
   f->image = prog->d_limage; f->readout = (a->marginals && !padx) ? prog->d_lreadout : nullptr; f->bail = mp->d_bail;
   f->n_bundles = lp.n_bundles; f->HL = lp.HL; f->n_cprod = lp.n_cprod; f->WL = lp.WL;
   f->n_ext = n_ext; f->init = a->init_messages; f->dense = dense ? 1 : 0;
+  f->ticket = nullptr;
   const bool waived = (a->flags & MLBP_SWEEP_NO_MESSAGE_WRITEBACK) && !padx && (a->marginals || grad) && (!a->gradient || grad);
   f->keep = waived ? 0 : 1;
   *ok = true;
   return MLBP_OK;
 }
 
-typedef void (*lean_fn)(SweepDev, LeanDev, const int32_t*, int, GradFusedDev);
+typedef void (*lean_fn)(SweepDev, LeanDev, const int32_t*, int, GradFusedDev, SweepDev, FusedDev);
 
 template <bool MULTI>
 static lean_fn pick_lean(int P, bool padx) {
@@ -799,8 +913,12 @@
   }
 }
 
-int launch_lean_sweep(const mlbp_program* prog, const mlbp_sweep_args* a, const GradFusedDev* gf, void* stream, bool* launched) {
+static int wgs_per_cu(size_t bytes, int cap) { return (int)std::min<size_t>((size_t)cap, (160 * 1024) / std::max<size_t>(bytes, 1)); }
+
+int launch_lean_sweep(const mlbp_program* prog, const mlbp_sweep_args* a, const GradFusedDev* gf, void* stream, bool* launched,
+                      const SweepDev* xd, const FusedDev* xf, size_t xlds, bool* took_all) {
   *launched = false;
+  if (took_all) *took_all = false;
   SweepDev d;
   LeanDev f;
   size_t lds = 0;
@@ -808,11 +926,24 @@
   if (int e = lean_plan(prog, a, gf != nullptr, &ok, &d, &f, &lds)) return e;
   if (!ok) return MLBP_OK;
   lean_fn k = gf ? pick_lean_grad(prog->P) : pick_lean<false>(prog->P, a->X < 64);
+  const int nt = prog->P <= 4 ? prog->P : (prog->P <= 6 ? 6 : 8);
+  if (xd && xf && took_all && !gf && a->X == 64 && single_launch_instance(nt, false, false, prog->P == 7 ? 1 : 0, false)) {
+    const int nb = (a->B + FIXUP_GRAPHS_PER_WG - 1) / FIXUP_GRAPHS_PER_WG;
+    const bool post = xf->post.labels != nullptr, total = post && xf->post.sum_out != nullptr;
+    const size_t lds_one = std::max(std::max(lds, xlds), total ? (size_t)nb * sizeof(double) : (size_t)0);
+    const int cap = prog->P >= 7 ? 1 : (prog->P >= 4 ? 2 : 3);
+    if ((!post || prog->n_vars <= 8) && (!total || nb <= LP_MAX_BLOCKS) && lds_one <= 80 * 1024 && wgs_per_cu(lds_one, cap) == wgs_per_cu(lds, cap)) {
+      f.ticket = reinterpret_cast<unsigned*>(prog->d_status + 1);
+      lds = lds_one;
+    }
+  }
   if (int e = grant_lds((const void*)k, lds)) return e;
   launch_begin();
-  MLBP_LAUNCH(k, dim3(a->B), dim3(WG), lds, (hipStream_t)stream, d, f, nullptr, 0, gf ? *gf : GradFusedDev{});
+  MLBP_LAUNCH(k, dim3(a->B), dim3(WG), lds, (hipStream_t)stream, d, f, nullptr, 0, gf ? *gf : GradFusedDev{}, xd ? *xd : SweepDev{},
+              xf ? *xf : FusedDev{});
   if (int e = launch_verdict("lean sweep")) return e;
   *launched = true;
+  if (took_all) *took_all = f.ticket != nullptr;
   return MLBP_OK;
 }
 
@@ -855,7 +986,7 @@
   lean_fn k = pick_lean<true>(p_max, false);
   if (int e = grant_lds((const void*)k, lds_max)) return e;
   launch_begin();
-  MLBP_LAUNCH(k, dim3(total), dim3(WG), lds_max, (hipStream_t)stream, d0, f0, d_gtable, n_in, GradFusedDev{});
+  MLBP_LAUNCH(k, dim3(total), dim3(WG), lds_max, (hipStream_t)stream, d0, f0, d_gtable, n_in, GradFusedDev{}, SweepDev{}, FusedDev{});
   return launch_verdict("grouped lean sweep");
 }
 
diff --git a/macaronicusermodeling_amd/csrc/mlbp_sweep.hip b/macaronicusermodeling_amd/csrc/mlbp_sweep.hip
--- a/macaronicusermodeling_amd/csrc/mlbp_sweep.hip
+++ b/macaronicusermodeling_amd/csrc/mlbp_sweep.hip
@@ -13,13 +13,12 @@
 
 #include "mlbp_internal.h"
 #include "mlbp_device.h"
+#include "mlbp_exact.h"
 
 using mlbp::fail;
 using namespace mlbp_dev;
 
 namespace {
-
-constexpr int WG = 256;
 
 __device__ __forceinline__ bool tables_in_range(const SweepDev& d, int g) {
   bool ok = true;
@@ -32,418 +31,9 @@
   return all_ok != 0;
 }
 
-__device__ __forceinline__ void marginals_from_lds_x64(const SweepDev& d, const double* msg, int g, int wave, int lane) {
-  if (!d.marginals) return;
-  const const_i32p off = as_const(d.readout), slots = as_const(d.readout + d.n_vars + 1);
-  for (int v = wave; v < d.n_vars; v += 4) {
-    double acc = 1.0 / 64.0;
-    for (int q = off[v]; q < off[v + 1]; ++q) acc = mul_nan_to_num(msg[slots[q] * 64 + lane], acc);
-    d.marginals[((size_t)g * d.n_vars + v) * 64 + lane] = renorm(acc, wave_sum(acc), 1.0 / 64.0, true);
-  }
-}
-
-using mlbp::FOP_UNARY; using mlbp::FOP_PAIR_TM; using mlbp::FOP_PAIR_MT; using mlbp::FOP_VAR;
-using mlbp::FOP_VAR_PAIR_TM; using mlbp::FOP_VAR_PAIR_MT; using mlbp::FOP_BUNDLED;
-
-constexpr int LP_MAX_BLOCKS = 4096;
 constexpr int LP_WG = 256;
 __device__ double g_lp_partials[LP_MAX_BLOCKS];
 __device__ unsigned g_lp_done[2] = {0, 0};
-
-struct PosteriorDev {
-  const int32_t* labels;
-  double* out;
-  double* sum_out;
-  unsigned generation;
-  int32_t pad_;
-};
-
-struct FusedDev {
-  PosteriorDev post;
-  const uint8_t* only;
-  const int32_t* image;
-  const int32_t* fsweeps;
-  int32_t n_fops, n_psrcs, n_hoist, n_cprod, n_cpw, n_ext, init;
-  int32_t n_graphs;
-};
-constexpr int FIXUP_GRAPHS_PER_WG = 64;
-
-template <bool MT>
-__device__ __forceinline__ void pair_partials(const double2 (&T)[8], const double* m, double* red, int rg, int cp,
-                                              int lane) {
-  if (MT) {
-    double a0 = 0.0, a1 = 0.0;
-#pragma unroll
-    for (int k = 0; k < 8; ++k) {
-      const double mi = m[8 * k + rg];
-      a0 += mi * T[k].x;
-      a1 += mi * T[k].y;
-    }
-    reinterpret_cast<double2*>(red + rg * 64)[cp] = make_double2(a0, a1);
-  } else {
-    const double2 mj = reinterpret_cast<const double2*>(m)[cp];
-    double v[8];
-#pragma unroll
-    for (int k = 0; k < 8; ++k) v[k] = T[k].x * mj.x + T[k].y * mj.y;
-    {
-      const bool up = lane & 8;
-#pragma unroll
-      for (int i = 0; i < 4; ++i) {
-        const double send = up ? v[i] : v[i + 4], keep = up ? v[i + 4] : v[i];
-        v[i] = keep + dpp_mov<0x140>(send);
-      }
-    }
-    {
-      const bool up = lane & 4;
-#pragma unroll
-      for (int i = 0; i < 2; ++i) {
-        const double send = up ? v[i] : v[i + 2], keep = up ? v[i + 2] : v[i];
-        v[i] = keep + dpp_mov<0x141>(send);
-      }
-    }
-    {
-      const bool up = lane & 2;
-      const double send = up ? v[0] : v[1], keep = up ? v[1] : v[0];
-      v[0] = keep + dpp_mov<0x1B>(send);
-    }
-    v[0] += dpp_mov<0xB1>(v[0]);
-    if ((lane & 1) == 0) {
-      const int k = ((lane >> 3) & 1) * 4 + ((lane >> 2) & 1) * 2 + ((lane >> 1) & 1);
-      red[((lane >> 4) & 1) * 64 + 8 * k + rg] = v[0];
-    }
-  }
-}
-
-template <int NT>
-__device__ __forceinline__ void gradient_epilogue_x64(const SweepDev& d, const GradFusedDev& gf, const double2 (&tab)[NT][8],
-                                                      const double* msg, const int32_t* umsg, const int32_t* upos,
-                                                      double* scratch, int g) {
-  const int32_t* ukind = upos + d.U;
-  const int32_t* uobs = ukind + d.U;
-  const int32_t* ulab = uobs + d.U;
-  constexpr int FEE = 3, FED = 6;
-  const int t = threadIdx.x, lane = t & 63, wave = t >> 6, rg = t >> 5, cp = t & 31;
-  double pacc[NT][FEE + 1];
-#pragma unroll
-  for (int p = 0; p < NT; ++p) {
-#pragma unroll
-    for (int f = 0; f <= FEE; ++f) pacc[p][f] = 0.0;
-    if (p < d.P) {
-      const double* c = msg + gf.pair_c_slot[p] * 64;
-      const double* r = msg + gf.pair_r_slot[p] * 64;
-      const double* phi = gf.pair_phi[p] ? gf.phi_en_en_w1 : gf.phi_en_en;
-      const double2 rj = reinterpret_cast<const double2*>(r)[cp];
-#pragma unroll
-      for (int k = 0; k < 8; ++k) {
-        const double ci = c[8 * k + rg];
-        const double w0 = (ci * rj.x) * tab[p][k].x, w1 = (ci * rj.y) * tab[p][k].y;
-        pacc[p][0] += w0 + w1;
-        const double* ph = phi + ((size_t)(8 * k + rg) * 64 + 2 * cp) * FEE;
-#pragma unroll
-        for (int f = 0; f < FEE; ++f) pacc[p][1 + f] += w0 * ph[f] + w1 * ph[FEE + f];
-      }
-#pragma unroll
-      for (int f = 0; f <= FEE; ++f) pacc[p][f] = wave_sum(pacc[p][f]);
-    }
-  }
-  double uee[FEE] = {0.0, 0.0, 0.0}, ued[FED] = {0.0, 0.0, 0.0, 0.0, 0.0, 0.0};
-  bool bad = false;
-  constexpr int UB = 3;
-  for (int u0 = wave; u0 < d.U; u0 += 4 * UB) {
-    double b[UB], pv[UB][FED];
-    int kd[UB], at[UB];
-#pragma unroll
-    for (int j = 0; j < UB; ++j) {
-      const int u = u0 + 4 * j;
-      kd[j] = -1;
-      if (u < d.U) {
-        const int kind = __builtin_amdgcn_readfirstlane(ukind[u]), obs = __builtin_amdgcn_readfirstlane(uobs[u]);
-        const int lab = __builtin_amdgcn_readfirstlane(ulab[u]);
-        const int cols = kind == 2 ? gf.Vde : 64;
-        if ((unsigned)obs >= (unsigned)cols || (unsigned)lab >= 64u) { bad = true; continue; }
-        kd[j] = kind;
-        b[j] = upos[u] ? msg[umsg[u] * 64 + lane] : 0.0;
-        if (kind == 2) {
-          const double* ph = gf.phi_en_de_t + ((size_t)obs * 64 + lane) * FED;
-          at[j] = (obs * 64 + lab) * FED;
-#pragma unroll
-          for (int f = 0; f < FED; ++f) pv[j][f] = ph[f];
-        } else {
-          const double* ph = (kind ? gf.phi_en_en_w1_t : gf.phi_en_en_t) + ((size_t)obs * 64 + lane) * FEE;
-          at[j] = (obs * 64 + lab) * FEE;
-#pragma unroll
-          for (int f = 0; f < FEE; ++f) pv[j][f] = ph[f];
-        }
-      }
-    }
-#pragma unroll
-    for (int j = 0; j < UB; ++j) {
-      if (kd[j] == 2) {
-#pragma unroll
-        for (int f = 0; f < FED; ++f) ued[f] += gf.phi_en_de_t[at[j] + f] - wave_sum(b[j] * pv[j][f]);
-      } else if (kd[j] >= 0) {
-        const double* base = kd[j] ? gf.phi_en_en_w1_t : gf.phi_en_en_t;
-#pragma unroll
-        for (int f = 0; f < FEE; ++f) uee[f] += base[at[j] + f] - wave_sum(b[j] * pv[j][f]);
-      }
-    }
-  }
-  if (bad && lane == 0) atomicExch(d.status, 1);
-  constexpr int PER = NT * (FEE + 1) + FEE + FED;
-  if (lane == 0) {
-    double* o = scratch + wave * PER;
-#pragma unroll
-    for (int p = 0; p < NT; ++p)
-#pragma unroll
-      for (int f = 0; f <= FEE; ++f) o[p * (FEE + 1) + f] = pacc[p][f];
-#pragma unroll
-    for (int f = 0; f < FEE; ++f) o[NT * (FEE + 1) + f] = uee[f];
-#pragma unroll
-    for (int f = 0; f < FED; ++f) o[NT * (FEE + 1) + FEE + f] = ued[f];
-  }
-  lds_barrier();
-  if (t == 0) {
-    double tot[PER];
-#pragma unroll
-    for (int q = 0; q < PER; ++q) tot[q] = (scratch[q] + scratch[PER + q]) + (scratch[2 * PER + q] + scratch[3 * PER + q]);
-    double gee[FEE];
-#pragma unroll
-    for (int f = 0; f < FEE; ++f) gee[f] = tot[NT * (FEE + 1) + f];
-    bool lbad = false;
-#pragma unroll
-    for (int p = 0; p < NT; ++p) {
-      if (p < d.P) {
-        const int l0 = gf.pair_label[((size_t)g * d.P + p) * 2], l1 = gf.pair_label[((size_t)g * d.P + p) * 2 + 1];
-        if ((unsigned)l0 >= 64u || (unsigned)l1 >= 64u) { lbad = true; continue; }
-        const double* phi = gf.pair_phi[p] ? gf.phi_en_en_w1 : gf.phi_en_en;
-        const double Z = tot[p * (FEE + 1)];
-#pragma unroll
-        for (int f = 0; f < FEE; ++f)
-          gee[f] += phi[((size_t)l0 * 64 + l1) * FEE + f] - (Z > 0.0 ? tot[p * (FEE + 1) + 1 + f] / Z : 0.0);
-      }
-    }
-    if (lbad) atomicExch(d.status, 1);
-#pragma unroll
-    for (int f = 0; f < FEE; ++f) gf.grad_en_en[(size_t)g * FEE + f] = gee[f];
-#pragma unroll
-    for (int f = 0; f < FED; ++f) gf.grad_en_de[(size_t)g * FED + f] = tot[NT * (FEE + 1) + FEE + f];
-  }
-}
-
-template <bool NORM, int NT, bool GRAD>
-__device__ __forceinline__ void sweep_x64_fused_body(const SweepDev& d, const FusedDev& f, const GradFusedDev& gf, const int g) {
-  extern __shared__ double lds[];
-  double* msg = lds;
-  double* gin = lds + (size_t)(d.n_msgs + f.n_ext) * 64;
-  double* red = gin + 64;
-  int32_t* prog = reinterpret_cast<int32_t*>(red + 512);
-  const int32_t* psrcs = prog + f.n_fops * 8;
-  const int32_t* phoist = psrcs + f.n_psrcs;
-  const int32_t* pcp = phoist + 2 * f.n_hoist;
-  int32_t* tabidx = const_cast<int32_t*>(pcp) + f.n_cpw;
-  int32_t* flags = tabidx + d.P + d.U;
-  int32_t* umsg = flags + 4;
-  int32_t* upos = umsg + d.U;
-
-  const int t = threadIdx.x;
-  const int lane = t & 63, wave = t >> 6;
-  const int rg = t >> 5, cp = t & 31;
-  double* gm = d.msgs + (size_t)g * d.n_msgs * 64;
-  const double uniform = 1.0 / 64.0;
-  const const_i32p c_fsweeps = as_const(f.fsweeps), c_pairseq = as_const(d.pairseq);
-
-  bool ok = true;
-  for (int i = t; i < d.P + d.U; i += WG) {
-    const int v = i < d.P ? d.pair_tab[(size_t)g * d.P + i] : d.unary_tab[(size_t)g * d.U + (i - d.P)];
-    ok &= (unsigned)v < (unsigned)(i < d.P ? d.n_pair_tables : d.n_unary_tables);
-    tabidx[i] = v;
-  }
-  {
-    const int n_img = f.n_fops * 8 + f.n_psrcs + 2 * f.n_hoist + f.n_cpw;
-    for (int i = t; i < n_img; i += WG) prog[i] = f.image[i];
-    double2* dst = reinterpret_cast<double2*>(msg);
-    if (f.init) {
-      for (int i = t; i < d.n_msgs * 32; i += WG) dst[i] = make_double2(uniform, uniform);
-    } else {
-      const double2* src = reinterpret_cast<const double2*>(gm);
-      for (int i = t; i < d.n_msgs * 32; i += WG) dst[i] = src[i];
-    }
-    if (t < 32) dst[d.n_msgs * 32 + t] = make_double2(uniform, uniform);
-    if (t == 0) flags[0] = 0;
-    if (GRAD)
-      for (int i = t; i < d.U; i += WG) {
-        umsg[i] = -1; upos[i] = 0;
-        upos[d.U + i] = gf.unary_kind[i];
-        upos[2 * d.U + i] = gf.unary_obs[(size_t)g * d.U + i];
-        upos[3 * d.U + i] = gf.unary_label[(size_t)g * d.U + i];
-      }
-  }
-  if (!__syncthreads_and(ok ? 1 : 0)) {
-    if (t == 0) atomicExch(d.status, 1);
-    return;
-  }
-
-  constexpr int NR = NT > 0 ? NT : 1;
-  double2 tab[NR][8];
-  int pair_k = 0;
-  if (NT > 0) {
-#pragma unroll
-    for (int p = 0; p < NT; ++p) {
-      if (p < d.P) {
-        const int ti = __builtin_amdgcn_readfirstlane(tabidx[p]);
-        const double2* T = reinterpret_cast<const double2*>(d.pair_tables + (size_t)ti * 4096);
-#pragma unroll
-        for (int k = 0; k < 8; ++k) tab[p][k] = T[k * WG + t];
-      }
-    }
-  } else {
-    const int s0 = c_pairseq[0];
-    if (s0 >= 0) {
-      const int ti = __builtin_amdgcn_readfirstlane(tabidx[s0]);
-      const double2* T = reinterpret_cast<const double2*>(d.pair_tables + (size_t)ti * 4096);
-#pragma unroll
-      for (int k = 0; k < 8; ++k) tab[0][k] = T[k * WG + t];
-    }
-  }
-  constexpr int HB = 8;
-  for (int h0 = wave; h0 < f.n_hoist; h0 += 4 * HB) {
-    double r[HB];
-#pragma unroll
-    for (int j = 0; j < HB; ++j) {
-      const int h = h0 + 4 * j;
-      r[j] = (h < f.n_hoist) ? d.unary_tables[(size_t)tabidx[d.P + phoist[2 * h]] * 64 + lane] : 0.0;
-    }
-#pragma unroll
-    for (int j = 0; j < HB; ++j) {
-      const int h = h0 + 4 * j;
-      if (h < f.n_hoist) {
-        const double tot = wave_sum(r[j]);
-        msg[phoist[2 * h + 1] * 64 + lane] = renorm(r[j], tot, uniform, NORM);
-        if (GRAD && lane == 0) { umsg[phoist[2 * h]] = phoist[2 * h + 1]; upos[phoist[2 * h]] = tot > 0.0 ? 1 : 0; }
-      }
-    }
-  }
-  lds_barrier();
-  {
-    int at = 0;
-    for (int k = 0; k < f.n_cprod; ++k) {
-      const int cnt = pcp[at];
-      if ((k & 3) == wave) {
-        double acc = uniform;
-        bool clean = true;
-        for (int q = 0; q < cnt; ++q) {
-          acc *= msg[pcp[at + 1 + q] * 64 + lane];
-          clean = clean && __all(__builtin_isfinite(acc));
-        }
-        msg[(d.n_msgs + 1 + k) * 64 + lane] = clean ? acc : __builtin_nan("");
-      }
-      at += 1 + cnt;
-    }
-  }
-  lds_barrier();
-
-  for (int s = 0; s < d.n_sweeps; ++s) {
-    const int op0 = c_fsweeps[2 * s], nop = c_fsweeps[2 * s + 1];
-    for (int o = op0; o < op0 + nop; ++o) {
-      const int4 h0 = reinterpret_cast<const int4*>(prog)[2 * o];
-      const int4 h1 = reinterpret_cast<const int4*>(prog)[2 * o + 1];
-      const int kind = __builtin_amdgcn_readfirstlane(h0.x) & 0xFF;
-      if (kind == FOP_UNARY) {
-        if (wave == 0) {
-          const int us = __builtin_amdgcn_readfirstlane(h0.y), c = __builtin_amdgcn_readfirstlane(h0.w);
-          const double r = d.unary_tables[(size_t)tabidx[d.P + us] * 64 + lane];
-          msg[c * 64 + lane] = renorm(r, wave_sum(r), uniform, NORM);
-        }
-        continue;
-      }
-      int pslot, dst;
-      const double* m;
-      const bool from_var = (kind == FOP_VAR || kind == FOP_VAR_PAIR_TM || kind == FOP_VAR_PAIR_MT);
-      const int c = __builtin_amdgcn_readfirstlane(h0.w);
-      if (from_var) {
-        if (wave == 0) {
-          const int a = __builtin_amdgcn_readfirstlane(h0.y), n = __builtin_amdgcn_readfirstlane(h0.z);
-          const int4 s4 = *reinterpret_cast<const int4*>(psrcs + a);
-          double acc = msg[s4.x * 64 + lane];
-          if (n > 1) acc *= msg[s4.y * 64 + lane];
-          if (n > 2) acc *= msg[s4.z * 64 + lane];
-          if (n > 3) acc *= msg[s4.w * 64 + lane];
-          for (int q = 4; q < n; ++q) acc *= msg[psrcs[a + q] * 64 + lane];
-          const bool fast = __all(acc >= 0.0 && acc < __builtin_huge_val()) && __any(acc > 0.0);
-          if (fast && kind != FOP_VAR) {
-            gin[lane] = acc;
-            if (lane == 0) flags[0] = 0;
-          } else {
-            const int ae = __builtin_amdgcn_readfirstlane(h1.z), ne = __builtin_amdgcn_readfirstlane(h1.w);
-            double ex = uniform;
-            for (int q = 0; q < ne; ++q) ex = mul_nan_to_num(msg[psrcs[ae + q] * 64 + lane], ex);
-            const double mn = renorm(ex, wave_sum(ex), uniform, NORM);
-            msg[c * 64 + lane] = mn;
-            gin[lane] = mn;
-            if (lane == 0) flags[0] = 1;
-          }
-        }
-        if (kind == FOP_VAR) continue;
-        m = gin;
-        pslot = __builtin_amdgcn_readfirstlane(h1.x);
-        dst = __builtin_amdgcn_readfirstlane(h1.y);
-      } else {
-        pslot = __builtin_amdgcn_readfirstlane(h0.y);
-        m = msg + __builtin_amdgcn_readfirstlane(h0.z) * 64;
-        dst = c;
-      }
-      const bool mt = (kind == FOP_PAIR_MT || kind == FOP_VAR_PAIR_MT);
-      lds_barrier();
-      if (NT > 0) {
-#pragma unroll
-        for (int p = 0; p < NT; ++p) {
-          if (p == pslot) {
-            if (mt) pair_partials<true>(tab[p], m, red, rg, cp, lane);
-            else pair_partials<false>(tab[p], m, red, rg, cp, lane);
-          }
-        }
-      } else {
-        double2 cur[8];
-#pragma unroll
-        for (int k = 0; k < 8; ++k) cur[k] = tab[0][k];
-        ++pair_k;
-        const int sn = c_pairseq[pair_k];
-        if (sn >= 0) {
-          const int ti = __builtin_amdgcn_readfirstlane(tabidx[sn]);
-          const double2* T = reinterpret_cast<const double2*>(d.pair_tables + (size_t)ti * 4096);
-#pragma unroll
-          for (int k = 0; k < 8; ++k) tab[0][k] = T[k * WG + t];
-        }
-        if (mt) pair_partials<true>(cur, m, red, rg, cp, lane);
-        else pair_partials<false>(cur, m, red, rg, cp, lane);
-      }
-      if (from_var && wave == 1 && flags[0] == 0) {
-        const double v = gin[lane];
-        msg[c * 64 + lane] = renorm(v, wave_sum(v), uniform, NORM);
-      }
-      lds_barrier();
-      if (wave == 0) {
-        double r;
-        if (mt) {
-          r = 0.0;
-#pragma unroll
-          for (int q = 0; q < 8; ++q) r += red[q * 64 + lane];
-        } else {
-          r = red[lane] + red[64 + lane];
-        }
-        msg[dst * 64 + lane] = renorm(r, wave_sum(r), uniform, NORM);
-      }
-    }
-  }
-  lds_barrier();
-  {
-    const double2* src = reinterpret_cast<const double2*>(msg);
-    double2* dst = reinterpret_cast<double2*>(gm);
-    for (int i = t; i < d.n_msgs * 32; i += WG) dst[i] = src[i];
-  }
-  if (NORM) marginals_from_lds_x64(d, msg, g, wave, lane);
-  if (GRAD) gradient_epilogue_x64<(NT > 0 ? NT : 1)>(d, gf, tab, msg, umsg, upos, red, g);
-}
 
 __device__ __forceinline__ int posterior_prefetch_label(const SweepDev& d, const PosteriorDev& p, int base, int n_graphs) {
   const int t = threadIdx.x, v = t >> 6, g = base + (t & 63);
@@ -462,10 +52,7 @@
     double lp = 0.0;
     if (wave < d.n_vars && base + lane < n_graphs) {
       if ((unsigned)my_label >= 64u) atomicExch(d.status, 1);
-      else {
-        lp = log(d.marginals[((size_t)(base + lane) * d.n_vars + wave) * 64 + my_label]);
-        if (lp == -__builtin_huge_val()) lp = -99.99;
-      }
+      else lp = posterior_term(d.marginals[((size_t)(base + lane) * d.n_vars + wave) * 64 + my_label]);
     }
     lpv[t] = lp;
     __syncthreads();
@@ -474,12 +61,7 @@
       p.out[g] = total;
     }
   } else if (t < FIXUP_GRAPHS_PER_WG && g < n_graphs) {
-    for (int v = 0; v < d.n_vars; ++v) {
-      const int lab = p.labels[(size_t)g * d.n_vars + v];
-      if ((unsigned)lab >= 64u) { atomicExch(d.status, 1); continue; }
-      const double lp = log(d.marginals[((size_t)g * d.n_vars + v) * 64 + lab]);
-      total += (lp == -__builtin_huge_val()) ? -99.99 : lp;
-    }
+    total = posterior_of_graph(d, p.labels, g);
     p.out[g] = total;
   }
   if (!p.sum_out) return;
@@ -895,6 +477,7 @@
 
 int g_sweep_variant = 1;
 thread_local int g_last_kernel = -1;
+thread_local int g_last_fixup_launched = 0;
 thread_local int g_last_fused_gradient = 0;
 }
 
@@ -985,8 +568,8 @@
   if (e == hipSuccess) e = up(&p->d_srcs, srcs_padded.data(), srcs_padded.size());
   if (e == hipSuccess) e = up(&p->d_sweeps, sweeps, (size_t)n_sweeps * 2);
   if (e == hipSuccess) e = up(&p->d_pairseq, pairseq.data(), pairseq.size());
-  int32_t zero = 0;
-  if (e == hipSuccess) e = up(&p->d_status, &zero, 1);
+  const int32_t zero[2] = {0, 0};
+  if (e == hipSuccess) e = up(&p->d_status, zero, 2);
   mlbp::FusedProgram fp;
   mlbp::build_fused_program(ops, srcs, sweeps, n_sweeps, n_msgs, fp);
   p->n_fops = (int)fp.fops.size() / 8;
@@ -1163,6 +746,9 @@
 
 static int run_sweep(const mlbp_program* prog, const mlbp_sweep_args* a, FastPass pass, int variant, void* stream) {
   g_last_fused_gradient = 0;
+  g_last_fixup_launched = 0;
+  const bool two_launches = variant != 5;
+  if (variant == 4 || variant == 5) variant = 1;
   hipStream_t st = (hipStream_t)stream;
   const bool norm = a->normalize_messages != 0;
   FixupGroup G;
@@ -1190,16 +776,26 @@
       gf.phi_en_en_t = ga->phi_en_en_t; gf.phi_en_en_w1_t = ga->phi_en_en_w1_t; gf.phi_en_de_t = ga->phi_en_de_t;
       gf.grad_en_en = ga->grad_en_en; gf.grad_en_de = ga->grad_en_de; gf.Vde = ga->Vde; gf.enabled = 1;
     }
+    const mlbp_posterior_args* pa = a->posterior;
     if (pass == FAST_NONE && fast && norm && prog->sf_ok && prog->P >= 1 && prog->P <= 8) {
-      bool launched = false;
-      if (int e = mlbp::launch_lean_sweep(prog, a, tail.grad_done ? &gf : nullptr, stream, &launched)) return e;
+      bool launched = false, took_all = false;
+      FusedDev xf = G.f;
+      if (pa) { xf.post.labels = pa->labels; xf.post.out = pa->out; xf.post.sum_out = pa->sum_out; }
+      const bool offer = !two_launches && !tail.grad_done;
+      if (int e = mlbp::launch_lean_sweep(prog, a, tail.grad_done ? &gf : nullptr, stream, &launched, offer ? &G.d : nullptr,
+                                          offer ? &xf : nullptr, lds, offer ? &took_all : nullptr)) return e;
       if (launched) pass = FAST_LEAN;
+      if (took_all) {
+        g_last_kernel = MLBP_KERNEL_LEAN;
+        tail.post_done = true;
+        return sweep_tail(prog, a, tail, stream);
+      }
     }
     g_last_kernel = pass == FAST_SHARED ? MLBP_KERNEL_SHARED_MFMA : (pass == FAST_LEAN ? MLBP_KERNEL_LEAN : MLBP_KERNEL_EXACT);
     g_last_fused_gradient = (tail.grad_done || tail.grad_flagged) ? 1 : 0;
+    g_last_fixup_launched = pass != FAST_NONE ? 1 : 0;
     FusedDev& f = G.f;
     f.only = pass != FAST_NONE ? mp->d_bail : nullptr;
-    const mlbp_posterior_args* pa = a->posterior;
     tail.post_done = pa && f.only && norm && (a->B + FIXUP_GRAPHS_PER_WG - 1) / FIXUP_GRAPHS_PER_WG <= LP_MAX_BLOCKS;
     if (tail.post_done) {
       f.post.labels = pa->labels; f.post.out = pa->out; f.post.sum_out = pa->sum_out;
@@ -1283,6 +879,7 @@
     }
   }
   g_last_kernel = lean_small ? MLBP_KERNEL_LEAN : MLBP_KERNEL_GENERIC;
+  g_last_fixup_launched = lean_small ? 1 : 0;
   size_t base = ((size_t)a->X + 4) * sizeof(double);
   size_t with_msgs = base + (size_t)prog->n_msgs * a->X * sizeof(double);
   mlbp::launch_begin();
@@ -1353,6 +950,7 @@
     if (member[k])
       if (int e = sweep_tail(progs[k], &args[k], tail, stream)) return e;
   g_last_kernel = MLBP_KERNEL_SHARED_MFMA;
+  g_last_fixup_launched = 1;
   g_last_fused_gradient = grads.empty() ? 0 : 1;
   *done = true;
   return MLBP_OK;
@@ -1367,7 +965,8 @@
     if (int e = check_sweep_args(eff[k], &args[k])) return e;
   }
   progs = eff.data();
-  const int variant = g_sweep_variant;
+  g_last_fixup_launched = 0;
+  const int variant = (g_sweep_variant == 4 || g_sweep_variant == 5) ? 1 : g_sweep_variant;
   std::vector<char> shared(n_groups, 0), lean(n_groups, 0);
   if (variant == 1) {
     std::vector<char> first(n_groups);
@@ -1538,7 +1137,7 @@
 }
 
 int mlbp_set_sweep_variant(int32_t variant) {
-  const bool known = variant == 1 || variant == 3;
+  const bool known = variant == 1 || variant == 3 || variant == 4 || variant == 5;
   if (!known) return fail(MLBP_EINVAL, "unknown sweep variant %d", variant);
   g_sweep_variant = variant;
   return MLBP_OK;
@@ -1546,6 +1145,7 @@
 
 int mlbp_last_sweep_kernel(void) { return g_last_kernel; }
 int mlbp_last_sweep_fused_gradient(void) { return g_last_fused_gradient; }
+int mlbp_last_sweep_fixup_launched(void) { return g_last_fixup_launched; }
 
 int mlbp_program_exact_count(const mlbp_program* prog, int32_t B) {
   if (!prog || B < 0) return fail(MLBP_EINVAL, "mlbp_program_exact_count: bad arguments");
```
